# phcavelar/graph-odenet

Measured on AMD Instinct MI355X. Metric: full-graph ODE-GCN forward+backward steps/sec at 64 RK4 evals, higher is better.
Workload: dtype f32; 1 GPU; RMAT scale-20 / 10000000 edges (+self loops, dedup) row-normalised, d=128, ODEGCN3 rk4(3/8) 16 steps = 64 f-evals fwd, adjoint bwd, Adam; one graph per GPU; nodes=1048576, nnz=10758918, nfeat=128, hidden=128, nclass=16, parallelism=dp1 (one graph per rank, 1 gradient all-reduce/step)

## Files before the change

### graph_odenet_amd/_lib.py

```python
import ctypes
import os

import torch

_HERE = os.path.dirname(os.path.abspath(__file__))
LIB_PATH = os.path.join(_HERE, "libgraphode.so")

GODE_MAX_TERMS = 8


class LinComb(ctypes.Structure):
    _fields_ = [("n", ctypes.c_int32),
                ("coef", ctypes.c_float * GODE_MAX_TERMS),
                ("ptr", ctypes.c_void_p * GODE_MAX_TERMS)]


class SpmmEpilogue(ctypes.Structure):
    _fields_ = [("bias", ctypes.c_void_p), ("relu", ctypes.c_int32), ("alpha", ctypes.c_float),
                ("pre", LinComb), ("cot", LinComb), ("Y2", ctypes.c_void_p), ("Y2_colsum", ctypes.c_void_p)]


class Graph(ctypes.Structure):
    _fields_ = [("rowptr", ctypes.c_void_p), ("col", ctypes.c_void_p), ("val", ctypes.c_void_p),
                ("items", ctypes.c_void_p), ("n_items", ctypes.c_int64),
                ("long_rows", ctypes.c_void_p), ("n_long", ctypes.c_int64), ("partial", ctypes.c_void_p),
                ("n_rows", ctypes.c_int64), ("nnz", ctypes.c_int64)]


class GcnOdeFunc(ctypes.Structure):
    _fields_ = [("A", Graph), ("AT", Graph), ("n", ctypes.c_int64), ("d", ctypes.c_int64),
                ("groups", ctypes.c_int32), ("eps", ctypes.c_float),
                ("W", ctypes.c_void_p), ("b", ctypes.c_void_p), ("gamma", ctypes.c_void_p), ("beta", ctypes.c_void_p)]


class GatProj(ctypes.Structure):
    _fields_ = [("ps", ctypes.c_void_p), ("ld_s", ctypes.c_int64), ("pt", ctypes.c_void_p), ("ld_t", ctypes.c_int64),
                ("as_", ctypes.c_void_p), ("at", ctypes.c_void_p), ("ld_a", ctypes.c_int64)]


class Rk4Workspace(ctypes.Structure):
    _fields_ = [("S", ctypes.c_void_p), ("dZ", ctypes.c_void_p), ("dS", ctypes.c_void_p), ("S2", ctypes.c_void_p),
                ("ky", ctypes.c_void_p * 4), ("ka", ctypes.c_void_p * 4), ("ktheta", ctypes.c_void_p * 4),
                ("wpart", ctypes.c_void_p), ("gpart", ctypes.c_void_p), ("bpart", ctypes.c_void_p),
                ("colsum_scratch", ctypes.c_void_p), ("X", ctypes.c_void_p * 2), ("small_part", ctypes.c_void_p),
                ("y2_colsum", ctypes.c_void_p)]


class ReduceSeg(ctypes.Structure):
    _fields_ = [("out", ctypes.c_void_p), ("part", ctypes.c_void_p), ("n_part", ctypes.c_int64), ("ld", ctypes.c_int64),
                ("col0", ctypes.c_int64), ("col_stride", ctypes.c_int64), ("len", ctypes.c_int64),
                ("w_row0", ctypes.c_void_p), ("time_len", ctypes.c_int64)]


class GatOdeFunc(ctypes.Structure):
    _fields_ = [("mt", Graph), ("ms_inc", Graph), ("mt_inc", Graph), ("src", ctypes.c_void_p), ("tgt", ctypes.c_void_p),
                ("n_edges", ctypes.c_int64), ("n", ctypes.c_int64), ("d", ctypes.c_int64), ("groups", ctypes.c_int32),
                ("eps_gn", ctypes.c_float), ("eps", ctypes.c_float), ("Wsrc", ctypes.c_void_p), ("Wtgt", ctypes.c_void_p),
                ("Wlog", ctypes.c_void_p), ("bf", ctypes.c_void_p), ("bw", ctypes.c_void_p), ("gamma", ctypes.c_void_p),
                ("beta", ctypes.c_void_p), ("heads", ctypes.c_int32), ("Wpacked", ctypes.c_void_p)]


class GatWorkspace(ctypes.Structure):
    _fields_ = [(k, ctypes.c_void_p) for k in ("X", "Ps", "Pt", "A2", "a", "amax", "wgt", "den", "logits_scratch", "dz", "da",
                                               "dPs", "dPt", "dA2", "pair", "gp", "bp")] + \
               [("wp", ctypes.c_void_p * 3), ("maxpath_scratch", ctypes.c_void_p), ("colsum_scratch", ctypes.c_void_p),
                ("zeros", ctypes.c_void_p), ("heads_scratch", ctypes.c_void_p), ("colsum_scratch2", ctypes.c_void_p),
                ("small_part", ctypes.c_void_p)]


GODE_ADAM_MAX_TENSORS = 64


class AdamArgs(ctypes.Structure):
    _fields_ = [("param", ctypes.c_void_p * GODE_ADAM_MAX_TENSORS), ("grad", ctypes.c_void_p * GODE_ADAM_MAX_TENSORS),
                ("exp_avg", ctypes.c_void_p * GODE_ADAM_MAX_TENSORS), ("exp_avg_sq", ctypes.c_void_p * GODE_ADAM_MAX_TENSORS),
                ("len", ctypes.c_int64 * GODE_ADAM_MAX_TENSORS)]


c_i64 = ctypes.c_int64
c_p = ctypes.c_void_p
c_f = ctypes.c_float
c_i = ctypes.c_int

SIGNATURES = {
    "gode_abi_version": (c_i, []),
    "gode_error_string": (ctypes.c_char_p, [c_i]),
    "gode_set_option": (c_i, [ctypes.c_char_p, c_i]),
    "gode_get_option": (c_i, [ctypes.c_char_p]),
    "gode_spmm_csr_f32": (c_i, [c_p, c_p, c_p, c_p, c_i64, c_p, c_i64, c_p, c_p, c_i64, c_p, c_i64,
                                c_i64, c_i64, ctypes.POINTER(SpmmEpilogue), c_p]),
    "gode_spmm_csr_save_f32": (c_i, [c_p, c_p, c_p, c_p, c_i64, c_p, c_i64, c_p, c_p, c_i64, c_p, c_i64,
                                     c_i64, c_i64, ctypes.POINTER(SpmmEpilogue), c_p, c_p]),
    "gode_masked_cot_parts": (c_i64, [c_i64, c_i64]),
    "gode_masked_cot_f32": (c_i, [ctypes.POINTER(LinComb), c_p, c_p, c_i64, c_i64, c_p, c_p]),
    "gode_lincomb_f32": (c_i, [c_p, ctypes.POINTER(LinComb), c_i64, c_p]),
    "gode_lincomb_multi_f32": (c_i, [c_p, c_p, c_p, ctypes.c_int32, c_p]),
    "gode_rk_errnorm_multi_f32": (c_i, [c_p, c_p, c_p, c_p, c_p, ctypes.c_int32, c_f, c_f, c_p, c_p]),
    "gode_rk_errnorm_scratch_bytes": (c_i64, []),
    "gode_rk_errnorm_f32": (c_i, [c_p, c_p, c_p, ctypes.POINTER(LinComb), c_f, c_f, c_i64, c_p, c_p]),
    "gode_rk_scaled_sumsq_f32": (c_i, [c_p, ctypes.POINTER(LinComb), c_p, c_f, c_f, c_i64, c_p, c_p]),
    "gode_gn_time_gemm_f32": (c_i, [ctypes.POINTER(LinComb), c_i64, c_i64, ctypes.c_int32, c_f, c_p, c_p,
                                    c_p, c_i64, c_i, c_f, c_p, c_p]),
    "gode_gn_time_gemm_xout_f32": (c_i, [ctypes.POINTER(LinComb), c_i64, c_i64, ctypes.c_int32, c_f, c_p, c_p,
                                         c_p, c_i64, c_i, c_f, c_p, c_p, c_p]),
    "gode_gn_time_gemm_pair_f32": (c_i, [ctypes.POINTER(LinComb), c_i64, c_i64, ctypes.c_int32, c_f, c_p, c_p, c_p, c_p,
                                         c_i, c_f, c_p, c_p, c_p, c_p]),
    "gode_gemm_bwd_parts": (c_i64, [c_i64]),
    "gode_gn_time_gemm_bwd_f32": (c_i, [ctypes.POINTER(LinComb), c_i64, c_i64, ctypes.c_int32, c_f, c_p,
                                        c_p, c_i64, c_i, c_p, c_f, ctypes.POINTER(LinComb), c_p, c_p, c_p, c_p]),
    "gode_bwd_wgrad_supported": (c_i, [c_i64, c_i64, c_i64, ctypes.c_int32]),
    "gode_bwd_wgrad_parts": (c_i64, [c_i64]),
    "gode_gn_time_gemm_bwd_wgrad_f32": (c_i, [ctypes.POINTER(LinComb), c_i64, c_i64, ctypes.c_int32, c_f, c_p, c_p, c_p, c_i64, c_i,
                                              c_p, c_f, ctypes.POINTER(LinComb), c_p, c_p, c_p, c_p, c_p]),
    "gode_group_norm_parts": (c_i64, [c_i64]),
    "gode_group_norm_f32_fwd": (c_i, [c_p, c_i64, c_i64, ctypes.c_int32, c_f, c_p, c_p, c_p, c_p]),
    "gode_group_norm_f32_bwd": (c_i, [c_p, c_i64, c_i64, ctypes.c_int32, c_f, c_p, c_p, c_p, c_p, c_p, c_p]),
    "gode_rect_gemm_f32": (c_i, [c_p, c_i64, c_i64, c_i64, c_p, c_i64, c_p, c_i64, c_p]),
    "gode_rect_gemm_nt_f32": (c_i, [c_p, c_i64, c_i64, c_i64, c_p, c_i64, c_p, c_i64, c_p]),
    "gode_rect_wgrad_parts": (c_i64, [c_i64]),
    "gode_rect_wgrad_f32": (c_i, [c_p, c_i64, c_i64, c_i64, c_p, c_i64, c_i64, c_p, c_p]),
    "gode_rect_wgrad_sum_f32": (c_i, [c_p, c_i64, c_i64, c_i64, c_p, c_i64, c_i64, c_p, c_p, c_p]),
    "gode_gemm_f32": (c_i, [c_i, c_i, c_i64, c_i64, c_i64, c_p, c_i64, c_p, c_i64, c_p, c_i64, c_p, c_i, c_p, c_i64, c_p]),
    "gode_gemm_splitk_parts": (c_i64, [c_i64, c_i64, c_i64]),
    "gode_gemm_splitk_f32": (c_i, [c_i, c_i, c_i64, c_i64, c_i64, c_p, c_i64, c_p, c_i64, c_p, c_p, c_p]),
    "gode_cut_pad": (c_i64, [c_i64]),
    "gode_cut_bf16x3_f32": (c_i, [c_p, c_i64, c_i64, c_i64, c_p, c_p]),
    "gode_pgemm_workspace_bytes": (c_i64, [c_i64, c_i64, c_i64]),
    "gode_pgemm_bf16x3": (c_i, [c_i, c_i, c_i64, c_i64, c_i64, c_p, c_p, c_p, c_i64, c_p, c_i, c_p, c_i64, c_i, c_p, c_p]),
    "gode_adam_chunk": (c_i64, []),
    "gode_adam_tick_f32": (c_i, [c_p, c_f, c_f, c_p]),
    "gode_adam_f32": (c_i, [ctypes.POINTER(AdamArgs), ctypes.c_int32, c_p, c_i64, c_p, c_f, c_f, c_f, c_f, c_f, c_p]),
    "gode_gat_small_supported": (c_i, [c_i64, c_i64, ctypes.c_int32, c_i64]),
    "gode_gat_small_parts": (c_i64, [c_i64, c_i64]),
    "gode_gat_small_part_len": (c_i64, [c_i64, c_i64]),
    "gode_gat_project_small_f32": (c_i, [ctypes.POINTER(LinComb), c_i64, c_i64, ctypes.c_int32, c_f, c_p, c_p, c_p, c_p, c_p,
                                         c_i64, c_p, c_f, c_p, c_p, c_p, c_p, c_p, c_p]),
    "gode_gat_small_pack_len": (c_i64, [c_i64, c_i64]),
    "gode_gat_small_pack_f32": (c_i, [c_p, c_p, c_p, c_i64, c_i64, c_p, c_p]),
    "gode_gat_dense_vjp_small_f32": (c_i, [ctypes.POINTER(LinComb), c_i64, c_i64, ctypes.c_int32, c_f, c_p, c_p, c_p, c_p, c_p,
                                           c_i64, c_p, c_p, c_p, c_f, ctypes.POINTER(LinComb), c_p, c_p, c_p, c_p, c_p, c_i64, c_p, c_p]),
    "gode_gat_maxpath_heads_part_f32": (c_i, [c_p, c_p, c_i64, c_i64, c_p, c_p, c_p]),
    "gode_gat_heads_block_cap": (c_i64, []),
    "gode_gat_small_finish_f32": (c_i, [c_p, c_i64, c_i64, c_i64, c_f, c_p, c_p, c_p]),
    "gode_gat_small_finish_step_f32": (c_i, [c_p, c_i64, c_i64, c_i64, ctypes.c_int32, c_p, c_p, c_p, c_p, c_p]),
    "gode_gcn_small_supported": (c_i, [c_i64, c_i64, ctypes.c_int32]),
    "gode_gcn_small_parts": (c_i64, [c_i64]),
    "gode_gcn_small_part_len": (c_i64, [c_i64]),
    "gode_gcn_feval_small_f32": (c_i, [ctypes.POINTER(GcnOdeFunc), ctypes.POINTER(LinComb), c_f, c_f, ctypes.POINTER(LinComb),
                                       ctypes.POINTER(LinComb), c_p, c_p, c_p]),
    "gode_gcn_feval_small_next_f32": (c_i, [ctypes.POINTER(GcnOdeFunc), ctypes.POINTER(LinComb), c_f, c_f, ctypes.POINTER(LinComb),
                                            ctypes.POINTER(LinComb), c_p, c_p, ctypes.POINTER(LinComb), c_p, c_p]),
    "gode_gcn_vjp_small_f32": (c_i, [ctypes.POINTER(GcnOdeFunc), ctypes.POINTER(LinComb), c_p, c_f, ctypes.POINTER(LinComb),
                                     c_p, c_p, c_p]),
    "gode_gcn_vjp_small_next_f32": (c_i, [ctypes.POINTER(GcnOdeFunc), ctypes.POINTER(LinComb), c_p, c_f, ctypes.POINTER(LinComb),
                                          c_p, c_p, ctypes.POINTER(LinComb), c_p, c_p, c_p]),
    "gode_gcn_feval_small_save_f32": (c_i, [ctypes.POINTER(GcnOdeFunc), ctypes.POINTER(LinComb), c_f, c_f,
                                            ctypes.POINTER(LinComb), c_p, c_p, c_p]),
    "gode_gcn_small_finish_f32": (c_i, [ctypes.POINTER(GcnOdeFunc), c_p, c_p, c_f, c_p]),
    "gode_gcn_small_finish_multi_f32": (c_i, [ctypes.POINTER(GcnOdeFunc), c_p, ctypes.c_int32, ctypes.POINTER(c_p), ctypes.POINTER(c_f), c_p]),
    "gode_gcn_small_finish4_f32": (c_i, [ctypes.POINTER(GcnOdeFunc), c_p, c_p, c_p, c_p, c_p]),
    "gode_wgrad_parts": (c_i64, [c_i64]),
    "gode_wgrad_f32": (c_i, [ctypes.POINTER(LinComb), c_i64, c_i64, ctypes.c_int32, c_f, c_p, c_p,
                             c_p, c_i64, c_i, c_p, c_p]),
    "gode_reduce_parts_f32": (c_i, [c_p, c_p, c_i64, c_i64, c_f, c_i, c_p]),
    "gode_reduce_parts2_f32": (c_i, [c_p, c_p, c_p, c_p, c_i64, c_i64, c_f, c_i, c_p]),
    "gode_reduce_segments_f32": (c_i, [ctypes.POINTER(ReduceSeg), ctypes.c_int32, c_f, c_p, c_p]),
    "gode_colsum_parts_f32": (c_i, [c_p, c_i64, c_i64, c_p, ctypes.POINTER(c_i64), c_p]),
    "gode_colsum_scratch_bytes": (c_i64, [c_i64, c_i64]),
    "gode_spmm_y2_colsum_rows": (c_i64, [c_i64, c_i64, c_i64]),
    "gode_colsum_f32": (c_i, [c_p, c_p, c_i64, c_i64, c_f, c_i, c_p, c_p]),
    "gode_gat_logits_scratch_bytes": (c_i64, [c_i64]),
    "gode_gat_logits_f32": (c_i, [ctypes.POINTER(GatProj), c_p, c_p, c_p, c_i64, c_p, c_p, c_p, c_p]),
    "gode_gat_agg_f32_fwd": (c_i, [ctypes.POINTER(Graph), c_p, c_p, ctypes.POINTER(GatProj), c_i64, c_p, c_p, c_p, c_f,
                                   c_p, c_p, c_p, c_p]),
    "gode_gat_agg_f32_bwd": (c_i, [ctypes.POINTER(Graph), c_p, c_p, ctypes.POINTER(GatProj), c_i64, c_p, c_p, c_p, c_p,
                                   c_p, ctypes.POINTER(LinComb), c_f, c_p, c_p, c_p, c_i64, c_p, c_i64,
                                   ctypes.POINTER(ctypes.c_int32), c_p]),
    "gode_gat_maxpath_scratch_bytes": (c_i64, [c_i64]),
    "gode_gat_maxpath_f32": (c_i, [c_p, c_p, c_p, c_i64, c_p, c_p, c_i64, c_p, c_p]),
    "gode_gat_heads_scratch_bytes": (c_i64, [c_i64, c_i64]),
    "gode_gat_logits_heads_f32": (c_i, [ctypes.POINTER(GatProj), c_p, c_p, c_p, c_i64, c_i64, c_p, c_p, c_p, c_p]),
    "gode_gat_maxpath_heads_f32": (c_i, [c_p, c_p, c_i64, c_i64, c_p, c_p, c_i64, c_p, c_p]),
    "gode_gat_heads_parts": (c_i64, [c_i64]),
    "gode_gat_logits_heads_raw_f32": (c_i, [ctypes.POINTER(GatProj), c_p, c_p, c_p, c_i64, c_i64, c_p, c_p, c_p]),
    "gode_gat_agg_heads_f32_fwd": (c_i, [ctypes.POINTER(Graph), c_p, c_p, ctypes.POINTER(GatProj), c_i64, c_p, c_p, c_p, c_i64,
                                         c_i64, c_f, c_p, c_p, c_p, c_p]),
    "gode_gat_maxpath_heads_raw_f32": (c_i, [c_p, c_p, c_i64, c_i64, c_p, c_p, c_i64, c_p, c_p]),
# ... 126 lines not shown
```

### graph_odenet_amd/csrc/api.hip

```cpp
#include "common.h"

extern "C" int gode_abi_version(void) { return GODE_ABI_VERSION; }

extern "C" const char* gode_error_string(int code) {
    switch (code) {
        case 0: return "success";
        case GODE_E_NULLPTR: return "graphode: required pointer is NULL";
        case GODE_E_SHAPE: return "graphode: invalid shape / leading dimension";
        case GODE_E_ALIGN: return "graphode: operand not 16-byte aligned";
        case GODE_E_RANGE: return "graphode: argument out of range";
        case GODE_E_UNSUPPORTED: return "graphode: unsupported configuration";
        default: break;
    }
    if (code > 0) return hipGetErrorString((hipError_t)code);
    return "graphode: unknown error";
}

#include "options.h"
#include <cstdlib>
#include <cstring>

namespace {
int env_int(const char* name, int dflt) { const char* e = getenv(name); return e ? atoi(e) : dflt; }
int g_gemm_split = -1, g_overlap = -1, g_wgrad_split = -1, g_wgrad_split_small = 0, g_bwd_pc = -1, g_fwd_pc = -1, g_small_fused = -1, g_bwd_wgrad = -1, g_y2_colsum = -1;
}

int gode_opt_gemm_split() { if (g_gemm_split < 0) { const int v = env_int("GODE_GEMM_SPLIT", 2); g_gemm_split = (v == 1 || v == 2) ? v : 0; } return g_gemm_split; }
int gode_opt_wgrad_split() {
    if (g_wgrad_split < 0) { const int v = env_int("GODE_WGRAD_SPLIT", 8); g_wgrad_split = (v == 6 || v == 8) ? v : 0; }
    return g_wgrad_split;
}
int gode_opt_wgrad_split_small() { return g_wgrad_split_small; }
int gode_opt_bwd_pc() { if (g_bwd_pc < 0) g_bwd_pc = env_int("GODE_BWD_PC", 1) != 0; return g_bwd_pc; }
int gode_opt_fwd_pc() { if (g_fwd_pc < 0) g_fwd_pc = env_int("GODE_FWD_PC", 3) & 3; return g_fwd_pc; }
int gode_opt_small_fused() { if (g_small_fused < 0) g_small_fused = env_int("GODE_SMALL_FUSED", 1) != 0; return g_small_fused; }
int gode_opt_bwd_wgrad() { if (g_bwd_wgrad < 0) g_bwd_wgrad = env_int("GODE_BWD_WGRAD", 1) != 0; return g_bwd_wgrad; }
int gode_opt_y2_colsum() { if (g_y2_colsum < 0) g_y2_colsum = env_int("GODE_Y2_COLSUM", 1) != 0; return g_y2_colsum; }
int gode_opt_overlap() { if (g_overlap < 0) g_overlap = env_int("GODE_OVERLAP", 1) != 0; return g_overlap; }

extern "C" int gode_set_option(const char* name, int value) {
    if (!name) return GODE_E_NULLPTR;
    if (!strcmp(name, "gemm_split")) { if (value < 0 || value > 2) return GODE_E_UNSUPPORTED; g_gemm_split = value; return 0; }
    if (!strcmp(name, "overlap")) { g_overlap = value != 0; return 0; }
    if (!strcmp(name, "wgrad_split_small")) { g_wgrad_split_small = value != 0; return 0; }
    if (!strcmp(name, "bwd_pc")) { g_bwd_pc = value != 0; return 0; }
    if (!strcmp(name, "small_fused")) { g_small_fused = value != 0; return 0; }
    if (!strcmp(name, "bwd_wgrad")) { g_bwd_wgrad = value != 0; return 0; }
    if (!strcmp(name, "y2_colsum")) { g_y2_colsum = value != 0; return 0; }
    if (!strcmp(name, "fwd_pc")) { if (value < 0 || value > 3) return GODE_E_UNSUPPORTED; g_fwd_pc = value; return 0; }
    if (!strcmp(name, "wgrad_split")) { if (value != 0 && value != 6 && value != 8) return GODE_E_UNSUPPORTED; g_wgrad_split = value; return 0; }
    return GODE_E_UNSUPPORTED;
}
extern "C" int gode_get_option(const char* name) {
    if (!name) return GODE_E_NULLPTR;
    if (!strcmp(name, "gemm_split")) return gode_opt_gemm_split();
    if (!strcmp(name, "overlap")) return gode_opt_overlap();
    if (!strcmp(name, "wgrad_split")) return gode_opt_wgrad_split();
    if (!strcmp(name, "wgrad_split_small")) return gode_opt_wgrad_split_small();
    if (!strcmp(name, "bwd_pc")) return gode_opt_bwd_pc();
    if (!strcmp(name, "small_fused")) return gode_opt_small_fused();
    if (!strcmp(name, "bwd_wgrad")) return gode_opt_bwd_wgrad();
    if (!strcmp(name, "y2_colsum")) return gode_opt_y2_colsum();
    if (!strcmp(name, "fwd_pc")) return gode_opt_fwd_pc();
    return GODE_E_UNSUPPORTED;
}
```

### graph_odenet_amd/csrc/common.h

```cpp
#pragma once
#include <hip/hip_runtime.h>
#include <stdint.h>
#include "../../include/graphode.h"

#define GODE_WAVE 64

struct LinComb {
    int n;
    float coef[GODE_MAX_TERMS];
    const float* ptr[GODE_MAX_TERMS];
};

static inline LinComb make_lincomb(const gode_lincomb_t* h) {
    LinComb lc;
    lc.n = 0;
    for (int j = 0; j < GODE_MAX_TERMS; ++j) { lc.coef[j] = 0.f; lc.ptr[j] = nullptr; }
    if (h) {
        lc.n = h->n;
        for (int j = 0; j < h->n && j < GODE_MAX_TERMS; ++j) { lc.coef[j] = h->coef[j]; lc.ptr[j] = h->ptr[j]; }
    }
    return lc;
}

static inline int check_lincomb(const gode_lincomb_t* h, bool required) {
    if (!h) return required ? GODE_E_NULLPTR : 0;
    if (h->n < 0 || h->n > GODE_MAX_TERMS) return GODE_E_RANGE;
    if (required && h->n == 0) return GODE_E_RANGE;
    for (int j = 0; j < h->n; ++j) if (!h->ptr[j]) return GODE_E_NULLPTR;
    return 0;
}

static inline bool lincomb_aligned16(const gode_lincomb_t* h) {
    if (!h) return true;
    for (int j = 0; j < h->n; ++j) if (((uintptr_t)h->ptr[j]) & 15) return false;
    return true;
}

template <int NT>
__device__ __forceinline__ float4 lc_load4_n(const LinComb& lc, int64_t idx) {
    float4 v[NT];
#pragma unroll
    for (int j = 0; j < NT; ++j) v[j] = *reinterpret_cast<const float4*>(lc.ptr[j] + idx);
    float4 r = make_float4(0.f, 0.f, 0.f, 0.f);
#pragma unroll
    for (int j = 0; j < NT; ++j) {
        const float c = lc.coef[j];
        r.x = fmaf(c, v[j].x, r.x); r.y = fmaf(c, v[j].y, r.y);
        r.z = fmaf(c, v[j].z, r.z); r.w = fmaf(c, v[j].w, r.w);
    }
    return r;
}

__device__ __forceinline__ float4 lc_load4(const LinComb& lc, int64_t idx) {
    switch (lc.n) {
        case 1: return lc_load4_n<1>(lc, idx);
        case 2: return lc_load4_n<2>(lc, idx);
        case 3: return lc_load4_n<3>(lc, idx);
        case 4: return lc_load4_n<4>(lc, idx);
        case 5: return lc_load4_n<5>(lc, idx);
        case 6: return lc_load4_n<6>(lc, idx);
        case 7: return lc_load4_n<7>(lc, idx);
        case 8: return lc_load4_n<8>(lc, idx);
        default: return make_float4(0.f, 0.f, 0.f, 0.f);
    }
}

__device__ __forceinline__ float lc_load1(const LinComb& lc, int64_t idx) {
    float r = 0.f;
#pragma unroll
    for (int j = 0; j < GODE_MAX_TERMS; ++j)
        if (j < lc.n) r = fmaf(lc.coef[j], lc.ptr[j][idx], r);
    return r;
}

__device__ __forceinline__ float wave_sum(float v) {
#pragma unroll
    for (int o = 32; o > 0; o >>= 1) v += __shfl_xor(v, o, 64);
    return v;
}
__device__ __forceinline__ double wave_sum(double v) {
#pragma unroll
    for (int o = 32; o > 0; o >>= 1) v += __shfl_xor(v, o, 64);
    return v;
}
__device__ __forceinline__ float wave_max(float v) {
#pragma unroll
    for (int o = 32; o > 0; o >>= 1) v = fmaxf(v, __shfl_xor(v, o, 64));
    return v;
}

int gode_set_lds_once(const void* fn, size_t bytes);
int gode_zero_f32(float* out, int64_t n, void* stream);

#define GODE_LAUNCH_CHECK() do { hipError_t e__ = hipGetLastError(); if (e__ != hipSuccess) return (int)e__; } while (0)
```

### graph_odenet_amd/csrc/dense_pc.h

```cpp
#pragma once
#include "common.h"

int gode_pc_fwd_launch(const LinComb& lc, int64_t n_rows, float eps, const float* gamma, const float* beta,
                       const float* W, int has_time, float t, float* S, float* xout, int cg, hipStream_t s);
int gode_pc_bwd_launch(const LinComb& lc, int64_t n_rows, float eps, const float* gamma, const float* W, int has_time,
                       const float* dS, float out_scale, const LinComb& pre, float* dx, float* dgamma_part,
                       float* dbeta_part, int64_t n_part, int cg, hipStream_t s);
int64_t gode_pc_bwd_wgrad_parts(int64_t n_rows);
int gode_pc_bwd_wgrad_launch(const LinComb& lc, int64_t n_rows, float eps, const float* gamma, const float* beta, const float* W,
                             int has_time, const float* dS, float out_scale, const LinComb& pre, float* dx,
                             float* dgamma_part, float* dbeta_part, int64_t n_part, float* dW_part, int cg, hipStream_t s);
```

### graph_odenet_amd/csrc/gemm.hip

```cpp
#include <map>
#include <mutex>
#include <utility>
#include "common.h"
#include "dense_common.h"
#include "dense_pc.h"
#include "options.h"
#include "prof.h"

namespace {

constexpr int kMaxBlocks = 512;
constexpr int64_t kWgradSplitMinRows = 65536;

template <int D, int NTHREADS, bool TRANSPOSE>
__device__ __forceinline__ void fill_w_lds(float* Wl, const float* __restrict__ W, int has_time) {
    constexpr int LDW = D + 4;
    constexpr int N4 = D * D / 4;
    constexpr int IT = (N4 + NTHREADS - 1) / NTHREADS;
    float4 v[IT];
#pragma unroll
    for (int it = 0; it < IT; ++it) {
        const int idx = threadIdx.x + it * NTHREADS;
        v[it] = make_float4(0.f, 0.f, 0.f, 0.f);
        if (idx < N4) v[it] = ld4(W + (int64_t)has_time * D + (int64_t)idx * 4);
// ... 71 lines not shown
    }
}

template <int NJ>
__device__ __forceinline__ void mfma_panel(const float* wl , const float4 (&xv)[NJ], f32x4 (&acc)[NJ]) {
    constexpr int LDW = 16 * NJ + 4;
    float a[2][NJ];
#pragma unroll
    for (int tt = 0; tt < NJ; ++tt) a[0][tt] = wl[16 * tt];
#pragma unroll
    for (int s = 0; s < 4 * NJ; ++s) {
        const int j = s / 4, c = s % 4;
        const float xb = c == 0 ? xv[j].x : (c == 1 ? xv[j].y : (c == 2 ? xv[j].z : xv[j].w));
        if (s + 1 < 4 * NJ) {
            const int jn = (s + 1) / 4, cn = (s + 1) % 4;
#pragma unroll
            for (int tt = 0; tt < NJ; ++tt) a[(s + 1) & 1][tt] = wl[(16 * jn + cn) * LDW + 16 * tt];
        }
#pragma unroll
        for (int tt = 0; tt < NJ; ++tt)
            acc[tt] = __builtin_amdgcn_mfma_f32_16x16x4f32(a[s & 1][tt], xb, acc[tt], 0, 0, 0);
        __builtin_amdgcn_sched_barrier(0);
    }
}

template <int NJ, int S0, int S1>
__device__ __forceinline__ void mfma_panel_part(const float* wl, const float4 (&xv)[NJ], f32x4 (&acc)[NJ]) {
    constexpr int LDW = 16 * NJ + 4;
    float a[2][NJ];
#pragma unroll
    for (int tt = 0; tt < NJ; ++tt) a[S0 & 1][tt] = wl[(16 * (S0 / 4) + (S0 % 4)) * LDW + 16 * tt];
#pragma unroll
    for (int s = S0; s < S1; ++s) {
        const int j = s / 4, c = s % 4;
        const float xb = c == 0 ? xv[j].x : (c == 1 ? xv[j].y : (c == 2 ? xv[j].z : xv[j].w));
        if (s + 1 < S1) {
            const int jn = (s + 1) / 4, cn = (s + 1) % 4;
#pragma unroll
            for (int tt = 0; tt < NJ; ++tt) a[(s + 1) & 1][tt] = wl[(16 * jn + cn) * LDW + 16 * tt];
        }
#pragma unroll
        for (int tt = 0; tt < NJ; ++tt)
            acc[tt] = __builtin_amdgcn_mfma_f32_16x16x4f32(a[s & 1][tt], xb, acc[tt], 0, 0, 0);
        __builtin_amdgcn_sched_barrier(0);
    }
}

template <int NJ>
__device__ __forceinline__ void issue_terms2(const LinComb& lc, int t0, int64_t base, bool valid, float4 (&v)[2][NJ]) {
#pragma unroll
    for (int tt = 0; tt < 2; ++tt)
        if (valid && t0 + tt < lc.n) {
#pragma unroll
            for (int j = 0; j < NJ; ++j) v[tt][j] = ld4(lc.ptr[t0 + tt] + base + 16 * j);
        }
}
template <int NJ>
__device__ __forceinline__ void fold_terms2(const LinComb& lc, int t0, bool valid, const float4 (&v)[2][NJ], float4 (&xv)[NJ]) {
#pragma unroll
    for (int tt = 0; tt < 2; ++tt)
        if (valid && t0 + tt < lc.n) {
            const float c = lc.coef[t0 + tt];
#pragma unroll
            for (int j = 0; j < NJ; ++j) {
                xv[j].x = fmaf(c, v[tt][j].x, xv[j].x); xv[j].y = fmaf(c, v[tt][j].y, xv[j].y);
                xv[j].z = fmaf(c, v[tt][j].z, xv[j].z); xv[j].w = fmaf(c, v[tt][j].w, xv[j].w);
            }
        }
}

__device__ __forceinline__ float4 to_mfma_layout(const float4 v, int src_m_lane_x4) {
    return make_float4(__int_as_float(__builtin_amdgcn_ds_bpermute(src_m_lane_x4, __float_as_int(v.x))),
                       __int_as_float(__builtin_amdgcn_ds_bpermute(src_m_lane_x4, __float_as_int(v.y))),
                       __int_as_float(__builtin_amdgcn_ds_bpermute(src_m_lane_x4, __float_as_int(v.z))),
                       __int_as_float(__builtin_amdgcn_ds_bpermute(src_m_lane_x4, __float_as_int(v.w))));
}
__device__ __forceinline__ float4 acc_to_mem_layout(const f32x4 a, int src_f_lane_x4) {
    return make_float4(__int_as_float(__builtin_amdgcn_ds_bpermute(src_f_lane_x4, __float_as_int(a[0]))),
                       __int_as_float(__builtin_amdgcn_ds_bpermute(src_f_lane_x4, __float_as_int(a[1]))),
                       __int_as_float(__builtin_amdgcn_ds_bpermute(src_f_lane_x4, __float_as_int(a[2]))),
                       __int_as_float(__builtin_amdgcn_ds_bpermute(src_f_lane_x4, __float_as_int(a[3]))));
}

template <int NJ, int CG>
__global__ __launch_bounds__(256, 2) void gn_gemm_fwd_kernel(LinComb xin, int n_rows, float eps,
                                                             const float* __restrict__ gamma,
                                                             const float* __restrict__ beta,
                                                             const float* __restrict__ W, int has_time, float t,
                                                             float* __restrict__ S, float* __restrict__ xout,
                                                             const float* __restrict__ W2, float* __restrict__ S2)
{
    constexpr int D = 16 * NJ;
    constexpr int LDW = D + 4;
    extern __shared__ __attribute__((aligned(16))) float smem[];
    if (blockIdx.y == 1) { W = W2; S = S2; xout = nullptr; }
    float* Ws = smem;
    float* Gs = smem + D * LDW;
    float* Bs = Gs + D;
    float* T0 = Bs + D;
    fill_w_lds<D, 256, false>(Ws, W, has_time);
    fill_vec_lds<D, 256>(Gs, gamma, 1.f);
    fill_vec_lds<D, 256>(Bs, beta, 0.f);
    for (int c = threadIdx.x; c < D; c += 256) T0[c] = has_time ? t * W[c] : 0.f;
    __syncthreads();
    const int wave = threadIdx.x >> 6, l = threadIdx.x & 63;
    const int r = l & 15, g = l >> 4;
    const int mr = l >> 2, mg = l & 3;
    const int to_f = (4 * r + g) * 4, to_m = (mg * 16 + mr) * 4;
    const int n_tiles = (n_rows + 15) / 16;
    const int stride = gridDim.x * 4;
    int tile = blockIdx.x * 4 + wave;
    if (tile >= n_tiles) return;
    float4 nx[NJ];
    load_tile<NJ, 2>(xin, (int64_t)(tile * 16 + mr) * D + 4 * mg, tile * 16 + mr < n_rows, nx);
    for (; tile < n_tiles; tile += stride) {
        const int row = tile * 16 + mr;
        const bool valid = row < n_rows;
        const int nrow = row + stride * 16;
        const bool nvalid = (tile + stride < n_tiles) && nrow < n_rows;
        const int64_t nbase = (int64_t)nrow * D + 4 * mg;
        float4 xv[NJ];
#pragma unroll
        for (int j = 0; j < NJ; ++j) {
            if (xout != nullptr && valid) *reinterpret_cast<float4*>(xout + (int64_t)row * D + 16 * j + 4 * mg) = nx[j];
            xv[j] = gn_forward_v<CG>(nx[j], eps, ld4(Gs + 16 * j + 4 * mg), ld4(Bs + 16 * j + 4 * mg));
            xv[j] = to_mfma_layout(xv[j], to_f);
            nx[j] = make_float4(0.f, 0.f, 0.f, 0.f);
        }
        f32x4 acc[NJ];
#pragma unroll
        for (int tt = 0; tt < NJ; ++tt) {
            const float4 w0 = ld4(T0 + 16 * tt + 4 * g);
            acc[tt] = (f32x4){w0.x, w0.y, w0.z, w0.w};
        }
        float4 v[2][NJ];
        issue_terms2<NJ>(xin, 0, nbase, nvalid, v);
        mfma_panel_part<NJ, 0, 2 * NJ>(Ws + 4 * g * LDW + r, xv, acc);
        fold_terms2<NJ>(xin, 0, nvalid, v, nx);
        issue_terms2<NJ>(xin, 2, nbase, nvalid, v);
        mfma_panel_part<NJ, 2 * NJ, 4 * NJ>(Ws + 4 * g * LDW + r, xv, acc);
        fold_terms2<NJ>(xin, 2, nvalid, v, nx);
        if (xin.n > 4) { issue_terms2<NJ>(xin, 4, nbase, nvalid, v); fold_terms2<NJ>(xin, 4, nvalid, v, nx); }
        if (xin.n > 6) { issue_terms2<NJ>(xin, 6, nbase, nvalid, v); fold_terms2<NJ>(xin, 6, nvalid, v, nx); }
#pragma unroll
        for (int tt = 0; tt < NJ; ++tt) {
            const float4 o = acc_to_mem_layout(acc[tt], to_m);
            if (valid) *reinterpret_cast<float4*>(S + (int64_t)row * D + 16 * tt + 4 * mg) = o;
        }
    }
}


__device__ __forceinline__ unsigned short bf16_bits(float x) {
    const __bf16 h = (__bf16)x;
    return __builtin_bit_cast(unsigned short, h);
}
__device__ __forceinline__ float bf16_val(unsigned short b) { return __uint_as_float((unsigned)b << 16); }
__device__ __forceinline__ void split3(float x, unsigned short& h, unsigned short& m, unsigned short& l) {
    h = bf16_bits(x);
    const float r1 = x - bf16_val(h);
    m = bf16_bits(r1);
    l = bf16_bits(r1 - bf16_val(m));
}

template <int CG, int NX>
__global__ __launch_bounds__(512, 2) void gn_gemm_fwd_split_kernel(LinComb xin, int n_rows, float eps,
                                                                   const float* __restrict__ gamma,
                                                                   const float* __restrict__ beta,
                                                                   const float* __restrict__ W, int has_time, float t,
                                                                   float* __restrict__ S)
{
    constexpr int D = 128, NJ = 8, NK = 4;
    constexpr int LDK = D + 8;
    extern __shared__ __attribute__((aligned(16))) float smem[];
    unsigned short* Wp = reinterpret_cast<unsigned short*>(smem);
    float* Gs = smem + (3 * D * LDK) / 2;
    float* Bs = Gs + D;
    float* T0 = Bs + D;
    for (int idx = threadIdx.x; idx < D * D / 4; idx += 512) {
        const int k = idx / (D / 4), n = (idx % (D / 4)) * 4;
        const float4 w = ld4(W + (int64_t)(k + has_time) * D + n);
        const float wv[4] = {w.x, w.y, w.z, w.w};
#pragma unroll
        for (int q = 0; q < 4; ++q) {
            unsigned short h, m, l;
            split3(wv[q], h, m, l);
            Wp[(0 * D + n + q) * LDK + k] = h; Wp[(1 * D + n + q) * LDK + k] = m; Wp[(2 * D + n + q) * LDK + k] = l;
        }
    }
    fill_vec_lds<D, 512>(Gs, gamma, 1.f);
    fill_vec_lds<D, 512>(Bs, beta, 0.f);
    for (int c = threadIdx.x; c < D; c += 512) T0[c] = has_time ? t * W[c] : 0.f;
    __syncthreads();
    const int wave = threadIdx.x >> 6, l = threadIdx.x & 63;
    const int r = l & 15, g = l >> 4;
    const int mr = l >> 2, mg = l & 3;
    const int to_m = (mg * 16 + mr) * 4;
    const int n_tiles = (n_rows + 15) / 16;
    constexpr int NXR = NX > 0 ? NX : 1;
    float4 raw[NXR][NJ];
    auto request = [&](int tile) {
        const int rr = tile * 16 + mr;
        const int64_t base = (int64_t)(rr < n_rows ? rr : n_rows - 1) * D + 4 * mg;
#pragma unroll
        for (int t = 0; t < NXR; ++t)
#pragma unroll
            for (int j = 0; j < NJ; ++j) raw[t][j] = ld4(xin.ptr[t] + base + 16 * j);
    };
    if (NX > 0 && blockIdx.x * 8 + wave < n_tiles) request(blockIdx.x * 8 + wave);
    for (int tile = blockIdx.x * 8 + wave; tile < n_tiles; tile += gridDim.x * 8) {
        const int row = tile * 16 + mr;
        const bool valid = row < n_rows;
        float4 xv[NJ];
        if (NX > 0) {
#pragma unroll
            for (int j = 0; j < NJ; ++j) {
                xv[j] = make_float4(0.f, 0.f, 0.f, 0.f);
#pragma unroll
                for (int t = 0; t < NXR; ++t) {
                    const float c = xin.coef[t];
                    xv[j].x = fmaf(c, raw[t][j].x, xv[j].x); xv[j].y = fmaf(c, raw[t][j].y, xv[j].y);
                    xv[j].z = fmaf(c, raw[t][j].z, xv[j].z); xv[j].w = fmaf(c, raw[t][j].w, xv[j].w);
                }
                if (!valid) xv[j] = make_float4(0.f, 0.f, 0.f, 0.f);
            }
            const int nt_ = tile + gridDim.x * 8;
// ... 870 lines not shown
int fast_cg(int64_t d_in, int64_t d_out, int32_t groups) {
    if (d_in != d_out) return -1;
    if (d_in != 16 && d_in != 32 && d_in != 64 && d_in != 128) return -1;
    if (groups == 0) return 0;
    if (d_in % groups) return -1;
    const int64_t cg = d_in / groups;
    if (cg == 1 || cg == 2 || cg == 4) return (int)cg;
    return -1;
}

int narrow_cg(int64_t d_in, int64_t d_out, int32_t groups) {
    if (d_out != 2) return -1;
    if (d_in != 16 && d_in != 32 && d_in != 64 && d_in != 128) return -1;
    if (groups == 0) return 0;
    if (d_in % groups) return -1;
    const int64_t cg = d_in / groups;
    return (cg == 1 || cg == 2 || cg == 4) ? (int)cg : -1;
}

int64_t fwd_blocks(int64_t n_rows) {
    int64_t b = ((n_rows + 15) / 16 + 3) / 4;
    if (b < 1) b = 1;
    if (b > kMaxBlocks) b = kMaxBlocks;
    return b;
}
int64_t wgrad_blocks(int64_t n_rows) {
    int64_t b = (n_rows + 31) / 32;
    if (b < 1) b = 1;
    if (b > kMaxBlocks) b = kMaxBlocks;
    return b;
}

}

int gode_set_lds_once(const void* fn, size_t bytes) {
    if (bytes <= 64 * 1024) return 0;
    static std::mutex mu;
    static std::map<std::pair<int, const void*>, size_t> done;
    int dev = 0;
    hipError_t e = hipGetDevice(&dev);
    if (e != hipSuccess) return (int)e;
    std::lock_guard<std::mutex> lk(mu);
    auto key = std::make_pair(dev, fn);
    auto it = done.find(key);
    if (it != done.end() && it->second >= bytes) return 0;
    e = hipFuncSetAttribute(fn, hipFuncAttributeMaxDynamicSharedMemorySize, (int)bytes);
    if (e != hipSuccess) return (int)e;
    done[key] = bytes;
    return 0;
}

#define GODE_DISPATCH_NJ_CG(NJV, CGV, MACRO)                                        \
    if (nj == NJV && cg == CGV) { MACRO(NJV, CGV) }

#define GODE_DISPATCH_ALL(MACRO)                                                    \
    GODE_DISPATCH_NJ_CG(1, 0, MACRO) GODE_DISPATCH_NJ_CG(1, 1, MACRO)               \
    GODE_DISPATCH_NJ_CG(2, 0, MACRO) GODE_DISPATCH_NJ_CG(2, 1, MACRO)               \
    GODE_DISPATCH_NJ_CG(4, 0, MACRO) GODE_DISPATCH_NJ_CG(4, 2, MACRO)               \
    GODE_DISPATCH_NJ_CG(8, 0, MACRO) GODE_DISPATCH_NJ_CG(8, 4, MACRO)               \
    GODE_DISPATCH_NJ_CG(1, 2, MACRO) GODE_DISPATCH_NJ_CG(1, 4, MACRO)               \
    GODE_DISPATCH_NJ_CG(2, 2, MACRO) GODE_DISPATCH_NJ_CG(2, 4, MACRO)               \
    GODE_DISPATCH_NJ_CG(4, 1, MACRO) GODE_DISPATCH_NJ_CG(4, 4, MACRO)               \
    GODE_DISPATCH_NJ_CG(8, 1, MACRO) GODE_DISPATCH_NJ_CG(8, 2, MACRO)

static int check_common(const gode_lincomb_t* xin, int64_t n_rows, int64_t d_in, int32_t groups, int64_t d_out) {
    if (n_rows < 0 || d_in <= 0 || d_out <= 0 || groups < 0) return GODE_E_SHAPE;
    if (groups > 0 && d_in % groups) return GODE_E_SHAPE;
    if (n_rows > INT32_MAX || d_in > 2048 || d_out > 65536) return GODE_E_RANGE;
    return check_lincomb(xin, true);
}

extern "C" int gode_gn_time_gemm_f32(const gode_lincomb_t* xin, int64_t n_rows, int64_t d_in, int32_t groups,
                                     float eps, const float* gamma, const float* beta, const float* W,
                                     int64_t d_out, int has_time, float t, float* S, void* stream)
{
    return gode_gn_time_gemm_xout_f32(xin, n_rows, d_in, groups, eps, gamma, beta, W, d_out, has_time, t, S, nullptr,
                                      stream);
}

extern "C" int gode_gn_time_gemm_xout_f32(const gode_lincomb_t* xin, int64_t n_rows, int64_t d_in, int32_t groups,
                                          float eps, const float* gamma, const float* beta, const float* W,
                                          int64_t d_out, int has_time, float t, float* S, float* x_out, void* stream)
{
    int rc = check_common(xin, n_rows, d_in, groups, d_out); if (rc) return rc;
    if (n_rows == 0) return 0;
    if (!W || !S) return GODE_E_NULLPTR;
    if (x_out && (((uintptr_t)x_out) & 15)) return GODE_E_ALIGN;
    has_time = has_time ? 1 : 0;
    hipStream_t s = (hipStream_t)stream;
    LinComb lc = make_lincomb(xin);
    const int cg = fast_cg(d_in, d_out, groups);
    const bool al = lincomb_aligned16(xin) && !(((uintptr_t)S) & 15) && !(((uintptr_t)W) & 15) &&
                    (!gamma || !(((uintptr_t)gamma) & 15)) && (!beta || !(((uintptr_t)beta) & 15));
    if (cg >= 0 && al && d_in == 128 && (n_rows >= kWgradSplitMinRows || gode_opt_wgrad_split_small()) &&
        ((lc.n <= 2 && !x_out) ? (gode_opt_fwd_pc() & 1) : (gode_opt_fwd_pc() & 2))) {
        rc = gode_pc_fwd_launch(lc, n_rows, eps, gamma, beta, W, has_time, t, S, x_out, cg, s);
        if (rc != GODE_E_UNSUPPORTED) return rc;
    }
    if (cg >= 0 && al && d_in == 128 && !x_out && (gode_opt_gemm_split() == 1 || (gode_opt_gemm_split() == 2 && lc.n <= 2 && n_rows >= 65536))) {
        const size_t lds = (size_t)3 * 128 * (128 + 8) * sizeof(unsigned short) + 3 * 128 * sizeof(float);
        int64_t blocks = ((n_rows + 15) / 16 + 7) / 8; if (blocks < 1) blocks = 1; if (blocks > 256) blocks = 256;
#define GODE_FWDS2(CGV, NXV) { rc = set_lds(gn_gemm_fwd_split_kernel<CGV, NXV>, lds); if (rc) return rc;    \
          const int slot = gode_prof_begin(s, d_in, n_rows, (int64_t)lc.n - 1, GODE_PROF_GEMM_FWD | GODE_PROF_FORM_SPLIT); \
          hipLaunchKernelGGL((gn_gemm_fwd_split_kernel<CGV, NXV>), dim3((unsigned)blocks), dim3(512), lds, s, \
                             lc, (int)n_rows, eps, gamma, beta, W, has_time, t, S);                           \
          gode_prof_end(s, slot);                                                                             \
          GODE_LAUNCH_CHECK(); return 0; }
#define GODE_FWDS(CGV) { if (lc.n == 1) GODE_FWDS2(CGV, 1) else if (lc.n == 2) GODE_FWDS2(CGV, 2) else GODE_FWDS2(CGV, 0) }
        if (cg == 0) GODE_FWDS(0) else if (cg == 1) GODE_FWDS(1) else if (cg == 2) GODE_FWDS(2) else GODE_FWDS(4)
#undef GODE_FWDS
#undef GODE_FWDS2
    }
    if (cg >= 0 && al) {
        const int nj = (int)(d_in / 16);
        const size_t lds = ((size_t)d_in * (d_in + 4) + 3 * d_in) * sizeof(float);
        const int64_t blocks = fwd_blocks(n_rows);
#define GODE_FWD(NJV, CGV)                                                                          \
        { rc = set_lds(gn_gemm_fwd_kernel<NJV, CGV>, lds); if (rc) return rc;                       \
          const int slot = gode_prof_begin(s, d_in, n_rows, (int64_t)lc.n - 1 + (x_out ? 1 : 0), GODE_PROF_GEMM_FWD); \
          hipLaunchKernelGGL((gn_gemm_fwd_kernel<NJV, CGV>), dim3((unsigned)blocks), dim3(256), lds, s, \
                             lc, (int)n_rows, eps, gamma, beta, W, has_time, t, S, x_out,           \
                             (const float*)nullptr, (float*)nullptr);                               \
          gode_prof_end(s, slot);                                                                   \
          GODE_LAUNCH_CHECK(); return 0; }
        GODE_DISPATCH_ALL(GODE_FWD)
#undef GODE_FWD
    }
    {
        const int cg = narrow_cg(d_in, d_out, groups);
        if (cg >= 0 && al) {
            const int nj = (int)(d_in / 16);
            const int64_t blocks = fwd_blocks(n_rows);
#define GODE_NFWD(NJV, CGV)                                                                                 \
            { hipLaunchKernelGGL((gn_narrow_fwd_kernel<NJV, CGV, 2>), dim3((unsigned)blocks), dim3(256), 0, s, \
                                 lc, (int)n_rows, eps, gamma, beta, W, has_time, t, S, x_out);              \
              GODE_LAUNCH_CHECK(); return 0; }
            GODE_DISPATCH_ALL(GODE_NFWD)
#undef GODE_NFWD
        }
    }
    if (x_out) { rc = gode_lincomb_f32(x_out, xin, n_rows * d_in, stream); if (rc) return rc; }
    const size_t lds = ((size_t)RB * d_in + (size_t)RB * (groups > 0 ? groups : 1) * 2) * sizeof(float);
    rc = set_lds(gn_gemm_fwd_generic, lds); if (rc) return rc;
    int64_t blocks = (n_rows + RB - 1) / RB; if (blocks > 2048) blocks = 2048;
    hipLaunchKernelGGL(gn_gemm_fwd_generic, dim3((unsigned)blocks), dim3(256), lds, s, lc, (int)n_rows, (int)d_in,
                       (int)groups, eps, gamma, beta, W, (int)d_out, has_time, t, S);
    GODE_LAUNCH_CHECK();
    return 0;
}

extern "C" int gode_gn_time_gemm_pair_f32(const gode_lincomb_t* xin, int64_t n_rows, int64_t d, int32_t groups, float eps,
                                          const float* gamma, const float* beta, const float* Wa, const float* Wb,
                                          int has_time, float t, float* Sa, float* Sb, float* x_out, void* stream)
{
    int rc = check_common(xin, n_rows, d, groups, d); if (rc) return rc;
    if (n_rows == 0) return 0;
    if (!Wa || !Wb || !Sa || !Sb) return GODE_E_NULLPTR;
    has_time = has_time ? 1 : 0;
    hipStream_t s = (hipStream_t)stream;
    LinComb lc = make_lincomb(xin);
    const int cg = fast_cg(d, d, groups);
    const bool al = lincomb_aligned16(xin) && !((((uintptr_t)Sa) | ((uintptr_t)Sb) | ((uintptr_t)Wa) | ((uintptr_t)Wb)) & 15) &&
                    (!gamma || !(((uintptr_t)gamma) & 15)) && (!beta || !(((uintptr_t)beta) & 15)) &&
                    (!x_out || !(((uintptr_t)x_out) & 15));
    if (cg >= 0 && al) {
        const int nj = (int)(d / 16);
        const size_t lds = ((size_t)d * (d + 4) + 3 * d) * sizeof(float);
        const int64_t blocks = fwd_blocks(n_rows);
#define GODE_FWDP(NJV, CGV)                                                                         \
        { rc = set_lds(gn_gemm_fwd_kernel<NJV, CGV>, lds); if (rc) return rc;                       \
          hipLaunchKernelGGL((gn_gemm_fwd_kernel<NJV, CGV>), dim3((unsigned)blocks, 2), dim3(256), lds, s, \
                             lc, (int)n_rows, eps, gamma, beta, Wa, has_time, t, Sa, x_out, Wb, Sb);  \
          GODE_LAUNCH_CHECK(); return 0; }
        GODE_DISPATCH_ALL(GODE_FWDP)
#undef GODE_FWDP
    }
    rc = gode_gn_time_gemm_xout_f32(xin, n_rows, d, groups, eps, gamma, beta, Wa, d, has_time, t, Sa, x_out, stream);
    if (rc) return rc;
    return gode_gn_time_gemm_f32(xin, n_rows, d, groups, eps, gamma, beta, Wb, d, has_time, t, Sb, stream);
}

extern "C" int64_t gode_gemm_bwd_parts(int64_t n_rows) {
    int64_t a = fwd_blocks(n_rows);
    int64_t b = (n_rows + RB - 1) / RB; if (b > 2048) b = 2048; if (b < 1) b = 1;
    return a > b ? a : b;
}

extern "C" int gode_gn_time_gemm_bwd_f32(const gode_lincomb_t* xin, int64_t n_rows, int64_t d_in, int32_t groups,
                                         float eps, const float* gamma, const float* W, int64_t d_out,
                                         int has_time, const float* dS, float out_scale,
                                         const gode_lincomb_t* pre, float* dx,
                                         float* dgamma_part, float* dbeta_part, void* stream)
{
    int rc = check_common(xin, n_rows, d_in, groups, d_out); if (rc) return rc;
    if (n_rows == 0) return 0;
    if (!W || !dS || !dx) return GODE_E_NULLPTR;
    if ((dgamma_part == nullptr) != (dbeta_part == nullptr)) return GODE_E_NULLPTR;
    if (pre && pre->n > 0) { rc = check_lincomb(pre, true); if (rc) return rc; } else pre = nullptr;
    has_time = has_time ? 1 : 0;
    hipStream_t s = (hipStream_t)stream;
    LinComb lc = make_lincomb(xin);
    LinComb lpre = make_lincomb(pre);
    const int64_t n_part = gode_gemm_bwd_parts(n_rows);
    const int cg = fast_cg(d_in, d_out, groups);
    const bool al = lincomb_aligned16(xin) && lincomb_aligned16(pre) && !(((uintptr_t)dS) & 15) && !(((uintptr_t)dx) & 15) &&
                    (!gamma || !(((uintptr_t)gamma) & 15)) &&
                    (!dgamma_part || (!(((uintptr_t)dgamma_part) & 15) && !(((uintptr_t)dbeta_part) & 15)));
    if ((cg == 0 || cg == 4) && al && d_in == 128 && gode_opt_bwd_pc() &&
        (n_rows >= kWgradSplitMinRows || gode_opt_wgrad_split_small())) {
        rc = gode_pc_bwd_launch(lc, n_rows, eps, gamma, W, has_time, dS, out_scale, lpre, dx, dgamma_part, dbeta_part,
                                n_part, cg, s);
        if (rc != GODE_E_UNSUPPORTED) return rc;
    }
    if (cg >= 0 && al) {
        const int nj = (int)(d_in / 16);
        size_t lds = ((size_t)d_in * (d_in + 4) + d_in) * sizeof(float);
        if (lds < (size_t)8 * d_in * sizeof(float)) lds = (size_t)8 * d_in * sizeof(float);
        const int64_t blocks = fwd_blocks(n_rows);
#define GODE_BWD(NJV, CGV)                                                                          \
        { rc = set_lds(gn_gemm_bwd_kernel<NJV, CGV>, lds); if (rc) return rc;                       \
          const int slot = gode_prof_begin(s, d_in, n_rows, (int64_t)lc.n - 1 + lpre.n, GODE_PROF_GEMM_BWD); \
          hipLaunchKernelGGL((gn_gemm_bwd_kernel<NJV, CGV>), dim3((unsigned)blocks), dim3(256), lds, s, \
                             lc, (int)n_rows, eps, gamma, W, has_time, dS, out_scale, lpre, dx, dgamma_part, dbeta_part, (int)n_part); \
          gode_prof_end(s, slot);                                                                   \
          GODE_LAUNCH_CHECK(); return 0; }
        GODE_DISPATCH_ALL(GODE_BWD)
#undef GODE_BWD
    }
    {
        const int ncg = narrow_cg(d_in, d_out, groups);
        if (ncg >= 0 && al) {
            const int nj = (int)(d_in / 16);
            const int cg = ncg;
            const int64_t blocks = fwd_blocks(n_rows);
#define GODE_NBWD(NJV, CGV)                                                                                 \
            { hipLaunchKernelGGL((gn_narrow_bwd_kernel<NJV, CGV, 2>), dim3((unsigned)blocks), dim3(256), 0, s, \
                                 lc, (int)n_rows, eps, gamma, W, has_time, dS, out_scale, lpre, dx, dgamma_part, \
                                 dbeta_part, (int)n_part);                                                  \
              GODE_LAUNCH_CHECK(); return 0; }
            GODE_DISPATCH_ALL(GODE_NBWD)
#undef GODE_NBWD
        }
    }
    const size_t g2 = (size_t)RB * (groups > 0 ? groups : 1) * 2;
    const size_t lds = ((size_t)RB * d_in * 2 + g2 * 2) * sizeof(float);
    rc = set_lds(gn_gemm_bwd_generic, lds); if (rc) return rc;
    int64_t blocks = (n_rows + RB - 1) / RB; if (blocks > 2048) blocks = 2048;
    hipLaunchKernelGGL(gn_gemm_bwd_generic, dim3((unsigned)blocks), dim3(256), lds, s, lc, (int)n_rows, (int)d_in,
                       (int)groups, eps, gamma, W, (int)d_out, has_time, dS, out_scale, lpre, dx, dgamma_part, dbeta_part,
                       (int)n_part);
    GODE_LAUNCH_CHECK();
    return 0;
}

extern "C" int gode_bwd_wgrad_supported(int64_t n_rows, int64_t d_in, int64_t d_out, int32_t groups) {
// ... 143 lines not shown
```

### graph_odenet_amd/csrc/gemm_pc.hip

```cpp
#include "common.h"
#include "dense_common.h"
#include "dense_pc.h"
#include "prof.h"

namespace {

constexpr int D = 128;
constexpr int LDK = D + 8;
constexpr int LDX = D + 4;
constexpr int kBlocks = 256;
template <int R> struct Img { static constexpr int PIECE_B = R * LDK * 2, BUF_B = 3 * PIECE_B; };

__device__ __forceinline__ bf16x8 pack8(const unsigned (&u)[8]) {
    const uint2 a = pack_hi16x4(u[0], u[1], u[2], u[3]), b = pack_hi16x4(u[4], u[5], u[6], u[7]);
    typedef unsigned u32x4 __attribute__((ext_vector_type(4)));
    const u32x4 v = {a.x, a.y, b.x, b.y};
    return __builtin_bit_cast(bf16x8, v);
}

template <typename F>
__device__ __forceinline__ void load_weight_pieces(bf16x8 (&A)[4][3], F element) {
    const int l = threadIdx.x & 63, m = l & 15, g = l >> 4;
#pragma unroll
    for (int kb = 0; kb < 4; ++kb) {
        unsigned h[8], md[8], lo[8];
#pragma unroll
        for (int e = 0; e < 8; ++e) split3_trunc(element(m, 32 * kb + 8 * g + e), h[e], md[e], lo[e]);
        A[kb][0] = pack8(h); A[kb][1] = pack8(md); A[kb][2] = pack8(lo);
    }
}

template <int R>
__device__ __forceinline__ void tile_product(const char* img , const bf16x8 (&A)[4][3], f32x4 (&acc)[R / 16]) {
    constexpr int PIECE_B = Img<R>::PIECE_B, NS = (R / 16) * 4;
    bf16x8 b[2][3];
#pragma unroll
    for (int pc = 0; pc < 3; ++pc) b[0][pc] = *reinterpret_cast<const bf16x8*>(img + pc * PIECE_B);
#pragma unroll
    for (int s = 0; s < NS; ++s) {
        const int rt = s >> 2, kb = s & 3;
        if (s + 1 < NS) {
            const int rt2 = (s + 1) >> 2, kb2 = (s + 1) & 3;
#pragma unroll
            for (int pc = 0; pc < 3; ++pc)
                b[(s + 1) & 1][pc] = *reinterpret_cast<const bf16x8*>(img + pc * PIECE_B + rt2 * 16 * LDK * 2 + kb2 * 64);
        }
        const bf16x8 bh = b[s & 1][0], bm = b[s & 1][1], bl = b[s & 1][2];
        f32x4 c = acc[rt];
        c = __builtin_amdgcn_mfma_f32_16x16x32_bf16(A[kb][2], bm, c, 0, 0, 0);
        c = __builtin_amdgcn_mfma_f32_16x16x32_bf16(A[kb][1], bl, c, 0, 0, 0);
        c = __builtin_amdgcn_mfma_f32_16x16x32_bf16(A[kb][2], bh, c, 0, 0, 0);
        c = __builtin_amdgcn_mfma_f32_16x16x32_bf16(A[kb][0], bl, c, 0, 0, 0);
        c = __builtin_amdgcn_mfma_f32_16x16x32_bf16(A[kb][1], bm, c, 0, 0, 0);
        c = __builtin_amdgcn_mfma_f32_16x16x32_bf16(A[kb][1], bh, c, 0, 0, 0);
        c = __builtin_amdgcn_mfma_f32_16x16x32_bf16(A[kb][0], bm, c, 0, 0, 0);
        c = __builtin_amdgcn_mfma_f32_16x16x32_bf16(A[kb][0], bh, c, 0, 0, 0);
        acc[rt] = c;
        __builtin_amdgcn_sched_barrier(0);
    }
}

template <int PIECE_B>
__device__ __forceinline__ void stage_row4(char* dst , const float4 v) {
    unsigned h0, m0, l0, h1, m1, l1, h2, m2, l2, h3, m3, l3;
    split3_trunc(v.x, h0, m0, l0); split3_trunc(v.y, h1, m1, l1); split3_trunc(v.z, h2, m2, l2); split3_trunc(v.w, h3, m3, l3);
    *reinterpret_cast<uint2*>(dst) = pack_hi16x4(h0, h1, h2, h3);
    *reinterpret_cast<uint2*>(dst + PIECE_B) = pack_hi16x4(m0, m1, m2, m3);
    *reinterpret_cast<uint2*>(dst + 2 * PIECE_B) = pack_hi16x4(l0, l1, l2, l3);
}

struct TileWalk {
    int n_tiles, stride, mine;
    __device__ TileWalk(int n_rows, int R) {
        n_tiles = (n_rows + R - 1) / R;
        stride = gridDim.x;
        mine = (int)blockIdx.x < n_tiles ? (n_tiles - 1 - (int)blockIdx.x) / stride + 1 : 0;
    }
    __device__ int tile(int k) const { return blockIdx.x + k * stride; }
    __device__ int clamped(int k) const { return blockIdx.x + (k < mine ? k : (mine > 0 ? mine - 1 : 0)) * stride; }
};

template <int CG, int NX, bool XOUT, int R>
__global__ __launch_bounds__(1024, 1) void gn_gemm_fwd_pc_kernel(LinComb xin, int n_rows, float eps,
                                                                const float* __restrict__ gamma,
                                                                const float* __restrict__ beta,
                                                                const float* __restrict__ W, int has_time, float t,
                                                                float* __restrict__ S, float* __restrict__ xout)
{
    constexpr int PIECE_B = Img<R>::PIECE_B, BUF_B = Img<R>::BUF_B;
    constexpr int RPT = R / 8;
    extern __shared__ __attribute__((aligned(16))) float smem[];
    char* lds = reinterpret_cast<char*>(smem);
    const TileWalk tw(n_rows, R);
    if (threadIdx.x >= 512) {
        const int grp = (threadIdx.x - 512) >> 8, pt = (threadIdx.x - 512) & 255;
        const int trow = pt >> 5, tcol = 4 * (pt & 31);
        const float4 gmv = gamma ? ld4(gamma + tcol) : make_float4(1.f, 1.f, 1.f, 1.f);
        const float4 btv = beta ? ld4(beta + tcol) : make_float4(0.f, 0.f, 0.f, 0.f);
        constexpr int NXR = NX > 0 ? NX : 1;
        float4 xr[NXR][RPT];
        auto prefetch = [&](int k) {
            const int tile = tw.clamped(k);
#pragma unroll
            for (int p = 0; p < RPT; ++p) {
                const int row = tile * R + RPT * trow + p;
                const int64_t off = (int64_t)(row < n_rows ? row : n_rows - 1) * D + tcol;
                if (NX > 0) {
#pragma unroll
                    for (int j = 0; j < NXR; ++j) xr[j][p] = ld4(xin.ptr[j] + off);
                } else {
                    xr[0][p] = lc_load4(xin, off);
                }
            }
        };
        auto stage = [&](int k) {
            char* img = lds + (k & 1) * BUF_B + (RPT * trow) * LDK * 2 + tcol * 2;
            const int tile = tw.tile(k);
#pragma unroll
            for (int p = 0; p < RPT; ++p) {
                const int row = tile * R + RPT * trow + p;
                float4 x = xr[0][p];
                if (NX > 0) {
                    x = make_float4(0.f, 0.f, 0.f, 0.f);
#pragma unroll
                    for (int j = 0; j < NXR; ++j) {
                        const float c = xin.coef[j];
                        x.x = fmaf(c, xr[j][p].x, x.x); x.y = fmaf(c, xr[j][p].y, x.y);
                        x.z = fmaf(c, xr[j][p].z, x.z); x.w = fmaf(c, xr[j][p].w, x.w);
                    }
                }
                if (XOUT && row < n_rows) *reinterpret_cast<float4*>(xout + (int64_t)row * D + tcol) = x;
                float4 xn = gn_forward_v<CG>(x, eps, gmv, btv);
                if (row >= n_rows) xn = make_float4(0.f, 0.f, 0.f, 0.f);
                stage_row4<PIECE_B>(img + p * LDK * 2, xn);
            }
        };
        prefetch(grp);
        if (grp == 0 && tw.mine > 0) { stage(0); prefetch(2); }
        lds_barrier();
        for (int k = 0; k < tw.mine; ++k) {
            if (((k + 1) & 1) == grp && k + 1 < tw.mine) { stage(k + 1); prefetch(k + 3); }
            lds_barrier();
        }
        return;
    }
    const int wave = threadIdx.x >> 6, l = threadIdx.x & 63, r = l & 15, g = l >> 4;
    const int n0 = 16 * wave;
    bf16x8 A[4][3];
    load_weight_pieces(A, [&](int m, int k) { return W[(int64_t)(k + has_time) * D + n0 + m]; });
    f32x4 t0 = {0.f, 0.f, 0.f, 0.f};
    if (has_time) { const float4 w0 = ld4(W + n0 + 4 * g); t0 = (f32x4){t * w0.x, t * w0.y, t * w0.z, t * w0.w}; }
    const int rd_off = r * LDK * 2 + g * 16;
    lds_barrier();
    for (int k = 0; k < tw.mine; ++k) {
        f32x4 acc[R / 16];
#pragma unroll
        for (int rt = 0; rt < R / 16; ++rt) acc[rt] = t0;
        tile_product<R>(lds + (k & 1) * BUF_B + rd_off, A, acc);
        const int row0 = tw.tile(k) * R + r;
#pragma unroll
        for (int rt = 0; rt < R / 16; ++rt) {
            const int row = row0 + 16 * rt;
            if (row < n_rows)
                *reinterpret_cast<float4*>(S + (int64_t)row * D + n0 + 4 * g) = make_float4(acc[rt][0], acc[rt][1], acc[rt][2], acc[rt][3]);
        }
        lds_barrier();
    }
}

template <int CG, int NX, bool XLDS>
__global__ __launch_bounds__(1024, 1) void gn_gemm_bwd_pc_kernel(LinComb xin, int n_rows, float eps,
                                                                const float* __restrict__ gamma,
                                                                const float* __restrict__ W, int has_time,
                                                                const float* __restrict__ dS, float out_scale,
                                                                LinComb pre, float* __restrict__ dx,
                                                                float* __restrict__ dgamma_part,
                                                                float* __restrict__ dbeta_part, int n_part)
{
    constexpr int R = 32, PIECE_B = Img<R>::PIECE_B;
    constexpr int XT_B = (CG != 0 && XLDS) ? R * LDX * 4 : 0;
    constexpr int BUF_B = Img<R>::BUF_B + XT_B;
    extern __shared__ __attribute__((aligned(16))) float smem[];
    char* lds = reinterpret_cast<char*>(smem);
    const TileWalk tw(n_rows, R);
    if (threadIdx.x >= 512) {
        const int grp = (threadIdx.x - 512) >> 8, pt = (threadIdx.x - 512) & 255;
        const int trow = pt >> 5, tcol = 4 * (pt & 31);
        constexpr int NXR = NX > 0 ? NX : 1;
        float4 gr[4], xr[NXR][4];
        auto prefetch = [&](int k) {
            const int tile = tw.clamped(k);
#pragma unroll
            for (int p = 0; p < 4; ++p) {
                const int row = tile * R + 4 * trow + p;
                const int64_t off = (int64_t)(row < n_rows ? row : n_rows - 1) * D + tcol;
                gr[p] = ld4(dS + off);
                if (CG != 0 && XLDS) {
                    if (NX > 0) {
#pragma unroll
                        for (int j = 0; j < NXR; ++j) xr[j][p] = ld4(xin.ptr[j] + off);
                    } else {
                        xr[0][p] = lc_load4(xin, off);
                    }
                }
            }
        };
        auto stage = [&](int k) {
            char* buf = lds + (k & 1) * BUF_B;
            char* img = buf + (4 * trow) * LDK * 2 + tcol * 2;
            const int tile = tw.tile(k);
#pragma unroll
            for (int p = 0; p < 4; ++p) {
                float4 v = gr[p];
                if (tile * R + 4 * trow + p >= n_rows) v = make_float4(0.f, 0.f, 0.f, 0.f);
// ... 261 lines not shown
                if (valid) {
                    dgs.x += dy.x * xh.x; dgs.y += dy.y * xh.y; dgs.z += dy.z * xh.z; dgs.w += dy.w * xh.w;
                    dbs.x += dy.x; dbs.y += dy.y; dbs.z += dy.z; dbs.w += dy.w;
                }
                const float m1 = ((dh.x + dh.y) + (dh.z + dh.w)) * 0.25f;
                const float m2 = ((dh.x * xh.x + dh.y * xh.y) + (dh.z * xh.z + dh.w * xh.w)) * 0.25f;
                const float rs = rstd.x;
                o4 = make_float4(rs * (dh.x - m1 - xh.x * m2), rs * (dh.y - m1 - xh.y * m2),
                                 rs * (dh.z - m1 - xh.z * m2), rs * (dh.w - m1 - xh.w * m2));
            }
            if (valid) {
                float4 o = make_float4(out_scale * o4.x, out_scale * o4.y, out_scale * o4.z, out_scale * o4.w);
                if (pre.n > 0) {
                    const float4 pv = lc_load4(pre, (int64_t)row * D + c0);
                    o.x += pv.x; o.y += pv.y; o.z += pv.z; o.w += pv.w;
                }
                *reinterpret_cast<float4*>(dx + (int64_t)row * D + c0) = o;
            }
        }
        const char* Gp = buf + tr_off;
        const char* Xp = buf + IMG_B + tr_off;
        bf16x8 Bf[2][3];
#pragma unroll
        for (int b = 0; b < 2; ++b)
#pragma unroll
            for (int pc = 0; pc < 3; ++pc) Bf[b][pc] = tr_frag(Gp + pc * PIECE_B, 16 * (b0 + b) * 2);
#pragma unroll
        for (int a = 0; a < 4; ++a) {
            bf16x8 Af[3];
#pragma unroll
            for (int pc = 0; pc < 3; ++pc) Af[pc] = tr_frag(Xp + pc * PIECE_B, 16 * (a0 + a) * 2);
#pragma unroll
            for (int b = 0; b < 2; ++b) {
                f32x4 c = wacc[a][b];
                c = __builtin_amdgcn_mfma_f32_16x16x32_bf16(Af[2], Bf[b][1], c, 0, 0, 0);
                c = __builtin_amdgcn_mfma_f32_16x16x32_bf16(Af[1], Bf[b][2], c, 0, 0, 0);
                c = __builtin_amdgcn_mfma_f32_16x16x32_bf16(Af[2], Bf[b][0], c, 0, 0, 0);
                c = __builtin_amdgcn_mfma_f32_16x16x32_bf16(Af[0], Bf[b][2], c, 0, 0, 0);
                c = __builtin_amdgcn_mfma_f32_16x16x32_bf16(Af[1], Bf[b][1], c, 0, 0, 0);
                c = __builtin_amdgcn_mfma_f32_16x16x32_bf16(Af[1], Bf[b][0], c, 0, 0, 0);
                c = __builtin_amdgcn_mfma_f32_16x16x32_bf16(Af[0], Bf[b][1], c, 0, 0, 0);
                c = __builtin_amdgcn_mfma_f32_16x16x32_bf16(Af[0], Bf[b][0], c, 0, 0, 0);
                wacc[a][b] = c;
            }
        }
        lds_barrier();
    }
#pragma unroll
    for (int a = 0; a < 4; ++a)
#pragma unroll
        for (int b = 0; b < 2; ++b)
#pragma unroll
            for (int q = 0; q < 4; ++q) {
                const int i = 16 * (a0 + a) + 4 * g + q;
                out[(int64_t)(i + has_time) * D + 16 * (b0 + b) + r] = wacc[a][b][q];
            }
    if (CG != 0 && dgamma_part) {
#pragma unroll
        for (int o = 1; o < 16; o <<= 1) {
            dgs.x += __shfl_xor(dgs.x, o, 64); dgs.y += __shfl_xor(dgs.y, o, 64); dgs.z += __shfl_xor(dgs.z, o, 64); dgs.w += __shfl_xor(dgs.w, o, 64);
            dbs.x += __shfl_xor(dbs.x, o, 64); dbs.y += __shfl_xor(dbs.y, o, 64); dbs.z += __shfl_xor(dbs.z, o, 64); dbs.w += __shfl_xor(dbs.w, o, 64);
        }
        if (r == 0) {
            *reinterpret_cast<float4*>(dgamma_part + (int64_t)blockIdx.x * D + c0) = dgs;
            *reinterpret_cast<float4*>(dbeta_part + (int64_t)blockIdx.x * D + c0) = dbs;
        }
    }
    __syncthreads();
}

int64_t pc_blocks(int64_t n_rows, int R) {
    int64_t b = (n_rows + R - 1) / R;
    if (b < 1) b = 1;
    if (b > kBlocks) b = kBlocks;
    return b;
}

template <typename K>
int set_lds_pc(K kernel, size_t bytes) { return gode_set_lds_once(reinterpret_cast<const void*>(kernel), bytes); }

}

int gode_pc_fwd_launch(const LinComb& lc, int64_t n_rows, float eps, const float* gamma, const float* beta,
                       const float* W, int has_time, float t, float* S, float* xout, int cg, hipStream_t s)
{
    int rc = 0;
#define GODE_FPC4(CGV, NXV, XO, RV)                                                                               \
    { const size_t lds = 2 * (size_t)Img<RV>::BUF_B;                                                               \
      const int64_t blocks = pc_blocks(n_rows, RV);                                                                \
      rc = set_lds_pc(gn_gemm_fwd_pc_kernel<CGV, NXV, XO, RV>, lds); if (rc) return rc;                            \
      const int slot = gode_prof_begin(s, D, n_rows, (int64_t)lc.n - 1 + (XO ? 1 : 0), GODE_PROF_GEMM_FWD | GODE_PROF_FORM_PC); \
      hipLaunchKernelGGL((gn_gemm_fwd_pc_kernel<CGV, NXV, XO, RV>), dim3((unsigned)blocks), dim3(1024), lds, s,    \
                         lc, (int)n_rows, eps, gamma, beta, W, has_time, t, S, xout);                             \
      gode_prof_end(s, slot);                                                                                      \
      GODE_LAUNCH_CHECK(); return 0; }
#define GODE_FPC2(CGV, NXV, RV) { if (xout) GODE_FPC4(CGV, NXV, true, RV) else GODE_FPC4(CGV, NXV, false, RV) }
#define GODE_FPC(CGV) { switch (lc.n) { case 1: GODE_FPC2(CGV, 1, 32) case 2: GODE_FPC2(CGV, 2, 32) case 3: GODE_FPC2(CGV, 3, 32) \
                                        case 4: GODE_FPC2(CGV, 4, 32) default: GODE_FPC2(CGV, 0, 32) } }
    if (cg == 0) GODE_FPC(0) else if (cg == 1) GODE_FPC(1) else if (cg == 2) GODE_FPC(2) else if (cg == 4) GODE_FPC(4)
#undef GODE_FPC
#undef GODE_FPC2
#undef GODE_FPC4
    return GODE_E_UNSUPPORTED;
}

int gode_pc_bwd_launch(const LinComb& lc, int64_t n_rows, float eps, const float* gamma, const float* W, int has_time,
                       const float* dS, float out_scale, const LinComb& pre, float* dx, float* dgamma_part,
                       float* dbeta_part, int64_t n_part, int cg, hipStream_t s)
{
    const int64_t blocks = pc_blocks(n_rows, 32);
    int rc = 0;
#define GODE_BPC3(CGV, NXV, XL)                                                                                   \
    { const size_t lds = 2 * ((size_t)Img<32>::BUF_B + ((CGV != 0 && XL) ? 32 * LDX * 4 : 0));                     \
      rc = set_lds_pc(gn_gemm_bwd_pc_kernel<CGV, NXV, XL>, lds); if (rc) return rc;                                \
      const int slot = gode_prof_begin(s, D, n_rows, (int64_t)lc.n - 1 + pre.n, GODE_PROF_GEMM_BWD | GODE_PROF_FORM_PC); \
      hipLaunchKernelGGL((gn_gemm_bwd_pc_kernel<CGV, NXV, XL>), dim3((unsigned)blocks), dim3(1024), lds, s,        \
                         lc, (int)n_rows, eps, gamma, W, has_time, dS, out_scale, pre, dx, dgamma_part, dbeta_part, \
                         (int)n_part);                                                                             \
      gode_prof_end(s, slot);                                                                                      \
      GODE_LAUNCH_CHECK(); return 0; }
#define GODE_BPC(CGV) { if (lc.n == 1) GODE_BPC3(CGV, 1, false) else if (lc.n == 2) GODE_BPC3(CGV, 2, true) else GODE_BPC3(CGV, 0, true) }
    if (cg == 0) GODE_BPC3(0, 1, false) else if (cg == 4) GODE_BPC(4)
#undef GODE_BPC
#undef GODE_BPC3
    return GODE_E_UNSUPPORTED;
}

int64_t gode_pc_bwd_wgrad_parts(int64_t n_rows) { return pc_blocks(n_rows, 32); }

int gode_pc_bwd_wgrad_launch(const LinComb& lc, int64_t n_rows, float eps, const float* gamma, const float* beta, const float* W,
                             int has_time, const float* dS, float out_scale, const LinComb& pre, float* dx,
                             float* dgamma_part, float* dbeta_part, int64_t n_part, float* dW_part, int cg, hipStream_t s)
{
    const int64_t blocks = pc_blocks(n_rows, 32);
    int rc = 0;
#define GODE_BW(CGV, NXV)                                                                                          \
    { const size_t lds = 2 * ((size_t)2 * 3 * Img<32>::PIECE_B + (CGV != 0 ? 32 * LDX * 4 : 0));                     \
      rc = set_lds_pc(gn_gemm_bwd_wgrad_pc_kernel<CGV, NXV>, lds); if (rc) return rc;                               \
      const int slot = gode_prof_begin(s, D, n_rows, (int64_t)lc.n - 1 + pre.n, GODE_PROF_BWD_WGRAD | GODE_PROF_FORM_PC); \
      hipLaunchKernelGGL((gn_gemm_bwd_wgrad_pc_kernel<CGV, NXV>), dim3((unsigned)blocks), dim3(768), lds, s,         \
                         lc, (int)n_rows, eps, gamma, beta, W, has_time, dS, out_scale, pre, dx, dgamma_part,       \
                         dbeta_part, (int)n_part, dW_part);                                                        \
      gode_prof_end(s, slot);                                                                                       \
      GODE_LAUNCH_CHECK(); return 0; }
#define GODE_BWN(CGV) { if (lc.n == 1) GODE_BW(CGV, 1) else if (lc.n == 2) GODE_BW(CGV, 2) else GODE_BW(CGV, 0) }
    if (cg == 0) GODE_BWN(0) else if (cg == 4) GODE_BWN(4)
#undef GODE_BWN
#undef GODE_BW
    return GODE_E_UNSUPPORTED;
}
```

### graph_odenet_amd/csrc/ode_driver.hip

```cpp
#include <map>
#include <mutex>
#include <utility>
#include "common.h"
#include "options.h"

namespace {

const double C38[4] = {0.0, 1.0 / 3.0, 2.0 / 3.0, 1.0};
const double A38[4][3] = {{0.0, 0.0, 0.0}, {1.0 / 3.0, 0.0, 0.0}, {-1.0 / 3.0, 1.0, 0.0}, {1.0, -1.0, 1.0}};
const double B38[4] = {1.0 / 8.0, 3.0 / 8.0, 3.0 / 8.0, 1.0 / 8.0};

gode_lincomb_t stage_terms(const float* y, float* const* k, int s, double h) {
    gode_lincomb_t lc;
    lc.n = 0;
    lc.coef[lc.n] = 1.f; lc.ptr[lc.n] = y; ++lc.n;
    for (int j = 0; j < s; ++j)
        if (A38[s][j] != 0.0) { lc.coef[lc.n] = (float)(h * A38[s][j]); lc.ptr[lc.n] = k[j]; ++lc.n; }
    return lc;
}
gode_lincomb_t combine_terms(const float* y, float* const* k, double h) {
    gode_lincomb_t lc;
    lc.n = 0;
    lc.coef[lc.n] = 1.f; lc.ptr[lc.n] = y; ++lc.n;
    for (int j = 0; j < 3; ++j) { lc.coef[lc.n] = (float)(h * B38[j]); lc.ptr[lc.n] = k[j]; ++lc.n; }
    return lc;
}

int spmm(const gode_graph_t& g, const float* X, float* Y, int64_t d, const gode_spmm_epilogue_t* ep, void* s) {
    return gode_spmm_csr_f32(g.rowptr, g.col, g.val, g.items, g.n_items, g.long_rows, g.n_long, g.partial,
                             X, d, Y, d, g.n_rows, d, ep, s);
}

__global__ void theta_fixup_kernel(float* ktheta, const float* W, float t, int d, int64_t off_at) {
    __shared__ float sm[4];
    float s = 0.f;
    for (int c = threadIdx.x; c < d; c += blockDim.x) s += ktheta[c] * W[c];
    s = wave_sum(s);
    if ((threadIdx.x & 63) == 0) sm[threadIdx.x >> 6] = s;
    __syncthreads();
    if (threadIdx.x == 0) ktheta[off_at] = sm[0] + sm[1] + sm[2] + sm[3];
    __syncthreads();
    for (int c = threadIdx.x; c < d; c += blockDim.x) ktheta[c] *= t;
}

#define GODE_TRY(expr) do { int rc__ = (expr); if (rc__) return rc__; } while (0)

constexpr int64_t kMergedFinishMaxRows = 1 << 16;

int stage_finish_merged(const gode_gcn_odefunc_t* f, const gode_rk4_workspace_t* ws, float* kt, float ts, void* stream) {
    const int64_t n = f->n, d = f->d, nW = (d + 1) * d, P = gode_gcn_ode_theta_len(d);
    int64_t cparts = 0;
    GODE_TRY(gode_colsum_parts_f32(ws->dZ, n, d, (float*)ws->colsum_scratch, &cparts, stream));
    const int64_t gp = gode_gemm_bwd_parts(n);
    gode_reduce_seg_t sg[4] = {};
    sg[0] = {kt, ws->wpart, gode_wgrad_parts(n), nW, 0, 1, nW, f->W, d};
    sg[1] = {kt + nW, (const float*)ws->colsum_scratch, cparts, d, 0, 1, d, nullptr, 0};
    sg[2] = {kt + nW + d, ws->gpart, gp, d, 0, 1, d, nullptr, 0};
    sg[3] = {kt + nW + 2 * d, ws->bpart, gp, d, 0, 1, d, nullptr, 0};
    GODE_TRY(gode_reduce_segments_f32(sg, f->groups > 0 ? 4 : 2, ts, kt + (P - 1), stream));
    if (f->groups <= 0) GODE_TRY(gode_zero_f32(kt + nW + d, 2 * d, stream));
    return 0;
}

bool fused_small(const gode_gcn_odefunc_t* f) {
    return gode_opt_small_fused() && gode_gcn_small_supported(f->n, f->d, f->groups);
}
gode_lincomb_t negated(gode_lincomb_t lc) { for (int j = 0; j < lc.n; ++j) lc.coef[j] = -lc.coef[j]; return lc; }

}

extern "C" int64_t gode_gcn_ode_theta_len(int64_t d) { return (d + 1) * d + 3 * d + 1; }

extern "C" int gode_gcn_ode_rk4_forward(const gode_gcn_odefunc_t* f, float* y, float** result,
                                        const gode_rk4_workspace_t* ws, float t0, float t1, int32_t n_steps,
                                        void* stream)
{
    if (!f || !y || !ws || !result) return GODE_E_NULLPTR;
    if (n_steps <= 0 || f->n <= 0 || f->d <= 0) return GODE_E_SHAPE;
    if (!ws->S || !ws->ky[0] || !ws->ky[1] || !ws->ky[2] || !ws->ky[3]) return GODE_E_NULLPTR;
    const int64_t n = f->n, d = f->d;
    const double h = ((double)t1 - (double)t0) / n_steps;
    float* cur = y;
    float* k[4] = {ws->ky[0], ws->ky[1], ws->ky[2], ws->ky[3]};
    const bool fused = fused_small(f);
    for (int i = 0; i < n_steps; ++i) {
        const double t = (double)t0 + i * h;
        for (int s = 0; s < 4; ++s) {
            gode_lincomb_t xin = stage_terms(cur, k, s, h);
            if (fused) {
                gode_lincomb_t pre = combine_terms(cur, k, h);
                GODE_TRY(gode_gcn_feval_small_f32(f, &xin, (float)(t + C38[s] * h), s == 3 ? (float)(h * B38[3]) : 1.f,
                                                  s == 3 ? &pre : nullptr, nullptr, nullptr, k[s], stream));
                continue;
            }
            GODE_TRY(gode_gn_time_gemm_f32(&xin, n, d, f->groups, f->eps, f->gamma, f->beta, f->W, d, 1,
                                           (float)(t + C38[s] * h), ws->S, stream));
            gode_spmm_epilogue_t ep = {};
            ep.bias = f->b; ep.relu = 1; ep.alpha = 1.f;
            if (s == 3) { ep.pre = combine_terms(cur, k, h); ep.alpha = (float)(h * B38[3]); }
            GODE_TRY(spmm(f->A, ws->S, k[s], d, &ep, stream));
        }
        float* tmp = cur; cur = k[3]; k[3] = tmp;
    }
    *result = cur;
    return 0;
}

namespace {

struct Overlap {
    hipStream_t side = nullptr;
    hipEvent_t sp = nullptr, gf = nullptr, spt = nullptr, wg = nullptr;
    bool ok = false;
};
Overlap* overlap_ctx(hipStream_t caller) {
    static std::mutex mu;
    static std::map<std::pair<int, hipStream_t>, Overlap*> ctxs;
    int dev = 0;
    if (hipGetDevice(&dev) != hipSuccess) return nullptr;
    std::lock_guard<std::mutex> lk(mu);
    auto key = std::make_pair(dev, caller);
    auto it = ctxs.find(key);
    if (it != ctxs.end()) return it->second;
    Overlap* c = new Overlap();
    if (hipStreamCreateWithFlags(&c->side, hipStreamNonBlocking) == hipSuccess) {
        bool ok = true;
        for (hipEvent_t* ev : {&c->sp, &c->gf, &c->spt, &c->wg})
            ok = ok && hipEventCreateWithFlags(ev, hipEventDisableTiming) == hipSuccess;
        c->ok = ok;
    }
    ctxs[key] = c;
    return c;
}
#define GODE_HIP(expr) do { hipError_t e__ = (expr); if (e__ != hipSuccess) return (int)e__; } while (0)

}

extern "C" int gode_gcn_ode_rk4_adjoint(const gode_gcn_odefunc_t* f, float* y, float* a, float* theta,
                                        float** y_result, float** a_result,
                                        const gode_rk4_workspace_t* ws, float t0, float t1, int32_t n_steps,
                                        void* stream)
{
    if (!f || !y || !a || !theta || !ws || !y_result || !a_result) return GODE_E_NULLPTR;
    if (n_steps <= 0 || f->n <= 0 || f->d <= 0) return GODE_E_SHAPE;
    for (int s = 0; s < 4; ++s) if (!ws->ky[s] || !ws->ka[s] || !ws->ktheta[s]) return GODE_E_NULLPTR;
    if (!ws->S || !ws->dZ || !ws->dS || !ws->wpart || !ws->colsum_scratch) return GODE_E_NULLPTR;
    if (f->groups > 0 && (!ws->gpart || !ws->bpart)) return GODE_E_NULLPTR;
    const int64_t n = f->n, d = f->d;
    const int64_t nW = (d + 1) * d, P = gode_gcn_ode_theta_len(d);
    const double h = ((double)t1 - (double)t0) / n_steps;
    hipStream_t hs = (hipStream_t)stream;
    const bool small = f->n <= kMergedFinishMaxRows;
    Overlap* ov = (!small && ws->S2 != nullptr && gode_opt_overlap()) ? overlap_ctx(hs) : nullptr;
    const bool two = ov != nullptr && ov->ok;
    void* side = two ? (void*)ov->side : stream;
    float* Sbuf[2] = {ws->S, two ? ws->S2 : ws->S};
    float* ycur = y; float* acur = a;
    float* ky[4] = {ws->ky[0], ws->ky[1], ws->ky[2], ws->ky[3]};
    float* ka[4] = {ws->ka[0], ws->ka[1], ws->ka[2], ws->ka[3]};
    const int64_t wparts = gode_wgrad_parts(n), gparts = gode_gemm_bwd_parts(n);
    const int total = 4 * n_steps;
    const bool bw = !small && gode_bwd_wgrad_supported(n, d, d, f->groups) && gode_bwd_wgrad_parts(n) <= wparts;

    const bool mat = ws->X[0] != nullptr && ws->X[1] != nullptr;
    auto x_out_of = [&](int g) -> float* { return (mat && (g % 4) >= 2) ? ws->X[g & 1] : nullptr; };

    const bool fused = fused_small(f) && ws->small_part != nullptr;
    if (!fused) {
        gode_lincomb_t yin0 = stage_terms(ycur, ky, 0, h);
        GODE_TRY(gode_gn_time_gemm_xout_f32(&yin0, n, d, f->groups, f->eps, f->gamma, f->beta, f->W, d, 1,
                                            (float)((double)t0), Sbuf[0], x_out_of(0), stream));
    }
    bool wg_pending = false;
    float stage_t[4] = {0.f, 0.f, 0.f, 0.f};
    for (int g = 0; g < total; ++g) {
        const int i = g / 4, s = g % 4;
        const float ts = (float)((double)t0 + i * h + C38[s] * h);
        if (fused) {
            const gode_lincomb_t yin = stage_terms(ycur, ky, s, h);
            const gode_lincomb_t cot = negated(stage_terms(acur, ka, s, h));
            const gode_lincomb_t ypre = combine_terms(ycur, ky, h), apre = combine_terms(acur, ka, h);
            GODE_TRY(gode_gcn_feval_small_f32(f, &yin, ts, s == 3 ? (float)(h * B38[3]) : 1.f, s == 3 ? &ypre : nullptr,
                                              &cot, ws->dZ, ky[s], stream));
            const int64_t slot = gode_gcn_small_parts(n) * gode_gcn_small_part_len(d);
            GODE_TRY(gode_gcn_vjp_small_f32(f, &yin, ws->dZ, s == 3 ? (float)(h * B38[3]) : 1.f, s == 3 ? &apre : nullptr,
                                            ka[s], ws->small_part + s * slot, stream));
            stage_t[s] = ts;
            if (s == 3) {
                const float wb[4] = {(float)(h * B38[0]), (float)(h * B38[1]), (float)(h * B38[2]), (float)(h * B38[3])};
                GODE_TRY(gode_gcn_small_finish4_f32(f, ws->small_part, theta, wb, stage_t, stream));
                float* tmp = ycur; ycur = ky[3]; ky[3] = tmp;
                tmp = acur; acur = ka[3]; ka[3] = tmp;
            }
            continue;
        }
        gode_lincomb_t yin = stage_terms(ycur, ky, s, h);
        if (x_out_of(g)) { yin.n = 1; yin.coef[0] = 1.f; yin.ptr[0] = x_out_of(g); }
        gode_lincomb_t ain = stage_terms(acur, ka, s, h);
        gode_spmm_epilogue_t ep = {};
        ep.bias = f->b; ep.relu = 1; ep.alpha = 1.f;
        ep.cot = ain;
        for (int j = 0; j < ep.cot.n; ++j) ep.cot.coef[j] = -ep.cot.coef[j];
        ep.Y2 = ws->dZ;
        const int64_t y2rows = (bw && ws->y2_colsum && gode_opt_y2_colsum())
            ? gode_spmm_y2_colsum_rows(f->A.items ? f->A.n_items : f->A.n_rows, f->A.items ? f->A.n_long : 0, d) : 0;
        if (y2rows > 0) ep.Y2_colsum = ws->y2_colsum;
        gode_lincomb_t apre; apre.n = 0;
        if (s == 3) { ep.pre = combine_terms(ycur, ky, h); ep.alpha = (float)(h * B38[3]); apre = combine_terms(acur, ka, h); }
        if (two && g > 0) GODE_HIP(hipStreamWaitEvent(hs, ov->gf, 0));
        GODE_TRY(spmm(f->A, Sbuf[g & 1], ky[s], d, &ep, stream));
        float* ycur_n = ycur; float* ky_n[4] = {ky[0], ky[1], ky[2], ky[3]};
        if (s == 3) { ycur_n = ky[3]; ky_n[3] = ycur; }
        if (two && wg_pending) GODE_HIP(hipStreamWaitEvent(hs, ov->wg, 0));
        GODE_TRY(spmm(f->AT, ws->dZ, ws->dS, d, nullptr, stream));
        if (two) {
            GODE_HIP(hipEventRecord(ov->spt, hs));
            GODE_HIP(hipStreamWaitEvent(ov->side, ov->spt, 0));
        }
        float* kt = ws->ktheta[s];
        if (bw) {
            if (two) GODE_HIP(hipStreamWaitEvent(ov->side, ov->spt, 0));
            if (y2rows > 0) GODE_TRY(gode_colsum_f32(kt + nW, ws->y2_colsum, y2rows, d, 1.f, 0, ws->colsum_scratch, side));
            else GODE_TRY(gode_colsum_f32(kt + nW, ws->dZ, n, d, 1.f, 0, ws->colsum_scratch, side));
            GODE_TRY(gode_gn_time_gemm_bwd_wgrad_f32(&yin, n, d, f->groups, f->eps, f->gamma, f->beta, f->W, d, 1, ws->dS,
                                                     s == 3 ? (float)(h * B38[3]) : 1.f, s == 3 ? &apre : nullptr, ka[s],
                                                     f->groups > 0 ? ws->gpart : nullptr, f->groups > 0 ? ws->bpart : nullptr,
                                                     ws->wpart, stream));
            if (two) {
                GODE_HIP(hipEventRecord(ov->sp, hs));
                GODE_HIP(hipStreamWaitEvent(ov->side, ov->sp, 0));
            }
            GODE_TRY(gode_reduce_parts_f32(kt, ws->wpart, gode_bwd_wgrad_parts(n), nW, 1.f, 0, side));
            hipLaunchKernelGGL(theta_fixup_kernel, dim3(1), dim3(256), 0, (hipStream_t)side, kt, f->W, ts, (int)d, P - 1);
            GODE_LAUNCH_CHECK();
            if (f->groups > 0) {
                GODE_TRY(gode_reduce_parts2_f32(kt + nW + d, ws->gpart, kt + nW + 2 * d, ws->bpart, gparts, d, 1.f, 0, side));
            } else {
                GODE_TRY(gode_zero_f32(kt + nW + d, 2 * d, side));
            }
            if (two) { GODE_HIP(hipEventRecord(ov->wg, ov->side)); wg_pending = true; }
            if (g + 1 < total) {
                const int i2 = (g + 1) / 4, s2 = (g + 1) % 4;
                gode_lincomb_t yin2 = stage_terms(ycur_n, ky_n, s2, h);
                GODE_TRY(gode_gn_time_gemm_xout_f32(&yin2, n, d, f->groups, f->eps, f->gamma, f->beta, f->W, d, 1,
                                                    (float)((double)t0 + i2 * h + C38[s2] * h), Sbuf[(g + 1) & 1],
                                                    x_out_of(g + 1), stream));
                if (two) GODE_HIP(hipEventRecord(ov->gf, hs));
            }
            if (two) { GODE_HIP(hipStreamWaitEvent(hs, ov->wg, 0)); wg_pending = false; }
        } else {
        const bool merged = small;
        GODE_TRY(gode_wgrad_f32(&yin, n, d, f->groups, f->eps, f->gamma, f->beta, ws->dS, d, 1, ws->wpart, side));
        if (!merged) {
            GODE_TRY(gode_reduce_parts_f32(kt, ws->wpart, wparts, nW, 1.f, 0, side));
            hipLaunchKernelGGL(theta_fixup_kernel, dim3(1), dim3(256), 0, (hipStream_t)side, kt, f->W, ts, (int)d, P - 1);
            GODE_LAUNCH_CHECK();
        }
        if (two) { GODE_HIP(hipEventRecord(ov->wg, ov->side)); wg_pending = true; }
        if (g + 1 < total) {
            const int i2 = (g + 1) / 4, s2 = (g + 1) % 4;
            gode_lincomb_t yin2 = stage_terms(ycur_n, ky_n, s2, h);
            GODE_TRY(gode_gn_time_gemm_xout_f32(&yin2, n, d, f->groups, f->eps, f->gamma, f->beta, f->W, d, 1,
                                                (float)((double)t0 + i2 * h + C38[s2] * h), Sbuf[(g + 1) & 1],
                                                x_out_of(g + 1), side));
            if (two) GODE_HIP(hipEventRecord(ov->gf, ov->side));
        }
        GODE_TRY(gode_gn_time_gemm_bwd_f32(&yin, n, d, f->groups, f->eps, f->gamma, f->W, d, 1, ws->dS,
                                           s == 3 ? (float)(h * B38[3]) : 1.f, s == 3 ? &apre : nullptr, ka[s],
                                           f->groups > 0 ? ws->gpart : nullptr, f->groups > 0 ? ws->bpart : nullptr, stream));
        if (merged) {
            GODE_TRY(stage_finish_merged(f, ws, kt, ts, stream));
        } else {
            GODE_TRY(gode_colsum_f32(kt + nW, ws->dZ, n, d, 1.f, 0, ws->colsum_scratch, stream));
            if (f->groups > 0) {
                GODE_TRY(gode_reduce_parts2_f32(kt + nW + d, ws->gpart, kt + nW + 2 * d, ws->bpart, gparts, d, 1.f, 0, stream));
            } else {
                GODE_TRY(gode_zero_f32(kt + nW + d, 2 * d, stream));
            }
        }
        }
        if (s == 3) {
            if (two) { GODE_HIP(hipStreamWaitEvent(hs, ov->wg, 0)); wg_pending = false; }
            gode_lincomb_t tc;
            tc.n = 5; tc.coef[0] = 1.f; tc.ptr[0] = theta;
            for (int q = 0; q < 4; ++q) { tc.coef[1 + q] = (float)(h * B38[q]); tc.ptr[1 + q] = ws->ktheta[q]; }
            GODE_TRY(gode_lincomb_f32(theta, &tc, P, stream));
            float* tmp = ycur; ycur = ky[3]; ky[3] = tmp;
            tmp = acur; acur = ka[3]; ka[3] = tmp;
        }
    }
    if (two) {
        GODE_HIP(hipEventRecord(ov->gf, ov->side));
        GODE_HIP(hipStreamWaitEvent(hs, ov->gf, 0));
    }
    *y_result = ycur;
    *a_result = acur;
    return 0;
}

namespace {

const double DPC[7] = {0.0, 1.0 / 5, 3.0 / 10, 4.0 / 5, 8.0 / 9, 1.0, 1.0};
const double DPA[7][6] = {
    {0, 0, 0, 0, 0, 0},
    {1.0 / 5, 0, 0, 0, 0, 0},
    {3.0 / 40, 9.0 / 40, 0, 0, 0, 0},
    {44.0 / 45, -56.0 / 15, 32.0 / 9, 0, 0, 0},
    {19372.0 / 6561, -25360.0 / 2187, 64448.0 / 6561, -212.0 / 729, 0, 0},
    {9017.0 / 3168, -355.0 / 33, 46732.0 / 5247, 49.0 / 176, -5103.0 / 18656, 0},
    {35.0 / 384, 0, 500.0 / 1113, 125.0 / 192, -2187.0 / 6784, 11.0 / 84},
};
const double DPB[7] = {35.0 / 384, 0, 500.0 / 1113, 125.0 / 192, -2187.0 / 6784, 11.0 / 84, 0};
const double DPE[7] = {35.0 / 384 - 1951.0 / 21600, 0, 500.0 / 1113 - 22642.0 / 50085, 125.0 / 192 - 451.0 / 720,
                       -2187.0 / 6784 - -12231.0 / 42400, 11.0 / 84 - 649.0 / 6300, -1.0 / 60.0};

gode_lincomb_t dp_terms(const float* y, float* const* k, const double* coef, int count, double h, bool with_y) {
    gode_lincomb_t lc;
    lc.n = 0;
    if (with_y) { lc.coef[0] = 1.f; lc.ptr[0] = y; lc.n = 1; }
    for (int j = 0; j < count; ++j)
        if (coef[j] != 0.0) { lc.coef[lc.n] = (float)(h * coef[j]); lc.ptr[lc.n] = k[j]; ++lc.n; }
    return lc;
}

int dp_eval_forward(const gode_gcn_odefunc_t* f, const gode_rk4_workspace_t* ws, const gode_lincomb_t* yin, float t,
                    float* k_out, const gode_lincomb_t* next, float* x_next, void* stream) {
    if (fused_small(f)) return gode_gcn_feval_small_next_f32(f, yin, t, 1.f, nullptr, nullptr, nullptr, k_out, next, x_next, stream);
    GODE_TRY(gode_gn_time_gemm_f32(yin, f->n, f->d, f->groups, f->eps, f->gamma, f->beta, f->W, f->d, 1, t, ws->S, stream));
    gode_spmm_epilogue_t ep = {};
// ... 63 lines not shown
    gode_lincomb_t sol = dp_terms(y, k, DPB, 7, h, true);
    GODE_TRY(gode_lincomb_f32(y1, &sol, nd, stream));
    gode_lincomb_t err = dp_terms(nullptr, k, DPE, 7, h, false);
    return gode_rk_errnorm_f32(sums, y, y1, &err, rtol, atol, nd, err_scratch, stream);
}

extern "C" int gode_gcn_ode_dopri5_step_adjoint(const gode_gcn_odefunc_t* f, const float* y, const float* a,
                                                const float* theta, float* const* ky, float* const* ka,
                                                float* const* kth, float* y1, float* a1, float* theta1,
                                                const gode_rk4_workspace_t* ws, double t, double h, float rtol,
                                                float atol, double* sums , void* err_scratch, void* stream)
{
    if (!f || !y || !a || !theta || !ky || !ka || !kth || !y1 || !a1 || !theta1 || !ws || !sums || !err_scratch)
        return GODE_E_NULLPTR;
    if (f->n <= 0 || f->d <= 0) return GODE_E_SHAPE;
    for (int s = 0; s < 7; ++s) if (!ky[s] || !ka[s] || !kth[s]) return GODE_E_NULLPTR;
    if (!ws->S || !ws->dZ || !ws->dS || !ws->wpart || !ws->colsum_scratch) return GODE_E_NULLPTR;
    if (f->groups > 0 && (!ws->gpart || !ws->bpart)) return GODE_E_NULLPTR;
    const int64_t nd = f->n * f->d, P = gode_gcn_ode_theta_len(f->d);
    const bool fused = fused_small(f) && ws->small_part;
    const bool chain = fused && ws->X[0] && ws->X[1];
    for (int s = 1; s < 7; ++s) {
        gode_lincomb_t yin = dp_terms(y, ky, DPA[s], s, h, true);
        if (chain && s >= 2) { yin.n = 1; yin.coef[0] = 1.f; yin.ptr[0] = ws->X[s & 1]; }
        gode_lincomb_t ain = dp_terms(a, ka, DPA[s], s, h, true);
        gode_lincomb_t nxt; nxt.n = 0;
        if (chain && s < 6) nxt = dp_terms(y, ky, DPA[s + 1], s + 1, h, true);
        GODE_TRY(dp_eval_adjoint(f, ws, yin, ain, (float)(t + DPC[s] * h), ky[s], ka[s], kth[s], nxt.n > 0 ? &nxt : nullptr,
                                 nxt.n > 0 ? ws->X[(s + 1) & 1] : nullptr, fused ? s - 1 : -1, stream));
    }
    if (fused) {
        float* kout[6]; float tsv[6];
        for (int s = 1; s < 7; ++s) { kout[s - 1] = kth[s]; tsv[s - 1] = (float)(t + DPC[s] * h); }
        GODE_TRY(gode_gcn_small_finish_multi_f32(f, ws->small_part, 6, kout, tsv, stream));
    }
    gode_lincomb_t sy = dp_terms(y, ky, DPB, 7, h, true), sa = dp_terms(a, ka, DPB, 7, h, true),
                   st = dp_terms(theta, kth, DPB, 7, h, true);
    {
        float* outs[3] = {y1, a1, theta1};
        const gode_lincomb_t sols[3] = {sy, sa, st};
        const int64_t lens[3] = {nd, nd, P};
        GODE_TRY(gode_lincomb_multi_f32(outs, sols, lens, 3, stream));
    }
    gode_lincomb_t ey = dp_terms(nullptr, ky, DPE, 7, h, false), ea = dp_terms(nullptr, ka, DPE, 7, h, false),
                   et = dp_terms(nullptr, kth, DPE, 7, h, false);
    gode_lincomb_t et_at = et;
    for (int j = 0; j < et_at.n; ++j) et_at.ptr[j] = et.ptr[j] + (P - 1);
    const float* e0[4] = {y, a, theta + (P - 1), theta};
    const float* e1[4] = {y1, a1, theta1 + (P - 1), theta1};
    const gode_lincomb_t errs[4] = {ey, ea, et_at, et};
    const int64_t ens[4] = {nd, nd, 1, P - 1};
    return gode_rk_errnorm_multi_f32(sums, e0, e1, errs, ens, 4, rtol, atol, err_scratch, stream);
}

namespace {

int spmm_save(const gode_graph_t& g, const float* X, float* Y, int64_t d, const gode_spmm_epilogue_t* ep, float* K, void* s) {
    return gode_spmm_csr_save_f32(g.rowptr, g.col, g.val, g.items, g.n_items, g.long_rows, g.n_long, g.partial,
                                  X, d, Y, d, g.n_rows, d, ep, K, s);
}

gode_lincomb_t stage_cotangent(const float* abar, float* const* ybar, int s, double h) {
    gode_lincomb_t lc;
    lc.n = 0;
    lc.coef[lc.n] = (float)(h * B38[s]); lc.ptr[lc.n] = abar; ++lc.n;
    for (int q = s + 1; q < 4; ++q)
        if (A38[q][s] != 0.0) { lc.coef[lc.n] = (float)(h * A38[q][s]); lc.ptr[lc.n] = ybar[q]; ++lc.n; }
    return lc;
}

}

extern "C" int gode_gcn_ode_rk4_forward_save(const gode_gcn_odefunc_t* f, const float* y0, float* y_end, float* save,
                                             const gode_rk4_workspace_t* ws, float t0, float t1, int32_t n_steps,
                                             int32_t step_begin, int32_t step_end, void* stream)
{
    if (!f || !y0 || !y_end || !save || !ws) return GODE_E_NULLPTR;
    if (n_steps <= 0 || f->n <= 0 || f->d <= 0) return GODE_E_SHAPE;
    if (step_begin < 0 || step_end > n_steps || step_begin >= step_end) return GODE_E_SHAPE;
    if (!ws->S) return GODE_E_NULLPTR;
    const int64_t n = f->n, d = f->d, nd = n * d;
    const double h = ((double)t1 - (double)t0) / n_steps;
    const bool fused = fused_small(f);
    if (y0 != save) {
        gode_lincomb_t c; c.n = 1; c.coef[0] = 1.f; c.ptr[0] = y0;
        GODE_TRY(gode_lincomb_f32(save, &c, nd, stream));
    }
    for (int i = step_begin; i < step_end; ++i) {
        float* rec = save + (int64_t)(i - step_begin) * 5 * nd;
        const float* y = rec;
        float* k[4] = {rec + nd, rec + 2 * nd, rec + 3 * nd, rec + 4 * nd};
        float* ynext = (i + 1 < step_end) ? rec + 5 * nd : y_end;
        const double t = (double)t0 + i * h;
        for (int s = 0; s < 4; ++s) {
            gode_lincomb_t xin = stage_terms(y, k, s, h);
            const float ts = (float)(t + C38[s] * h);
            if (fused) {
                if (s < 3) {
                    GODE_TRY(gode_gcn_feval_small_f32(f, &xin, ts, 1.f, nullptr, nullptr, nullptr, k[s], stream));
                } else {
                    gode_lincomb_t pre = combine_terms(y, k, h);
                    GODE_TRY(gode_gcn_feval_small_save_f32(f, &xin, ts, (float)(h * B38[3]), &pre, ynext, k[3], stream));
                }
                continue;
            }
            GODE_TRY(gode_gn_time_gemm_f32(&xin, n, d, f->groups, f->eps, f->gamma, f->beta, f->W, d, 1, ts, ws->S, stream));
            gode_spmm_epilogue_t ep = {};
            ep.bias = f->b; ep.relu = 1; ep.alpha = 1.f;
            if (s < 3) {
                GODE_TRY(spmm(f->A, ws->S, k[s], d, &ep, stream));
            } else {
                ep.pre = combine_terms(y, k, h); ep.alpha = (float)(h * B38[3]);
                GODE_TRY(spmm_save(f->A, ws->S, ynext, d, &ep, k[3], stream));
            }
        }
    }
    return 0;
}

extern "C" int gode_gcn_ode_rk4_backprop(const gode_gcn_odefunc_t* f, const float* save, float* a, float* theta,
                                         float** a_result, const gode_rk4_workspace_t* ws, float* cot_colpart,
                                         float t0, float t1, int32_t n_steps, int32_t step_begin, int32_t step_end,
                                         void* stream)
{
    if (!f || !save || !a || !theta || !a_result || !ws) return GODE_E_NULLPTR;
    if (n_steps <= 0 || f->n <= 0 || f->d <= 0) return GODE_E_SHAPE;
    if (step_begin < 0 || step_end > n_steps || step_begin >= step_end) return GODE_E_SHAPE;
    for (int s = 0; s < 4; ++s) if (!ws->ka[s] || !ws->ktheta[s]) return GODE_E_NULLPTR;
    if (!ws->dZ || !ws->dS || !ws->wpart || !ws->colsum_scratch) return GODE_E_NULLPTR;
    if (f->groups > 0 && (!ws->gpart || !ws->bpart)) return GODE_E_NULLPTR;
    const int64_t n = f->n, d = f->d, nd = n * d;
    const int64_t nW = (d + 1) * d, P = gode_gcn_ode_theta_len(d);
    const double h = ((double)t1 - (double)t0) / n_steps;
    float* acur = a;
    float* yb[4] = {ws->ka[0], ws->ka[1], ws->ka[2], ws->ka[3]};
    auto record = [&](int i) { return save + (int64_t)(i - step_begin) * 5 * nd; };
    const bool fused = fused_small(f) && ws->small_part != nullptr;
    if (fused) {
        const int64_t slot = gode_gcn_small_parts(n) * gode_gcn_small_part_len(d);
        float* dz[2] = {ws->dZ, ws->dS};
        int cur = 0;
        {
            const float* r = record(step_end - 1);
            const gode_lincomb_t c4 = stage_cotangent(acur, yb, 3, h);
            GODE_TRY(gode_masked_cot_f32(&c4, r + 4 * nd, dz[0], n, d, nullptr, stream));
        }
        for (int i = step_end - 1; i >= step_begin; --i) {
            const float* y = record(i);
            float* k[4] = {(float*)y + nd, (float*)y + 2 * nd, (float*)y + 3 * nd, (float*)y + 4 * nd};
            const double t = (double)t0 + i * h;
            float stage_t[4];
            for (int s = 3; s >= 0; --s) {
                stage_t[s] = (float)(t + C38[s] * h);
                const gode_lincomb_t yin = stage_terms(y, k, s, h);
                gode_lincomb_t pre; pre.n = 0;
                if (s == 0) {
                    pre.n = 4;
                    pre.coef[0] = 1.f; pre.ptr[0] = acur;
                    for (int q = 1; q < 4; ++q) { pre.coef[q] = 1.f; pre.ptr[q] = yb[q]; }
                }
                gode_lincomb_t nxt; nxt.n = 0;
                const float* knext = nullptr;
                if (s > 0) {
                    nxt = stage_cotangent(acur, yb, s - 1, h);
                    knext = k[s - 1];
                } else if (i > step_begin) {
                    nxt.n = 1; nxt.coef[0] = (float)(h * B38[3]); nxt.ptr[0] = yb[0];
                    knext = record(i - 1) + 4 * nd;
                }
                float* part = ws->small_part + s * slot;
                if (knext) {
                    GODE_TRY(gode_gcn_vjp_small_next_f32(f, &yin, dz[cur], 1.f, s == 0 ? &pre : nullptr, yb[s], part,
                                                         &nxt, knext, dz[cur ^ 1], stream));
                    cur ^= 1;
                } else {
                    GODE_TRY(gode_gcn_vjp_small_f32(f, &yin, dz[cur], 1.f, s == 0 ? &pre : nullptr, yb[s], part, stream));
                }
            }
            const float w1[4] = {1.f, 1.f, 1.f, 1.f};
            GODE_TRY(gode_gcn_small_finish4_f32(f, ws->small_part, theta, w1, stage_t, stream));
            float* tmp = acur; acur = yb[0]; yb[0] = tmp;
        }
        *a_result = acur;
        return 0;
    }
    const bool small = n <= kMergedFinishMaxRows;
    const int64_t wparts = gode_wgrad_parts(n), gparts = gode_gemm_bwd_parts(n);
    const bool bw = !small && gode_bwd_wgrad_supported(n, d, d, f->groups) && gode_bwd_wgrad_parts(n) <= wparts;
    const int64_t cparts = (!small && cot_colpart) ? gode_masked_cot_parts(n, d) : 0;
    for (int i = step_end - 1; i >= step_begin; --i) {
        const float* y = record(i);
        float* k[4] = {(float*)y + nd, (float*)y + 2 * nd, (float*)y + 3 * nd, (float*)y + 4 * nd};
        const double t = (double)t0 + i * h;
        for (int s = 3; s >= 0; --s) {
            const float ts = (float)(t + C38[s] * h);
// ... 48 lines not shown
```

### graph_odenet_amd/csrc/options.h

```cpp
#pragma once
int gode_opt_gemm_split();
int gode_opt_overlap();
int gode_opt_wgrad_split();
int gode_opt_wgrad_split_small();
int gode_opt_bwd_pc();
int gode_opt_fwd_pc();
int gode_opt_small_fused();
int gode_opt_bwd_wgrad();
int gode_opt_y2_colsum();
```

### graph_odenet_amd/csrc/spmm.hip

```cpp
#include "common.h"
#include "prof.h"

namespace {

struct Epilogue {
    const float* bias;
    int relu;
    float alpha;
    LinComb pre;
    LinComb cot;
    float* Y2;
    float* colpart;
    int64_t colpart_row0;
    float* K;
};

template <int LPR>
__device__ __forceinline__ float4 epilogue_store4(const Epilogue& ep, float4 z, int row, int lane,
                                                  int64_t d, float* Y, int64_t ldy) {
    if (ep.bias) {
        const float4 b = *reinterpret_cast<const float4*>(ep.bias + lane * 4);
        z.x += b.x; z.y += b.y; z.z += b.z; z.w += b.w;
    }
    float4 y = z;
    if (ep.relu) { y.x = fmaxf(z.x, 0.f); y.y = fmaxf(z.y, 0.f); y.z = fmaxf(z.z, 0.f); y.w = fmaxf(z.w, 0.f); }
    if (ep.K) *reinterpret_cast<float4*>(ep.K + (int64_t)row * d + lane * 4) = y;
    if (ep.pre.n > 0) {
        const float4 p = lc_load4(ep.pre, (int64_t)row * d + lane * 4);
        y.x = fmaf(ep.alpha, y.x, p.x); y.y = fmaf(ep.alpha, y.y, p.y);
        y.z = fmaf(ep.alpha, y.z, p.z); y.w = fmaf(ep.alpha, y.w, p.w);
    } else if (ep.alpha != 1.f) {
        y.x *= ep.alpha; y.y *= ep.alpha; y.z *= ep.alpha; y.w *= ep.alpha;
    }
    *reinterpret_cast<float4*>(Y + (int64_t)row * ldy + lane * 4) = y;
    if (ep.Y2) {
        const int64_t o = (int64_t)row * d + lane * 4;
        float4 g = lc_load4(ep.cot, o);
        g.x = z.x > 0.f ? g.x : 0.f; g.y = z.y > 0.f ? g.y : 0.f;
        g.z = z.z > 0.f ? g.z : 0.f; g.w = z.w > 0.f ? g.w : 0.f;
        *reinterpret_cast<float4*>(ep.Y2 + o) = g;
        return g;
    }
    return make_float4(0.f, 0.f, 0.f, 0.f);
}

template <int LPR>
__device__ __forceinline__ void block_colsum_store(const float4 g, float* __restrict__ colpart_row) {
    __shared__ float4 cs[256];
    cs[threadIdx.x] = g;
    __syncthreads();
    if (threadIdx.x < LPR) {
        float4 t = cs[threadIdx.x];
#pragma unroll
        for (int r = 1; r < 256 / LPR; ++r) {
            const float4 a = cs[r * LPR + threadIdx.x];
            t.x += a.x; t.y += a.y; t.z += a.z; t.w += a.w;
        }
        *reinterpret_cast<float4*>(colpart_row + 4 * threadIdx.x) = t;
    }
}

template <int LPR>
__global__ __launch_bounds__(256) void spmm_vec4_kernel(
    const int* __restrict__ rowptr, const int* __restrict__ col, const float* __restrict__ val,
    const int4* __restrict__ items, int n_items, float* __restrict__ partial,
    const float* __restrict__ X, int64_t ldx, float* __restrict__ Y, int64_t ldy, Epilogue ep)
{
    constexpr int U = 4;
    const int64_t tid = (int64_t)blockIdx.x * blockDim.x + threadIdx.x;
    const int gid = (int)(tid / LPR);
    const int lane = threadIdx.x & (LPR - 1);
    const bool active = gid < n_items;
    int row = 0, b = 0, e = 0, slot = -1;
    if (active) {
        if (items) { const int4 it = items[gid]; row = it.x; b = it.y; e = it.z; slot = it.w; }
        else { row = gid; b = rowptr[gid]; e = rowptr[gid + 1]; }
    }
    const int len = e - b;
    float4 acc = make_float4(0.f, 0.f, 0.f, 0.f);
    const float* Xl = X + lane * 4;

    for (int base = 0; __any(base < len); base += LPR) {
        int c = 0; float v = 0.f;
        if (base + lane < len) {
            c = col[b + base + lane];
            v = val ? val[b + base + lane] : 1.f;
        }
        const int cnt = len - base;
        for (int k = 0; k < LPR; k += U) {
            if (!__any(k < cnt)) break;
            int cc[U]; float vv[U]; float4 xv[U];
#pragma unroll
            for (int u = 0; u < U; ++u) {
                cc[u] = __shfl(c, k + u, LPR);
                vv[u] = __shfl(v, k + u, LPR);
            }
#pragma unroll
            for (int u = 0; u < U; ++u) {
                xv[u] = make_float4(0.f, 0.f, 0.f, 0.f);
                if (k + u < cnt && k + u < LPR)
                    xv[u] = *reinterpret_cast<const float4*>(Xl + (int64_t)cc[u] * ldx);
            }
#pragma unroll
            for (int u = 0; u < U; ++u) {
                acc.x = fmaf(vv[u], xv[u].x, acc.x); acc.y = fmaf(vv[u], xv[u].y, acc.y);
                acc.z = fmaf(vv[u], xv[u].z, acc.z); acc.w = fmaf(vv[u], xv[u].w, acc.w);
            }
        }
    }
    if (ep.colpart) {
        float4 g = make_float4(0.f, 0.f, 0.f, 0.f);
        if (active) {
            if (slot < 0) g = epilogue_store4<LPR>(ep, acc, row, lane, (int64_t)LPR * 4, Y, ldy);
            else *reinterpret_cast<float4*>(partial + (int64_t)slot * (LPR * 4) + lane * 4) = acc;
        }
        block_colsum_store<LPR>(g, ep.colpart + (int64_t)blockIdx.x * (LPR * 4));
        return;
    }
    if (!active) return;
    if (slot < 0) epilogue_store4<LPR>(ep, acc, row, lane, (int64_t)LPR * 4, Y, ldy);
    else *reinterpret_cast<float4*>(partial + (int64_t)slot * (LPR * 4) + lane * 4) = acc;
}

template <int LPR>
__global__ __launch_bounds__(256) void spmm_vec4_wave_kernel(
    const int* __restrict__ rowptr, const int* __restrict__ col, const float* __restrict__ val,
    const int4* __restrict__ items, int n_items, float* __restrict__ partial,
    const float* __restrict__ X, int64_t ldx, float* __restrict__ Y, int64_t ldy, Epilogue ep)
{
    const int gid = (int)(((int64_t)blockIdx.x * blockDim.x + threadIdx.x) >> 6);
    const int wl = threadIdx.x & 63;
    const int lane = wl & (LPR - 1), sub = wl / LPR;
    if (gid >= n_items) return;
    int row, b, e, slot = -1;
    if (items) { const int4 it = items[gid]; row = it.x; b = it.y; e = it.z; slot = it.w; }
    else { row = gid; b = rowptr[gid]; e = rowptr[gid + 1]; }
    const int len = e - b;
    float4 acc = make_float4(0.f, 0.f, 0.f, 0.f);
    const float* Xl = X + lane * 4;
    for (int base = sub * LPR; base - sub * LPR < len; base += 64) {
        int c = 0; float v = 0.f;
        if (base + lane < len) {
            c = col[b + base + lane];
            v = val ? val[b + base + lane] : 1.f;
        }
        const int cnt = len - base;
        constexpr int U = LPR < 4 ? LPR : 4;
        for (int k = 0; k < LPR; k += U) {
            if (!__any(k < cnt)) break;
            int cc[U]; float vv[U]; float4 xv[U];
#pragma unroll
            for (int u = 0; u < U; ++u) { cc[u] = __shfl(c, k + u, LPR); vv[u] = __shfl(v, k + u, LPR); }
#pragma unroll
            for (int u = 0; u < U; ++u) {
                xv[u] = make_float4(0.f, 0.f, 0.f, 0.f);
                if (k + u < cnt) xv[u] = *reinterpret_cast<const float4*>(Xl + (int64_t)cc[u] * ldx);
            }
#pragma unroll
            for (int u = 0; u < U; ++u) {
                acc.x = fmaf(vv[u], xv[u].x, acc.x); acc.y = fmaf(vv[u], xv[u].y, acc.y);
                acc.z = fmaf(vv[u], xv[u].z, acc.z); acc.w = fmaf(vv[u], xv[u].w, acc.w);
            }
        }
    }
#pragma unroll
    for (int off = LPR; off < 64; off <<= 1) {
        acc.x += __shfl_xor(acc.x, off, 64); acc.y += __shfl_xor(acc.y, off, 64);
        acc.z += __shfl_xor(acc.z, off, 64); acc.w += __shfl_xor(acc.w, off, 64);
    }
    if (sub != 0) return;
    if (slot < 0) epilogue_store4<LPR>(ep, acc, row, lane, (int64_t)LPR * 4, Y, ldy);
    else *reinterpret_cast<float4*>(partial + (int64_t)slot * (LPR * 4) + lane * 4) = acc;
}

template <int LPR>
__global__ __launch_bounds__(256) void spmm_finish_vec4_kernel(
    const int4* __restrict__ long_rows, int n_long, const float* __restrict__ partial,
    float* __restrict__ Y, int64_t ldy, Epilogue ep)
{
    const int64_t tid = (int64_t)blockIdx.x * blockDim.x + threadIdx.x;
    const int gid = (int)(tid / LPR);
    const int lane = threadIdx.x & (LPR - 1);
    const bool active = gid < n_long;
    if (!active && !ep.colpart) return;
    const int4 lr = active ? long_rows[gid] : make_int4(0, 0, 0, 0);
    float4 acc = make_float4(0.f, 0.f, 0.f, 0.f);
    int s = lr.y;
    for (; s + 3 < lr.z; s += 4) {
        const float4 p0 = *reinterpret_cast<const float4*>(partial + (int64_t)s * (LPR * 4) + lane * 4);
        const float4 p1 = *reinterpret_cast<const float4*>(partial + (int64_t)(s + 1) * (LPR * 4) + lane * 4);
        const float4 p2 = *reinterpret_cast<const float4*>(partial + (int64_t)(s + 2) * (LPR * 4) + lane * 4);
        const float4 p3 = *reinterpret_cast<const float4*>(partial + (int64_t)(s + 3) * (LPR * 4) + lane * 4);
        acc.x += p0.x; acc.y += p0.y; acc.z += p0.z; acc.w += p0.w;
        acc.x += p1.x; acc.y += p1.y; acc.z += p1.z; acc.w += p1.w;
        acc.x += p2.x; acc.y += p2.y; acc.z += p2.z; acc.w += p2.w;
        acc.x += p3.x; acc.y += p3.y; acc.z += p3.z; acc.w += p3.w;
    }
    for (; s < lr.z; ++s) {
        const float4 p = *reinterpret_cast<const float4*>(partial + (int64_t)s * (LPR * 4) + lane * 4);
        acc.x += p.x; acc.y += p.y; acc.z += p.z; acc.w += p.w;
    }
    if (ep.colpart) {
        float4 g = make_float4(0.f, 0.f, 0.f, 0.f);
        if (active) g = epilogue_store4<LPR>(ep, acc, lr.x, lane, (int64_t)LPR * 4, Y, ldy);
        block_colsum_store<LPR>(g, ep.colpart + (ep.colpart_row0 + blockIdx.x) * (LPR * 4));
        return;
    }
    epilogue_store4<LPR>(ep, acc, lr.x, lane, (int64_t)LPR * 4, Y, ldy);
}

__device__ __forceinline__ void epilogue_store1(const Epilogue& ep, float z, int row, int c, int64_t d,
                                                float* Y, int64_t ldy) {
    if (ep.bias) z += ep.bias[c];
    float y = ep.relu ? fmaxf(z, 0.f) : z;
    if (ep.K) ep.K[(int64_t)row * d + c] = y;
    if (ep.pre.n > 0) y = fmaf(ep.alpha, y, lc_load1(ep.pre, (int64_t)row * d + c));
    else y *= ep.alpha;
    Y[(int64_t)row * ldy + c] = y;
    if (ep.Y2) {
        const int64_t o = (int64_t)row * d + c;
        const float g = lc_load1(ep.cot, o);
        ep.Y2[o] = z > 0.f ? g : 0.f;
    }
}

__global__ __launch_bounds__(256) void spmm_generic_kernel(
    const int* __restrict__ rowptr, const int* __restrict__ col, const float* __restrict__ val,
    const int4* __restrict__ items, int n_items, float* __restrict__ partial,
    const float* __restrict__ X, int64_t ldx, float* __restrict__ Y, int64_t ldy, int d, int G, Epilogue ep)
{
    const int64_t tid = (int64_t)blockIdx.x * blockDim.x + threadIdx.x;
    const int gid = (int)(tid / G);
    const int lane = threadIdx.x & (G - 1);
    if (gid >= n_items) return;
    int row, b, e, slot = -1;
    if (items) { const int4 it = items[gid]; row = it.x; b = it.y; e = it.z; slot = it.w; }
    else { row = gid; b = rowptr[gid]; e = rowptr[gid + 1]; }
    for (int c = lane; c < d; c += G) {
        float acc = 0.f;
        int j = b;
        for (; j + 4 <= e; j += 4) {
            const int c0 = col[j], c1 = col[j + 1], c2 = col[j + 2], c3 = col[j + 3];
            const float x0 = X[(int64_t)c0 * ldx + c], x1 = X[(int64_t)c1 * ldx + c], x2 = X[(int64_t)c2 * ldx + c],
                        x3 = X[(int64_t)c3 * ldx + c];
            float v0 = 1.f, v1 = 1.f, v2 = 1.f, v3 = 1.f;
            if (val) { v0 = val[j]; v1 = val[j + 1]; v2 = val[j + 2]; v3 = val[j + 3]; }
            acc = fmaf(v0, x0, acc); acc = fmaf(v1, x1, acc); acc = fmaf(v2, x2, acc); acc = fmaf(v3, x3, acc);
        }
        for (; j < e; ++j) {
            const float v = val ? val[j] : 1.f;
            acc = fmaf(v, X[(int64_t)col[j] * ldx + c], acc);
        }
        if (slot < 0) epilogue_store1(ep, acc, row, c, d, Y, ldy);
        else partial[(int64_t)slot * d + c] = acc;
    }
}

__global__ __launch_bounds__(256) void spmv_wave_kernel(
    const int* __restrict__ rowptr, const int* __restrict__ col, const float* __restrict__ val,
    const int4* __restrict__ items, int n_items, float* __restrict__ partial,
    const float* __restrict__ X, int64_t ldx, float* __restrict__ Y, int64_t ldy, Epilogue ep)
{
    const int gid = (int)(((int64_t)blockIdx.x * blockDim.x + threadIdx.x) >> 6);
    const int lane = threadIdx.x & 63;
    if (gid >= n_items) return;
    int row, b, e, slot = -1;
    if (items) { const int4 it = items[gid]; row = it.x; b = it.y; e = it.z; slot = it.w; }
    else { row = gid; b = rowptr[gid]; e = rowptr[gid + 1]; }
    float acc = 0.f;
    for (int j = b + lane; j < e; j += 64) acc = fmaf(val ? val[j] : 1.f, X[(int64_t)col[j] * ldx], acc);
    acc = wave_sum(acc);
    if (lane == 0) {
        if (slot < 0) epilogue_store1(ep, acc, row, 0, 1, Y, ldy);
        else partial[slot] = acc;
    }
}

__global__ __launch_bounds__(256) void spmm_finish_generic_kernel(
    const int4* __restrict__ long_rows, int n_long, const float* __restrict__ partial,
    float* __restrict__ Y, int64_t ldy, int d, int G, Epilogue ep)
{
    const int64_t tid = (int64_t)blockIdx.x * blockDim.x + threadIdx.x;
    const int gid = (int)(tid / G);
    const int lane = threadIdx.x & (G - 1);
    if (gid >= n_long) return;
    const int4 lr = long_rows[gid];
    for (int c = lane; c < d; c += G) {
        float acc = 0.f;
        for (int s = lr.y; s < lr.z; ++s) acc += partial[(int64_t)s * d + c];
        epilogue_store1(ep, acc, lr.x, c, d, Y, ldy);
    }
}

template <int LPR>
int launch_vec4(const int* rowptr, const int* col, const float* val, const int4* items, int n_items,
                const int4* long_rows, int n_long, float* partial, const float* X, int64_t ldx,
                float* Y, int64_t ldy, const Epilogue& ep, hipStream_t s) {
    if (LPR < 64 && n_items > 0 && n_items <= 65536) {
        if (ep.colpart) return GODE_E_UNSUPPORTED;
        const int64_t wb = ((int64_t)n_items * 64 + 255) / 256;
        const int slot = gode_prof_begin(s, (int64_t)LPR * 4, n_items, (int64_t)ep.pre.n + ep.cot.n + (ep.Y2 ? 1 : 0));
        hipLaunchKernelGGL(spmm_vec4_wave_kernel<LPR>, dim3((unsigned)wb), dim3(256), 0, s,
                           rowptr, col, val, items, n_items, partial, X, ldx, Y, ldy, ep);
        gode_prof_end(s, slot);
        GODE_LAUNCH_CHECK();
        if (n_long > 0) {
            const int64_t b2 = ((int64_t)n_long * LPR + 255) / 256;
            hipLaunchKernelGGL(spmm_finish_vec4_kernel<LPR>, dim3((unsigned)b2), dim3(256), 0, s,
                               long_rows, n_long, partial, Y, ldy, ep);
            GODE_LAUNCH_CHECK();
        }
        return 0;
    }
    const int64_t threads = (int64_t)n_items * LPR;
    const int64_t blocks = (threads + 255) / 256;
    if (blocks > 0) {
        const int slot = gode_prof_begin(s, (int64_t)LPR * 4, n_items, (int64_t)ep.pre.n + ep.cot.n + (ep.Y2 ? 1 : 0));
        hipLaunchKernelGGL(spmm_vec4_kernel<LPR>, dim3((unsigned)blocks), dim3(256), 0, s,
                           rowptr, col, val, items, n_items, partial, X, ldx, Y, ldy, ep);
        gode_prof_end(s, slot);
        GODE_LAUNCH_CHECK();
    }
    if (n_long > 0) {
        const int64_t b2 = ((int64_t)n_long * LPR + 255) / 256;
        Epilogue ep2 = ep;
        ep2.colpart_row0 = blocks;
        hipLaunchKernelGGL(spmm_finish_vec4_kernel<LPR>, dim3((unsigned)b2), dim3(256), 0, s,
                           long_rows, n_long, partial, Y, ldy, ep2);
        GODE_LAUNCH_CHECK();
    }
    return 0;
}

}

extern "C" int64_t gode_spmm_y2_colsum_rows(int64_t n_items, int64_t n_long, int64_t d)
{
    if (n_items <= 0 || n_long < 0 || d <= 0 || d % 4) return 0;
    const int64_t lpr = d / 4;
    if (lpr > 64 || (lpr & (lpr - 1))) return 0;
    if (lpr < 64 && n_items <= 65536) return 0;
    return (n_items * lpr + 255) / 256 + (n_long * lpr + 255) / 256;
}

namespace {

int spmm_csr_impl(const int32_t* rowptr, const int32_t* col, const float* val,
                  const int32_t* items, int64_t n_items,
                  const int32_t* long_rows, int64_t n_long, float* partial,
                  const float* X, int64_t ldx, float* Y, int64_t ldy,
                  int64_t n_rows, int64_t d,
                  const gode_spmm_epilogue_t* epi, float* K, void* stream)
{
    if (n_rows < 0 || d <= 0 || ldx < d || ldy < d) return GODE_E_SHAPE;
    if (n_rows == 0) return 0;
    if (!rowptr || !col || !X || !Y) return GODE_E_NULLPTR;
    if (n_rows > INT32_MAX || d > (1 << 20)) return GODE_E_RANGE;
    if (!items) { n_items = n_rows; n_long = 0; }
    if (n_items < 0 || n_items > INT32_MAX || n_long < 0 || n_long > INT32_MAX) return GODE_E_RANGE;
    if (n_long > 0 && (!long_rows || !partial)) return GODE_E_NULLPTR;
    if (n_items * 64 >= ((int64_t)1 << 32)) return GODE_E_RANGE;
    const float* bias = epi ? epi->bias : nullptr;
    float* Y2 = epi ? epi->Y2 : nullptr;
    const gode_lincomb_t* cot = (epi && Y2) ? &epi->cot : nullptr;
    const gode_lincomb_t* pre = (epi && epi->pre.n > 0) ? &epi->pre : nullptr;
    if (Y2) { int rc = check_lincomb(cot, true); if (rc) return rc; }
    if (pre) { int rc = check_lincomb(pre, true); if (rc) return rc; }
    hipStream_t s = (hipStream_t)stream;

    Epilogue ep;
    ep.bias = bias; ep.relu = epi ? epi->relu : 0; ep.alpha = epi ? epi->alpha : 1.f;
    ep.pre = make_lincomb(pre); ep.cot = make_lincomb(cot); ep.Y2 = Y2;
    ep.colpart = (epi && Y2) ? epi->Y2_colsum : nullptr; ep.colpart_row0 = 0;
    ep.K = K;
    if (ep.colpart && ((((uintptr_t)ep.colpart) & 15) || gode_spmm_y2_colsum_rows(n_items, n_long, d) == 0)) return GODE_E_UNSUPPORTED;

    const bool al = !(((uintptr_t)X) & 15) && !(((uintptr_t)Y) & 15) && (ldx % 4 == 0) && (ldy % 4 == 0) &&
                    (!bias || !(((uintptr_t)bias) & 15)) && (!partial || !(((uintptr_t)partial) & 15)) &&
                    (!Y2 || (!(((uintptr_t)Y2) & 15) && lincomb_aligned16(cot))) && lincomb_aligned16(pre) &&
                    !(((uintptr_t)K) & 15);
    const int4* it4 = reinterpret_cast<const int4*>(items);
    const int4* lr4 = reinterpret_cast<const int4*>(long_rows);
    if (al && d % 4 == 0) {
        switch (d / 4) {
#define GODE_CASE(L) case L: return launch_vec4<L>(rowptr, col, val, it4, (int)n_items, lr4, (int)n_long, partial, X, ldx, Y, ldy, ep, s);
            GODE_CASE(1) GODE_CASE(2) GODE_CASE(4) GODE_CASE(8) GODE_CASE(16) GODE_CASE(32) GODE_CASE(64)
#undef GODE_CASE
            default: break;
        }
    }
    if (ep.colpart) return GODE_E_UNSUPPORTED;
    int G = 1; while (G < d && G < 64) G <<= 1;
    if (d == 1 && it4 != nullptr) {
        const int64_t blocks = ((int64_t)n_items * 64 + 255) / 256;
        const int slot = gode_prof_begin(s, 1, n_items, (int64_t)ep.pre.n + ep.cot.n + (ep.Y2 ? 1 : 0));
        hipLaunchKernelGGL(spmv_wave_kernel, dim3((unsigned)blocks), dim3(256), 0, s,
                           rowptr, col, val, it4, (int)n_items, partial, X, ldx, Y, ldy, ep);
        gode_prof_end(s, slot);
        GODE_LAUNCH_CHECK();
    } else {
        const int64_t blocks = ((int64_t)n_items * G + 255) / 256;
        hipLaunchKernelGGL(spmm_generic_kernel, dim3((unsigned)blocks), dim3(256), 0, s,
                           rowptr, col, val, it4, (int)n_items, partial, X, ldx, Y, ldy, (int)d, G, ep);
        GODE_LAUNCH_CHECK();
    }
    if (n_long > 0) {
        const int64_t b2 = ((int64_t)n_long * G + 255) / 256;
        hipLaunchKernelGGL(spmm_finish_generic_kernel, dim3((unsigned)b2), dim3(256), 0, s,
                           lr4, (int)n_long, partial, Y, ldy, (int)d, G, ep);
        GODE_LAUNCH_CHECK();
    }
    return 0;
}

}

extern "C" int gode_spmm_csr_f32(const int32_t* rowptr, const int32_t* col, const float* val,
                                 const int32_t* items, int64_t n_items,
                                 const int32_t* long_rows, int64_t n_long, float* partial,
                                 const float* X, int64_t ldx, float* Y, int64_t ldy,
                                 int64_t n_rows, int64_t d,
                                 const gode_spmm_epilogue_t* epi, void* stream)
{
    return spmm_csr_impl(rowptr, col, val, items, n_items, long_rows, n_long, partial, X, ldx, Y, ldy, n_rows, d, epi,
                         nullptr, stream);
}

extern "C" int gode_spmm_csr_save_f32(const int32_t* rowptr, const int32_t* col, const float* val,
                                      const int32_t* items, int64_t n_items,
                                      const int32_t* long_rows, int64_t n_long, float* partial,
                                      const float* X, int64_t ldx, float* Y, int64_t ldy,
                                      int64_t n_rows, int64_t d,
                                      const gode_spmm_epilogue_t* epi, float* K, void* stream)
{
    if (n_rows < 0 || d <= 0 || ldx < d || ldy < d) return GODE_E_SHAPE;
    if (n_rows > 0 && !K) return GODE_E_NULLPTR;
    return spmm_csr_impl(rowptr, col, val, items, n_items, long_rows, n_long, partial, X, ldx, Y, ldy, n_rows, d, epi,
                         K, stream);
}
```

### graph_odenet_amd/ops.py

```python
import ctypes

import torch

from . import _lib
from ._lib import check, lincomb, ptr, stream_ptr


def _need(t, name, dtype=torch.float32):
    if t is None:
        return
    if not t.is_cuda:
        raise RuntimeError("graph_odenet_amd: %s must live on the GPU (got %s); there is no CPU path" % (name, t.device))
    if t.dtype != dtype:
        raise TypeError("graph_odenet_amd: %s must be %s, got %s" % (name, dtype, t.dtype))
    if not t.is_contiguous():
        raise ValueError("graph_odenet_amd: %s must be contiguous" % name)


def _need_terms(terms, name):
    n = None
    for c, t in terms:
        _need(t, name)
        if n is None:
            n = t.numel()
        elif t.numel() != n:
            raise ValueError("graph_odenet_amd: %s terms differ in size" % name)
    return n


def spmm(graph, X, bias=None, relu=False, out=None, cot_terms=None, out2=None, pre_terms=None, alpha=1.0, out2_colsum=None):
    lib = _lib.load()
    _need(X, "X")
    _need(bias, "bias")
    if getattr(graph, "is_partitioned", False):
        if X.dim() != 2 or X.shape[0] != graph.n_cols:
            raise ValueError("spmm: X has shape %s, this rank owns %d rows" % (tuple(X.shape), graph.n_cols))
        X, graph = graph.gather(X), graph.local
    if X.dim() != 2 or X.shape[0] != graph.n_cols:
        raise ValueError("spmm: X has shape %s, graph is %d x %d" % (tuple(X.shape), graph.n_rows, graph.n_cols))
    d = X.shape[1]
    if bias is not None and bias.numel() != d:
        raise ValueError("spmm: bias has %d elements, expected %d" % (bias.numel(), d))
    ldy = d
    if out is None:
        out = torch.empty(graph.n_rows, d, dtype=torch.float32, device=X.device)
    else:
        if tuple(out.shape) != (graph.n_rows, d):
            raise ValueError("spmm: out has wrong shape")
        if out.is_contiguous():
            _need(out, "out")
        else:
            if not out.is_cuda or out.dtype != torch.float32 or out.stride(1) != 1 or out.stride(0) < d:
                raise ValueError("spmm: out must be contiguous or a unit-stride column block of a row-major matrix")
            ldy = out.stride(0)
    ep = None
    if bias is not None or relu or cot_terms is not None or pre_terms is not None or alpha != 1.0:
        ep = _lib.SpmmEpilogue()
        ep.bias = bias.data_ptr() if bias is not None else None
        ep.relu = 1 if relu else 0
        ep.alpha = float(alpha)
        if pre_terms is not None:
            if _need_terms(pre_terms, "pre") != graph.n_rows * d:
                raise ValueError("spmm: pre terms have wrong size")
            ep.pre = lincomb(pre_terms)
        if cot_terms is not None:
            if _need_terms(cot_terms, "cot") != graph.n_rows * d:
                raise ValueError("spmm: cotangent terms have wrong size")
            ep.cot = lincomb(cot_terms)
            if out2 is None:
                out2 = torch.empty(graph.n_rows, d, dtype=torch.float32, device=X.device)
            _need(out2, "out2")
            ep.Y2 = out2.data_ptr()
            if out2_colsum is not None:
                _need(out2_colsum, "out2_colsum")
                if out2_colsum.numel() != spmm_y2_colsum_rows(graph, d) * d or out2_colsum.numel() == 0:
                    raise ValueError("spmm: out2_colsum must be spmm_y2_colsum_rows(graph, d) x d (and the shape must support it)")
                ep.Y2_colsum = out2_colsum.data_ptr()
    partial = graph.partial(d)
    rc = lib.gode_spmm_csr_f32(ptr(graph.rowptr), ptr(graph.col), ptr(graph.val),
                               ptr(graph.items), graph.n_items,
                               ptr(graph.long_rows), graph.n_long, ptr(partial),
                               ptr(X), d, ptr(out), ldy, graph.n_rows, d,
                               ctypes.byref(ep) if ep is not None else None, stream_ptr())
    check(rc, "gode_spmm_csr_f32")
    return (out, out2) if cot_terms is not None else out


def spmm_y2_colsum_rows(graph, d):
    return int(_lib.load().gode_spmm_y2_colsum_rows(graph.n_items if graph.items is not None else graph.n_rows, graph.n_long, int(d)))


def lincomb_(out, terms):
    lib = _lib.load()
    _need(out, "out")
    if _need_terms(terms, "lincomb") != out.numel():
        raise ValueError("lincomb: size mismatch")
    lc = lincomb(terms)
    check(lib.gode_lincomb_f32(ptr(out), ctypes.byref(lc), out.numel(), stream_ptr()), "gode_lincomb_f32")
    return out


def lincomb_multi_(outs, terms_list):
    lib = _lib.load()
    k = len(outs)
    if k != len(terms_list) or not 1 <= k <= 4:
        raise ValueError("lincomb_multi: one term list per output, at most four")
    lcs = (_lib.LinComb * k)()
    ptrs = (ctypes.c_void_p * k)()
    ns = (ctypes.c_int64 * k)()
    for c, (out, terms) in enumerate(zip(outs, terms_list)):
        _need(out, "out")
        if _need_terms(terms, "lincomb") != out.numel():
            raise ValueError("lincomb_multi: size mismatch in component %d" % c)
        lcs[c] = lincomb(terms)
        ptrs[c] = out.data_ptr()
        ns[c] = out.numel()
    check(lib.gode_lincomb_multi_f32(ptrs, lcs, ns, k, stream_ptr()), "gode_lincomb_multi_f32")
    return outs


_red_scratch = {}
_retired = []


def _scratch(device, nbytes):
    key = (device, _lib.current_stream_handle(device.index if device.index is not None else torch.cuda.current_device()))
    buf = _red_scratch.get(key)
    if buf is None or buf.numel() < nbytes:
        if buf is not None:
            _retired.append(buf)
        buf = torch.empty(max(nbytes, 1 << 20), dtype=torch.uint8, device=device)
        _red_scratch[key] = buf
    return buf


def rk_error_sumsq(y0, y1, err_terms, rtol, atol, out=None):
    lib = _lib.load()
    _need(y0, "y0"); _need(y1, "y1")
    n = y0.numel()
    if _need_terms(err_terms, "err") != n or y1.numel() != n:
        raise ValueError("rk_error_sumsq: size mismatch")
    if out is None:
        out = torch.empty(1, dtype=torch.float64, device=y0.device)
    sc = _scratch(y0.device, lib.gode_rk_errnorm_scratch_bytes())
    lc = lincomb(err_terms)
    check(lib.gode_rk_errnorm_f32(ptr(out), ptr(y0), ptr(y1), ctypes.byref(lc), float(rtol), float(atol), n,
                                  ptr(sc), stream_ptr()), "gode_rk_errnorm_f32")
    return out


def rk_scaled_sumsq(terms, y, rtol, atol, out=None):
    lib = _lib.load()
    _need(y, "y")
    n = y.numel()
    if _need_terms(terms, "terms") != n:
        raise ValueError("rk_scaled_sumsq: size mismatch")
    if out is None:
        out = torch.empty(1, dtype=torch.float64, device=y.device)
    sc = _scratch(y.device, lib.gode_rk_errnorm_scratch_bytes())
    lc = lincomb(terms)
    check(lib.gode_rk_scaled_sumsq_f32(ptr(out), ctypes.byref(lc), ptr(y), float(rtol), float(atol), n,
                                       ptr(sc), stream_ptr()), "gode_rk_scaled_sumsq_f32")
    return out


def gn_time_gemm(x_terms, n_rows, d_in, groups, eps, gamma, beta, W, has_time, t, out=None, x_out=None):
    lib = _lib.load()
    _need(W, "W"); _need(gamma, "gamma"); _need(beta, "beta")
    if _need_terms(x_terms, "x") != n_rows * d_in:
        raise ValueError("gn_time_gemm: x terms have wrong size")
    if W.dim() != 2 or W.shape[0] != d_in + (1 if has_time else 0):
        raise ValueError("gn_time_gemm: W has shape %s" % (tuple(W.shape),))
    d_out = W.shape[1]
    if out is None:
        out = torch.empty(n_rows, d_out, dtype=torch.float32, device=W.device)
    _need(out, "out")
    lc = lincomb(x_terms)
    if x_out is not None:
        _need(x_out, "x_out")
        if x_out.numel() != n_rows * d_in:
            raise ValueError("gn_time_gemm: x_out has wrong size")
    check(lib.gode_gn_time_gemm_xout_f32(ctypes.byref(lc), n_rows, d_in, groups, float(eps), ptr(gamma), ptr(beta),
                                         ptr(W), d_out, 1 if has_time else 0, float(t), ptr(out), ptr(x_out),
                                         stream_ptr()), "gode_gn_time_gemm_xout_f32")
    return out


def gn_time_gemm_pair(x_terms, n_rows, d, groups, eps, gamma, beta, Wa, Wb, has_time, t, out_a, out_b, x_out=None):
    lib = _lib.load()
    for tns, nm in ((Wa, "Wa"), (Wb, "Wb"), (gamma, "gamma"), (beta, "beta"), (out_a, "out_a"), (out_b, "out_b"), (x_out, "x_out")):
        _need(tns, nm)
    if _need_terms(x_terms, "x") != n_rows * d:
        raise ValueError("gn_time_gemm_pair: x terms have wrong size")
    k = d + (1 if has_time else 0)
    if tuple(Wa.shape) != (k, d) or tuple(Wb.shape) != (k, d) or out_a.numel() != n_rows * d or out_b.numel() != n_rows * d:
        raise ValueError("gn_time_gemm_pair: weights must be (%d, %d) and outputs n x d" % (k, d))
    lc = lincomb(x_terms)
    check(lib.gode_gn_time_gemm_pair_f32(ctypes.byref(lc), n_rows, d, groups, float(eps), ptr(gamma), ptr(beta), ptr(Wa), ptr(Wb),
                                         1 if has_time else 0, float(t), ptr(out_a), ptr(out_b), ptr(x_out), stream_ptr()),
          "gode_gn_time_gemm_pair_f32")


def gat_small_supported(n_rows, d, groups, heads=1):
    lib = _lib.load()
    return bool(lib.gode_get_option(b"small_fused")) and bool(lib.gode_gat_small_supported(n_rows, d, groups, heads))


def gat_small_part(n_rows, d, heads, device):
    lib = _lib.load()
    return torch.empty(lib.gode_gat_small_parts(n_rows, d), lib.gode_gat_small_part_len(d, heads), dtype=torch.float32, device=device)


def gat_small_pack(Wsrc, Wtgt, Wlog, heads, out=None):
    lib = _lib.load()
    _need(Wsrc, "Wsrc"); _need(Wtgt, "Wtgt"); _need(Wlog, "Wlog"); _need(out, "packed")
    d = Wsrc.shape[1]
    n = lib.gode_gat_small_pack_len(d, heads)
    if out is None:
        out = torch.empty(n, dtype=torch.float32, device=Wsrc.device)
    elif out.numel() != n:
        raise ValueError("gat_small_pack: packed buffer must hold %d floats" % n)
    check(lib.gode_gat_small_pack_f32(ptr(Wsrc), ptr(Wtgt), ptr(Wlog), d, heads, ptr(out), stream_ptr()), "gode_gat_small_pack_f32")
    return out


def gat_project_small(x_terms, n_rows, d, groups, eps, gamma, beta, Wsrc, Wtgt, Wlog, heads, pt_bias, t, Ps, Pt, A2, x_out=None,
                      packed=None):
    lib = _lib.load()
    for tns, nm in ((gamma, "gamma"), (beta, "beta"), (Wsrc, "Wsrc"), (Wtgt, "Wtgt"), (Wlog, "Wlog"), (pt_bias, "pt_bias"),
                    (Ps, "Ps"), (Pt, "Pt"), (A2, "A2"), (x_out, "x_out")):
        _need(tns, nm)
    if _need_terms(x_terms, "x") != n_rows * d:
        raise ValueError("gat_project_small: x terms have wrong size")
    if tuple(Wsrc.shape) != (d + 1, d) or tuple(Wtgt.shape) != (d + 1, d) or tuple(Wlog.shape) != (d + 1, 2 * heads):
        raise ValueError("gat_project_small: weights must be (d+1) x d, (d+1) x d, (d+1) x 2H")
    if Ps.numel() != n_rows * d or Pt.numel() != n_rows * d or A2.numel() != n_rows * 2 * heads or \
            (x_out is not None and x_out.numel() != n_rows * d) or (pt_bias is not None and pt_bias.numel() != d):
        raise ValueError("gat_project_small: output buffers have wrong size")
    lc = lincomb(x_terms)
    check(lib.gode_gat_project_small_f32(ctypes.byref(lc), n_rows, d, groups, float(eps), ptr(gamma), ptr(beta), ptr(Wsrc), ptr(Wtgt),
                                         ptr(Wlog), heads, ptr(pt_bias), float(t), ptr(Ps), ptr(Pt), ptr(A2), ptr(x_out),
                                         ptr(packed), stream_ptr()), "gode_gat_project_small_f32")


def gat_dense_vjp_small(x_terms, n_rows, d, groups, eps, gamma, beta, Wsrc, Wtgt, Wlog, heads, dPs, dPt, dA2, ka, part,
                        out_scale=1.0, pre_terms=None, maxfix=None, packed=None):
    lib = _lib.load()
    for tns, nm in ((gamma, "gamma"), (beta, "beta"), (Wsrc, "Wsrc"), (Wtgt, "Wtgt"), (Wlog, "Wlog"), (dPs, "dPs"), (dPt, "dPt"),
                    (dA2, "dA2"), (ka, "ka"), (part, "part")):
        _need(tns, nm)
    if _need_terms(x_terms, "x") != n_rows * d:
        raise ValueError("gat_dense_vjp_small: x terms have wrong size")
    if tuple(Wsrc.shape) != (d + 1, d) or tuple(Wtgt.shape) != (d + 1, d) or tuple(Wlog.shape) != (d + 1, 2 * heads):
        raise ValueError("gat_dense_vjp_small: weights must be (d+1) x d, (d+1) x d, (d+1) x 2H")
    if dPs.numel() != n_rows * d or dPt.numel() != n_rows * d or dA2.numel() != n_rows * 2 * heads or ka.numel() != n_rows * d or \
            part.numel() != lib.gode_gat_small_parts(n_rows, d) * lib.gode_gat_small_part_len(d, heads):
        raise ValueError("gat_dense_vjp_small: buffers have wrong size")
    lc = lincomb(x_terms)
    pre = None
    if pre_terms:
        if _need_terms(pre_terms, "pre") != n_rows * d:
            raise ValueError("gat_dense_vjp_small: pre terms have wrong size")
        pre = lincomb(pre_terms)
    check(lib.gode_gat_dense_vjp_small_f32(ctypes.byref(lc), n_rows, d, groups, float(eps), ptr(gamma), ptr(beta), ptr(Wsrc), ptr(Wtgt),
# ... 822 lines not shown
```

### include/graphode.h

```cpp
#ifndef GRAPHODE_H
#define GRAPHODE_H

#include <stdint.h>

#ifdef __cplusplus
extern "C" {
#endif

#define GODE_ABI_VERSION 1

#define GODE_E_NULLPTR  (-1)
#define GODE_E_SHAPE    (-2)
#define GODE_E_ALIGN    (-3)
#define GODE_E_RANGE    (-4)
#define GODE_E_UNSUPPORTED (-5)

#define GODE_MAX_TERMS 8

typedef struct gode_lincomb {
    int32_t      n;
    float        coef[GODE_MAX_TERMS];
    const float* ptr[GODE_MAX_TERMS];
} gode_lincomb_t;

int         gode_abi_version(void);
int         gode_set_option(const char* name, int value);
int         gode_get_option(const char* name);
const char* gode_error_string(int code);

typedef struct gode_spmm_epilogue {
    const float*   bias;
    int32_t        relu;
    float          alpha;
    gode_lincomb_t pre;
    gode_lincomb_t cot;
    float*         Y2;
    float*         Y2_colsum;
} gode_spmm_epilogue_t;

int64_t gode_spmm_y2_colsum_rows(int64_t n_items, int64_t n_long, int64_t d);

int gode_spmm_csr_f32(const int32_t* rowptr, const int32_t* col, const float* val,
                      const int32_t* items, int64_t n_items,
                      const int32_t* long_rows, int64_t n_long, float* partial,
                      const float* X, int64_t ldx, float* Y, int64_t ldy,
                      int64_t n_rows, int64_t d,
                      const gode_spmm_epilogue_t* epi ,
                      void* stream);
int gode_spmm_csr_save_f32(const int32_t* rowptr, const int32_t* col, const float* val,
                           const int32_t* items, int64_t n_items,
                           const int32_t* long_rows, int64_t n_long, float* partial,
                           const float* X, int64_t ldx, float* Y, int64_t ldy,
                           int64_t n_rows, int64_t d,
                           const gode_spmm_epilogue_t* epi , float* K,
                           void* stream);

int64_t gode_masked_cot_parts(int64_t n_rows, int64_t d);
int gode_masked_cot_f32(const gode_lincomb_t* cot , const float* k, float* dZ, int64_t n_rows, int64_t d,
                        float* colpart , void* stream);

int gode_lincomb_f32(float* out, const gode_lincomb_t* lc , int64_t n, void* stream);
int gode_lincomb_multi_f32(float* const* outs , const gode_lincomb_t* lcs ,
                           const int64_t* ns , int32_t count, void* stream);

int64_t gode_rk_errnorm_scratch_bytes(void);
int gode_rk_errnorm_f32(double* out, const float* y0, const float* y1,
                        const gode_lincomb_t* elc , float rtol, float atol,
                        int64_t n, void* scratch, void* stream);
int gode_rk_errnorm_multi_f32(double* out, const float* const* y0 , const float* const* y1,
                              const gode_lincomb_t* elcs , const int64_t* ns, int32_t count, float rtol,
                              float atol, void* scratch, void* stream);

int gode_rk_scaled_sumsq_f32(double* out, const gode_lincomb_t* lc , const float* y,
                             float rtol, float atol, int64_t n, void* scratch, void* stream);

int gode_gn_time_gemm_f32(const gode_lincomb_t* xin , int64_t n_rows, int64_t d_in,
                          int32_t groups, float eps, const float* gamma, const float* beta,
                          const float* W, int64_t d_out, int has_time, float t,
                          float* S, void* stream);
int gode_gn_time_gemm_xout_f32(const gode_lincomb_t* xin , int64_t n_rows, int64_t d_in,
                               int32_t groups, float eps, const float* gamma, const float* beta,
                               const float* W, int64_t d_out, int has_time, float t,
                               float* S, float* x_out, void* stream);

int gode_gn_time_gemm_pair_f32(const gode_lincomb_t* xin , int64_t n_rows, int64_t d, int32_t groups, float eps,
                               const float* gamma, const float* beta, const float* Wa, const float* Wb,
                               int has_time, float t, float* Sa, float* Sb, float* x_out, void* stream);

int64_t gode_gemm_bwd_parts(int64_t n_rows);
int gode_gn_time_gemm_bwd_f32(const gode_lincomb_t* xin , int64_t n_rows, int64_t d_in,
                              int32_t groups, float eps, const float* gamma,
                              const float* W, int64_t d_out, int has_time,
                              const float* dS, float out_scale,
                              const gode_lincomb_t* pre , float* dx,
                              float* dgamma_part, float* dbeta_part, void* stream);

int gode_bwd_wgrad_supported(int64_t n_rows, int64_t d_in, int64_t d_out, int32_t groups);
int64_t gode_bwd_wgrad_parts(int64_t n_rows);
int gode_gn_time_gemm_bwd_wgrad_f32(const gode_lincomb_t* xin , int64_t n_rows, int64_t d_in, int32_t groups,
                                    float eps, const float* gamma, const float* beta, const float* W, int64_t d_out,
                                    int has_time, const float* dS, float out_scale, const gode_lincomb_t* pre ,
                                    float* dx, float* dgamma_part, float* dbeta_part, float* dW_part, void* stream);

#define GODE_MAX_REDUCE_SEGS 8
typedef struct gode_reduce_seg {
    float* out; const float* part;
    int64_t n_part, ld, col0, col_stride, len;
    const float* w_row0; int64_t time_len;
} gode_reduce_seg_t;
int gode_reduce_segments_f32(const gode_reduce_seg_t* segs, int32_t n_segs, float t, float* at , void* stream);
int gode_colsum_parts_f32(const float* X, int64_t n_rows, int64_t d, float* scratch, int64_t* n_parts , void* stream);

int64_t gode_group_norm_parts(int64_t n_rows);
int gode_group_norm_f32_fwd(const float* x, int64_t n_rows, int64_t d, int32_t groups, float eps,
                            const float* gamma , const float* beta , float* y, void* stream);
int gode_group_norm_f32_bwd(const float* x, int64_t n_rows, int64_t d, int32_t groups, float eps,
                            const float* gamma , const float* dy, float* dx,
                            float* dgamma_part , float* dbeta_part , void* stream);

int64_t gode_wgrad_parts(int64_t n_rows);
int gode_wgrad_f32(const gode_lincomb_t* xin , int64_t n_rows, int64_t d_in,
                   int32_t groups, float eps, const float* gamma, const float* beta,
                   const float* dS, int64_t d_out, int has_time,
                   float* dW_part, void* stream);

int gode_rect_gemm_f32(const float* X, int64_t ldx, int64_t n_rows, int64_t K, const float* W, int64_t M,
                       float* S, int64_t lds, void* stream);
int gode_rect_gemm_nt_f32(const float* dS, int64_t ldds, int64_t n_rows, int64_t M, const float* W, int64_t K,
                          float* dX, int64_t lddx, void* stream);
int64_t gode_rect_wgrad_parts(int64_t n_rows);
int gode_rect_wgrad_f32(const float* X, int64_t ldx, int64_t n_rows, int64_t K, const float* dS, int64_t ldds,
                        int64_t M, float* part, void* stream);
int gode_rect_wgrad_sum_f32(const float* X, int64_t ldx, int64_t n_rows, int64_t K, const float* dS, int64_t ldds, int64_t M,
                            float* part, float* dW, void* stream);

int gode_gemm_f32(int trans_a, int trans_b, int64_t M, int64_t N, int64_t K, const float* A, int64_t lda,
                  const float* B, int64_t ldb, float* C, int64_t ldc, const float* bias, int relu,
                  const float* mask, int64_t ldmask, void* stream);
int64_t gode_gemm_splitk_parts(int64_t M, int64_t N, int64_t K);
int gode_gemm_splitk_f32(int trans_a, int trans_b, int64_t M, int64_t N, int64_t K, const float* A, int64_t lda,
                         const float* B, int64_t ldb, float* part, float* C , void* stream);

int64_t gode_cut_pad(int64_t n);
int gode_cut_bf16x3_f32(const float* X, int64_t ld, int64_t R, int64_t C, void* planes, void* stream);
int64_t gode_pgemm_workspace_bytes(int64_t M, int64_t N, int64_t K);
int gode_pgemm_bf16x3(int trans_a, int trans_b, int64_t M, int64_t N, int64_t K, const void* A_planes,
                      const void* B_planes, float* C, int64_t ldc, const float* bias, int relu,
                      const float* mask, int64_t ldmask, int products, void* workspace, void* stream);

#define GODE_ADAM_MAX_TENSORS 64
typedef struct gode_adam_args {
    float*       param[GODE_ADAM_MAX_TENSORS];
    const float* grad[GODE_ADAM_MAX_TENSORS];
    float*       exp_avg[GODE_ADAM_MAX_TENSORS];
    float*       exp_avg_sq[GODE_ADAM_MAX_TENSORS];
    int64_t      len[GODE_ADAM_MAX_TENSORS];
} gode_adam_args_t;
int64_t gode_adam_chunk(void);
int gode_adam_tick_f32(float* state, float beta1, float beta2, void* stream);
int gode_adam_f32(const gode_adam_args_t* args , int32_t n_tensors, const void* chunks, int64_t n_chunks,
                  const float* state, float lr, float beta1, float beta2, float eps, float weight_decay, void* stream);

int gode_reduce_parts_f32(float* out, const float* part, int64_t n_part, int64_t len,
                          float scale, int accumulate, void* stream);
int gode_reduce_parts2_f32(float* out_a, const float* part_a, float* out_b, const float* part_b,
                           int64_t n_part, int64_t len, float scale, int accumulate, void* stream);
// ... 274 lines not shown
```

Before: 3.924 steps/s.

## Fuse RK step closing linear combination into GEMM and SpMM epilogues

Adds an auxiliary output to the fused group-norm/GEMM forward kernel and a third output to the SpMM cotangent epilogue. Each one computes a second linear combination of the same input terms with different coefficients, so the RK step's final combination (the state or adjoint update) is written while the stage inputs are already in registers. This removes a separate lincomb pass that would re-read all stage buffers from memory, at the cost of extra register pressure and an extra store stream in already heavy kernels. A new rk_close_once option, on by default, gates its use in the solver.

Result: faster. 4.042 steps/s, median of 6 (+3.0%).

```diff
diff --git a/graph_odenet_amd/_lib.py b/graph_odenet_amd/_lib.py
--- a/graph_odenet_amd/_lib.py
+++ b/graph_odenet_amd/_lib.py
@@ -17,7 +17,8 @@
 
 class SpmmEpilogue(ctypes.Structure):
     _fields_ = [("bias", ctypes.c_void_p), ("relu", ctypes.c_int32), ("alpha", ctypes.c_float),
-                ("pre", LinComb), ("cot", LinComb), ("Y2", ctypes.c_void_p), ("Y2_colsum", ctypes.c_void_p)]
+                ("pre", LinComb), ("cot", LinComb), ("Y2", ctypes.c_void_p), ("Y2_colsum", ctypes.c_void_p),
+                ("cot_out", ctypes.c_void_p), ("cot_out_coef", ctypes.c_float * GODE_MAX_TERMS)]
 
 
 class Graph(ctypes.Structure):
@@ -103,6 +104,8 @@
                                     c_p, c_i64, c_i, c_f, c_p, c_p]),
     "gode_gn_time_gemm_xout_f32": (c_i, [ctypes.POINTER(LinComb), c_i64, c_i64, ctypes.c_int32, c_f, c_p, c_p,
                                          c_p, c_i64, c_i, c_f, c_p, c_p, c_p]),
+    "gode_gn_time_gemm_xout_aux_f32": (c_i, [ctypes.POINTER(LinComb), c_i64, c_i64, ctypes.c_int32, c_f, c_p, c_p,
+                                             c_p, c_i64, c_i, c_f, c_p, c_p, c_p, c_p, c_p]),
     "gode_gn_time_gemm_pair_f32": (c_i, [ctypes.POINTER(LinComb), c_i64, c_i64, ctypes.c_int32, c_f, c_p, c_p, c_p, c_p,
                                          c_i, c_f, c_p, c_p, c_p, c_p]),
     "gode_gemm_bwd_parts": (c_i64, [c_i64]),
diff --git a/graph_odenet_amd/csrc/api.hip b/graph_odenet_amd/csrc/api.hip
--- a/graph_odenet_amd/csrc/api.hip
+++ b/graph_odenet_amd/csrc/api.hip
@@ -22,7 +22,7 @@
 
 namespace {
 int env_int(const char* name, int dflt) { const char* e = getenv(name); return e ? atoi(e) : dflt; }
-int g_gemm_split = -1, g_overlap = -1, g_wgrad_split = -1, g_wgrad_split_small = 0, g_bwd_pc = -1, g_fwd_pc = -1, g_small_fused = -1, g_bwd_wgrad = -1, g_y2_colsum = -1;
+int g_gemm_split = -1, g_overlap = -1, g_wgrad_split = -1, g_wgrad_split_small = 0, g_bwd_pc = -1, g_fwd_pc = -1, g_small_fused = -1, g_bwd_wgrad = -1, g_y2_colsum = -1, g_rk_close_once = -1;
 }
 
 int gode_opt_gemm_split() { if (g_gemm_split < 0) { const int v = env_int("GODE_GEMM_SPLIT", 2); g_gemm_split = (v == 1 || v == 2) ? v : 0; } return g_gemm_split; }
@@ -36,6 +36,7 @@
 int gode_opt_small_fused() { if (g_small_fused < 0) g_small_fused = env_int("GODE_SMALL_FUSED", 1) != 0; return g_small_fused; }
 int gode_opt_bwd_wgrad() { if (g_bwd_wgrad < 0) g_bwd_wgrad = env_int("GODE_BWD_WGRAD", 1) != 0; return g_bwd_wgrad; }
 int gode_opt_y2_colsum() { if (g_y2_colsum < 0) g_y2_colsum = env_int("GODE_Y2_COLSUM", 1) != 0; return g_y2_colsum; }
+int gode_opt_rk_close_once() { if (g_rk_close_once < 0) g_rk_close_once = env_int("GODE_RK_CLOSE_ONCE", 1) != 0; return g_rk_close_once; }
 int gode_opt_overlap() { if (g_overlap < 0) g_overlap = env_int("GODE_OVERLAP", 1) != 0; return g_overlap; }
 
 extern "C" int gode_set_option(const char* name, int value) {
@@ -47,6 +48,7 @@
     if (!strcmp(name, "small_fused")) { g_small_fused = value != 0; return 0; }
     if (!strcmp(name, "bwd_wgrad")) { g_bwd_wgrad = value != 0; return 0; }
     if (!strcmp(name, "y2_colsum")) { g_y2_colsum = value != 0; return 0; }
+    if (!strcmp(name, "rk_close_once")) { g_rk_close_once = value != 0; return 0; }
     if (!strcmp(name, "fwd_pc")) { if (value < 0 || value > 3) return GODE_E_UNSUPPORTED; g_fwd_pc = value; return 0; }
     if (!strcmp(name, "wgrad_split")) { if (value != 0 && value != 6 && value != 8) return GODE_E_UNSUPPORTED; g_wgrad_split = value; return 0; }
     return GODE_E_UNSUPPORTED;
@@ -61,6 +63,7 @@
     if (!strcmp(name, "small_fused")) return gode_opt_small_fused();
     if (!strcmp(name, "bwd_wgrad")) return gode_opt_bwd_wgrad();
     if (!strcmp(name, "y2_colsum")) return gode_opt_y2_colsum();
+    if (!strcmp(name, "rk_close_once")) return gode_opt_rk_close_once();
     if (!strcmp(name, "fwd_pc")) return gode_opt_fwd_pc();
     return GODE_E_UNSUPPORTED;
 }
diff --git a/graph_odenet_amd/csrc/common.h b/graph_odenet_amd/csrc/common.h
--- a/graph_odenet_amd/csrc/common.h
+++ b/graph_odenet_amd/csrc/common.h
@@ -65,6 +65,39 @@
     }
 }
 
+template <int NT>
+__device__ __forceinline__ void lc_load4_pair_n(const LinComb& lc, const float* coef2, int64_t idx, float4& r, float4& r2) {
+    float4 v[NT];
+#pragma unroll
+    for (int j = 0; j < NT; ++j) v[j] = *reinterpret_cast<const float4*>(lc.ptr[j] + idx);
+    r = make_float4(0.f, 0.f, 0.f, 0.f);
+    r2 = make_float4(0.f, 0.f, 0.f, 0.f);
+#pragma unroll
+    for (int j = 0; j < NT; ++j) {
+        const float c = lc.coef[j], c2 = coef2[j];
+        r.x = fmaf(c, v[j].x, r.x); r.y = fmaf(c, v[j].y, r.y);
+        r.z = fmaf(c, v[j].z, r.z); r.w = fmaf(c, v[j].w, r.w);
+        r2.x = fmaf(c2, v[j].x, r2.x); r2.y = fmaf(c2, v[j].y, r2.y);
+        r2.z = fmaf(c2, v[j].z, r2.z); r2.w = fmaf(c2, v[j].w, r2.w);
+    }
+}
+
+__device__ __forceinline__ void lc_load4_pair(const LinComb& lc, const float* coef2, int64_t idx, float4& r, float4& r2) {
+    switch (lc.n) {
+        case 1: lc_load4_pair_n<1>(lc, coef2, idx, r, r2); break;
+        case 2: lc_load4_pair_n<2>(lc, coef2, idx, r, r2); break;
+        case 3: lc_load4_pair_n<3>(lc, coef2, idx, r, r2); break;
+        case 4: lc_load4_pair_n<4>(lc, coef2, idx, r, r2); break;
+        case 5: lc_load4_pair_n<5>(lc, coef2, idx, r, r2); break;
+        case 6: lc_load4_pair_n<6>(lc, coef2, idx, r, r2); break;
+        case 7: lc_load4_pair_n<7>(lc, coef2, idx, r, r2); break;
+        case 8: lc_load4_pair_n<8>(lc, coef2, idx, r, r2); break;
+        default: r = make_float4(0.f, 0.f, 0.f, 0.f); r2 = r; break;
+    }
+}
+
+struct AuxCoef { float c[GODE_MAX_TERMS]; };
+
 __device__ __forceinline__ float lc_load1(const LinComb& lc, int64_t idx) {
     float r = 0.f;
 #pragma unroll
diff --git a/graph_odenet_amd/csrc/dense_pc.h b/graph_odenet_amd/csrc/dense_pc.h
--- a/graph_odenet_amd/csrc/dense_pc.h
+++ b/graph_odenet_amd/csrc/dense_pc.h
@@ -2,7 +2,8 @@
 #include "common.h"
 
 int gode_pc_fwd_launch(const LinComb& lc, int64_t n_rows, float eps, const float* gamma, const float* beta,
-                       const float* W, int has_time, float t, float* S, float* xout, int cg, hipStream_t s);
+                       const float* W, int has_time, float t, float* S, float* xout, const float* aux_coef, float* aux,
+                       int cg, hipStream_t s);
 int gode_pc_bwd_launch(const LinComb& lc, int64_t n_rows, float eps, const float* gamma, const float* W, int has_time,
                        const float* dS, float out_scale, const LinComb& pre, float* dx, float* dgamma_part,
                        float* dbeta_part, int64_t n_part, int cg, hipStream_t s);
diff --git a/graph_odenet_amd/csrc/gemm.hip b/graph_odenet_amd/csrc/gemm.hip
--- a/graph_odenet_amd/csrc/gemm.hip
+++ b/graph_odenet_amd/csrc/gemm.hip
@@ -177,13 +177,14 @@
                        __int_as_float(__builtin_amdgcn_ds_bpermute(src_f_lane_x4, __float_as_int(a[3]))));
 }
 
-template <int NJ, int CG>
+template <int NJ, int CG, bool AUX = false>
 __global__ __launch_bounds__(256, 2) void gn_gemm_fwd_kernel(LinComb xin, int n_rows, float eps,
                                                              const float* __restrict__ gamma,
                                                              const float* __restrict__ beta,
                                                              const float* __restrict__ W, int has_time, float t,
                                                              float* __restrict__ S, float* __restrict__ xout,
-                                                             const float* __restrict__ W2, float* __restrict__ S2)
+                                                             const float* __restrict__ W2, float* __restrict__ S2,
+                                                             AuxCoef acoef, float* __restrict__ aux)
 {
     constexpr int D = 16 * NJ;
     constexpr int LDW = D + 4;
@@ -207,7 +208,26 @@
     int tile = blockIdx.x * 4 + wave;
     if (tile >= n_tiles) return;
     float4 nx[NJ];
-    load_tile<NJ, 2>(xin, (int64_t)(tile * 16 + mr) * D + 4 * mg, tile * 16 + mr < n_rows, nx);
+    LinComb xa = xin;
+    float4 na[NJ];
+    if (AUX) {
+#pragma unroll
+        for (int j = 0; j < GODE_MAX_TERMS; ++j) xa.coef[j] = acoef.c[j];
+        const int64_t base0 = (int64_t)(tile * 16 + mr) * D + 4 * mg;
+        const bool valid0 = tile * 16 + mr < n_rows;
+#pragma unroll
+        for (int j = 0; j < NJ; ++j) { nx[j] = make_float4(0.f, 0.f, 0.f, 0.f); na[j] = nx[j]; }
+        float4 v0[2][NJ];
+#pragma unroll
+        for (int t0 = 0; t0 < GODE_MAX_TERMS; t0 += 2)
+            if (t0 < xin.n) {
+                issue_terms2<NJ>(xin, t0, base0, valid0, v0);
+                fold_terms2<NJ>(xin, t0, valid0, v0, nx);
+                fold_terms2<NJ>(xa, t0, valid0, v0, na);
+            }
+    } else {
+        load_tile<NJ, 2>(xin, (int64_t)(tile * 16 + mr) * D + 4 * mg, tile * 16 + mr < n_rows, nx);
+    }
     for (; tile < n_tiles; tile += stride) {
         const int row = tile * 16 + mr;
         const bool valid = row < n_rows;
@@ -218,6 +238,10 @@
 #pragma unroll
         for (int j = 0; j < NJ; ++j) {
             if (xout != nullptr && valid) *reinterpret_cast<float4*>(xout + (int64_t)row * D + 16 * j + 4 * mg) = nx[j];
+            if (AUX) {
+                if (valid) *reinterpret_cast<float4*>(aux + (int64_t)row * D + 16 * j + 4 * mg) = na[j];
+                na[j] = make_float4(0.f, 0.f, 0.f, 0.f);
+            }
             xv[j] = gn_forward_v<CG>(nx[j], eps, ld4(Gs + 16 * j + 4 * mg), ld4(Bs + 16 * j + 4 * mg));
             xv[j] = to_mfma_layout(xv[j], to_f);
             nx[j] = make_float4(0.f, 0.f, 0.f, 0.f);
@@ -232,11 +256,13 @@
         issue_terms2<NJ>(xin, 0, nbase, nvalid, v);
         mfma_panel_part<NJ, 0, 2 * NJ>(Ws + 4 * g * LDW + r, xv, acc);
         fold_terms2<NJ>(xin, 0, nvalid, v, nx);
+        if (AUX) fold_terms2<NJ>(xa, 0, nvalid, v, na);
         issue_terms2<NJ>(xin, 2, nbase, nvalid, v);
         mfma_panel_part<NJ, 2 * NJ, 4 * NJ>(Ws + 4 * g * LDW + r, xv, acc);
         fold_terms2<NJ>(xin, 2, nvalid, v, nx);
-        if (xin.n > 4) { issue_terms2<NJ>(xin, 4, nbase, nvalid, v); fold_terms2<NJ>(xin, 4, nvalid, v, nx); }
-        if (xin.n > 6) { issue_terms2<NJ>(xin, 6, nbase, nvalid, v); fold_terms2<NJ>(xin, 6, nvalid, v, nx); }
+        if (AUX) fold_terms2<NJ>(xa, 2, nvalid, v, na);
+        if (xin.n > 4) { issue_terms2<NJ>(xin, 4, nbase, nvalid, v); fold_terms2<NJ>(xin, 4, nvalid, v, nx); if (AUX) fold_terms2<NJ>(xa, 4, nvalid, v, na); }
+        if (xin.n > 6) { issue_terms2<NJ>(xin, 6, nbase, nvalid, v); fold_terms2<NJ>(xin, 6, nvalid, v, nx); if (AUX) fold_terms2<NJ>(xa, 6, nvalid, v, na); }
 #pragma unroll
         for (int tt = 0; tt < NJ; ++tt) {
             const float4 o = acc_to_mem_layout(acc[tt], to_m);
@@ -1273,22 +1299,42 @@
                                           float eps, const float* gamma, const float* beta, const float* W,
                                           int64_t d_out, int has_time, float t, float* S, float* x_out, void* stream)
 {
+    return gode_gn_time_gemm_xout_aux_f32(xin, n_rows, d_in, groups, eps, gamma, beta, W, d_out, has_time, t, S, x_out,
+                                          nullptr, nullptr, stream);
+}
+
+extern "C" int gode_gn_time_gemm_xout_aux_f32(const gode_lincomb_t* xin, int64_t n_rows, int64_t d_in, int32_t groups,
+                                              float eps, const float* gamma, const float* beta, const float* W,
+                                              int64_t d_out, int has_time, float t, float* S, float* x_out,
+                                              const float* aux_coef, float* aux_out, void* stream)
+{
     int rc = check_common(xin, n_rows, d_in, groups, d_out); if (rc) return rc;
+    if (aux_out && !aux_coef) return GODE_E_NULLPTR;
     if (n_rows == 0) return 0;
     if (!W || !S) return GODE_E_NULLPTR;
     if (x_out && (((uintptr_t)x_out) & 15)) return GODE_E_ALIGN;
+    if (aux_out && (((uintptr_t)aux_out) & 15)) return GODE_E_ALIGN;
+    if (aux_out) {
+        if (aux_out == S || aux_out == x_out) return GODE_E_RANGE;
+        for (int j = 0; j < xin->n; ++j) if (aux_out == xin->ptr[j]) return GODE_E_RANGE;
+    }
     has_time = has_time ? 1 : 0;
     hipStream_t s = (hipStream_t)stream;
     LinComb lc = make_lincomb(xin);
+    AuxCoef ac;
+    for (int j = 0; j < GODE_MAX_TERMS; ++j) ac.c[j] = (aux_out && j < lc.n) ? aux_coef[j] : 0.f;
     const int cg = fast_cg(d_in, d_out, groups);
     const bool al = lincomb_aligned16(xin) && !(((uintptr_t)S) & 15) && !(((uintptr_t)W) & 15) &&
                     (!gamma || !(((uintptr_t)gamma) & 15)) && (!beta || !(((uintptr_t)beta) & 15));
+    if (aux_out && !(cg >= 0 && al && d_in == 128)) return GODE_E_UNSUPPORTED;
     if (cg >= 0 && al && d_in == 128 && (n_rows >= kWgradSplitMinRows || gode_opt_wgrad_split_small()) &&
         ((lc.n <= 2 && !x_out) ? (gode_opt_fwd_pc() & 1) : (gode_opt_fwd_pc() & 2))) {
-        rc = gode_pc_fwd_launch(lc, n_rows, eps, gamma, beta, W, has_time, t, S, x_out, cg, s);
+        rc = gode_pc_fwd_launch(lc, n_rows, eps, gamma, beta, W, has_time, t, S, x_out, aux_coef, aux_out, cg, s);
         if (rc != GODE_E_UNSUPPORTED) return rc;
+        if (aux_out && (cg == 0 || cg == 1 || cg == 2 || cg == 4)) return GODE_E_UNSUPPORTED;
     }
     if (cg >= 0 && al && d_in == 128 && !x_out && (gode_opt_gemm_split() == 1 || (gode_opt_gemm_split() == 2 && lc.n <= 2 && n_rows >= 65536))) {
+        if (aux_out) return GODE_E_UNSUPPORTED;
         const size_t lds = (size_t)3 * 128 * (128 + 8) * sizeof(unsigned short) + 3 * 128 * sizeof(float);
         int64_t blocks = ((n_rows + 15) / 16 + 7) / 8; if (blocks < 1) blocks = 1; if (blocks > 256) blocks = 256;
 #define GODE_FWDS2(CGV, NXV) { rc = set_lds(gn_gemm_fwd_split_kernel<CGV, NXV>, lds); if (rc) return rc;    \
@@ -1311,10 +1357,24 @@
           const int slot = gode_prof_begin(s, d_in, n_rows, (int64_t)lc.n - 1 + (x_out ? 1 : 0), GODE_PROF_GEMM_FWD); \
           hipLaunchKernelGGL((gn_gemm_fwd_kernel<NJV, CGV>), dim3((unsigned)blocks), dim3(256), lds, s, \
                              lc, (int)n_rows, eps, gamma, beta, W, has_time, t, S, x_out,           \
-                             (const float*)nullptr, (float*)nullptr);                               \
+                             (const float*)nullptr, (float*)nullptr, ac, (float*)nullptr);          \
           gode_prof_end(s, slot);                                                                   \
           GODE_LAUNCH_CHECK(); return 0; }
+#define GODE_FWDA(NJV, CGV)                                                                         \
+        { rc = set_lds(gn_gemm_fwd_kernel<NJV, CGV, true>, lds); if (rc) return rc;                 \
+          const int slot = gode_prof_begin(s, d_in, n_rows, (int64_t)lc.n - 1 + (x_out ? 1 : 0) + 1, GODE_PROF_GEMM_FWD); \
+          hipLaunchKernelGGL((gn_gemm_fwd_kernel<NJV, CGV, true>), dim3((unsigned)blocks), dim3(256), lds, s, \
+                             lc, (int)n_rows, eps, gamma, beta, W, has_time, t, S, x_out,           \
+                             (const float*)nullptr, (float*)nullptr, ac, aux_out);                  \
+          gode_prof_end(s, slot);                                                                   \
+          GODE_LAUNCH_CHECK(); return 0; }
+        if (aux_out) {
+            GODE_DISPATCH_NJ_CG(8, 0, GODE_FWDA) GODE_DISPATCH_NJ_CG(8, 1, GODE_FWDA)
+            GODE_DISPATCH_NJ_CG(8, 2, GODE_FWDA) GODE_DISPATCH_NJ_CG(8, 4, GODE_FWDA)
+            return GODE_E_UNSUPPORTED;
+        }
         GODE_DISPATCH_ALL(GODE_FWD)
+#undef GODE_FWDA
 #undef GODE_FWD
     }
     {
@@ -1361,7 +1421,7 @@
 #define GODE_FWDP(NJV, CGV)                                                                         \
         { rc = set_lds(gn_gemm_fwd_kernel<NJV, CGV>, lds); if (rc) return rc;                       \
           hipLaunchKernelGGL((gn_gemm_fwd_kernel<NJV, CGV>), dim3((unsigned)blocks, 2), dim3(256), lds, s, \
-                             lc, (int)n_rows, eps, gamma, beta, Wa, has_time, t, Sa, x_out, Wb, Sb);  \
+                             lc, (int)n_rows, eps, gamma, beta, Wa, has_time, t, Sa, x_out, Wb, Sb, AuxCoef(), (float*)nullptr);  \
           GODE_LAUNCH_CHECK(); return 0; }
         GODE_DISPATCH_ALL(GODE_FWDP)
 #undef GODE_FWDP
diff --git a/graph_odenet_amd/csrc/gemm_pc.hip b/graph_odenet_amd/csrc/gemm_pc.hip
--- a/graph_odenet_amd/csrc/gemm_pc.hip
+++ b/graph_odenet_amd/csrc/gemm_pc.hip
@@ -80,13 +80,15 @@
     __device__ int clamped(int k) const { return blockIdx.x + (k < mine ? k : (mine > 0 ? mine - 1 : 0)) * stride; }
 };
 
-template <int CG, int NX, bool XOUT, int R>
+template <int CG, int NX, bool XOUT, int R, bool AUX = false>
 __global__ __launch_bounds__(1024, 1) void gn_gemm_fwd_pc_kernel(LinComb xin, int n_rows, float eps,
                                                                 const float* __restrict__ gamma,
                                                                 const float* __restrict__ beta,
                                                                 const float* __restrict__ W, int has_time, float t,
-                                                                float* __restrict__ S, float* __restrict__ xout)
+                                                                float* __restrict__ S, float* __restrict__ xout,
+                                                                AuxCoef acoef, float* __restrict__ aux)
 {
+    static_assert(!AUX || NX > 0, "the second combination needs the raw terms");
     constexpr int PIECE_B = Img<R>::PIECE_B, BUF_B = Img<R>::BUF_B;
     constexpr int RPT = R / 8;
     extern __shared__ __attribute__((aligned(16))) float smem[];
@@ -130,6 +132,16 @@
                     }
                 }
                 if (XOUT && row < n_rows) *reinterpret_cast<float4*>(xout + (int64_t)row * D + tcol) = x;
+                if (AUX) {
+                    float4 a = make_float4(0.f, 0.f, 0.f, 0.f);
+#pragma unroll
+                    for (int j = 0; j < NXR; ++j) {
+                        const float c = acoef.c[j];
+                        a.x = fmaf(c, xr[j][p].x, a.x); a.y = fmaf(c, xr[j][p].y, a.y);
+                        a.z = fmaf(c, xr[j][p].z, a.z); a.w = fmaf(c, xr[j][p].w, a.w);
+                    }
+                    if (row < n_rows) *reinterpret_cast<float4*>(aux + (int64_t)row * D + tcol) = a;
+                }
                 float4 xn = gn_forward_v<CG>(x, eps, gmv, btv);
                 if (row >= n_rows) xn = make_float4(0.f, 0.f, 0.f, 0.f);
                 stage_row4<PIECE_B>(img + p * LDK * 2, xn);
@@ -557,25 +569,35 @@
 }
 
 int gode_pc_fwd_launch(const LinComb& lc, int64_t n_rows, float eps, const float* gamma, const float* beta,
-                       const float* W, int has_time, float t, float* S, float* xout, int cg, hipStream_t s)
+                       const float* W, int has_time, float t, float* S, float* xout, const float* aux_coef, float* aux,
+                       int cg, hipStream_t s)
 {
     int rc = 0;
-#define GODE_FPC4(CGV, NXV, XO, RV)                                                                               \
+    AuxCoef ac;
+    for (int j = 0; j < GODE_MAX_TERMS; ++j) ac.c[j] = (aux && j < lc.n) ? aux_coef[j] : 0.f;
+#define GODE_FPC5(CGV, NXV, XO, RV, AX)                                                                           \
     { const size_t lds = 2 * (size_t)Img<RV>::BUF_B;                                                               \
       const int64_t blocks = pc_blocks(n_rows, RV);                                                                \
-      rc = set_lds_pc(gn_gemm_fwd_pc_kernel<CGV, NXV, XO, RV>, lds); if (rc) return rc;                            \
-      const int slot = gode_prof_begin(s, D, n_rows, (int64_t)lc.n - 1 + (XO ? 1 : 0), GODE_PROF_GEMM_FWD | GODE_PROF_FORM_PC); \
-      hipLaunchKernelGGL((gn_gemm_fwd_pc_kernel<CGV, NXV, XO, RV>), dim3((unsigned)blocks), dim3(1024), lds, s,    \
-                         lc, (int)n_rows, eps, gamma, beta, W, has_time, t, S, xout);                             \
+      rc = set_lds_pc(gn_gemm_fwd_pc_kernel<CGV, NXV, XO, RV, AX>, lds); if (rc) return rc;                        \
+      const int slot = gode_prof_begin(s, D, n_rows, (int64_t)lc.n - 1 + (XO ? 1 : 0) + (AX ? 1 : 0), GODE_PROF_GEMM_FWD | GODE_PROF_FORM_PC); \
+      hipLaunchKernelGGL((gn_gemm_fwd_pc_kernel<CGV, NXV, XO, RV, AX>), dim3((unsigned)blocks), dim3(1024), lds, s, \
+                         lc, (int)n_rows, eps, gamma, beta, W, has_time, t, S, xout, ac, aux);                    \
       gode_prof_end(s, slot);                                                                                      \
       GODE_LAUNCH_CHECK(); return 0; }
-#define GODE_FPC2(CGV, NXV, RV) { if (xout) GODE_FPC4(CGV, NXV, true, RV) else GODE_FPC4(CGV, NXV, false, RV) }
+#define GODE_FPC2(CGV, NXV, RV) { if (xout) GODE_FPC5(CGV, NXV, true, RV, false) else GODE_FPC5(CGV, NXV, false, RV, false) }
 #define GODE_FPC(CGV) { switch (lc.n) { case 1: GODE_FPC2(CGV, 1, 32) case 2: GODE_FPC2(CGV, 2, 32) case 3: GODE_FPC2(CGV, 3, 32) \
                                         case 4: GODE_FPC2(CGV, 4, 32) default: GODE_FPC2(CGV, 0, 32) } }
+#define GODE_FPCA(CGV) { if (xout) GODE_FPC5(CGV, 4, true, 32, true) else GODE_FPC5(CGV, 4, false, 32, true) }
+    if (aux) {
+        if (lc.n != 4) return GODE_E_UNSUPPORTED;
+        if (cg == 0) GODE_FPCA(0) else if (cg == 1) GODE_FPCA(1) else if (cg == 2) GODE_FPCA(2) else if (cg == 4) GODE_FPCA(4)
+        return GODE_E_UNSUPPORTED;
+    }
     if (cg == 0) GODE_FPC(0) else if (cg == 1) GODE_FPC(1) else if (cg == 2) GODE_FPC(2) else if (cg == 4) GODE_FPC(4)
+#undef GODE_FPCA
 #undef GODE_FPC
 #undef GODE_FPC2
-#undef GODE_FPC4
+#undef GODE_FPC5
     return GODE_E_UNSUPPORTED;
 }
 
diff --git a/graph_odenet_amd/csrc/ode_driver.hip b/graph_odenet_amd/csrc/ode_driver.hip
--- a/graph_odenet_amd/csrc/ode_driver.hip
+++ b/graph_odenet_amd/csrc/ode_driver.hip
@@ -67,6 +67,25 @@
 }
 gode_lincomb_t negated(gode_lincomb_t lc) { for (int j = 0; j < lc.n; ++j) lc.coef[j] = -lc.coef[j]; return lc; }
 
+bool close_once_route(const gode_gcn_odefunc_t* f) {
+    return gode_opt_rk_close_once() && !fused_small(f) && f->n > kMergedFinishMaxRows && f->d == 128;
+}
+gode_lincomb_t one_term(const float* p) { gode_lincomb_t lc; lc.n = 1; lc.coef[0] = 1.f; lc.ptr[0] = p; return lc; }
+
+int gf_last_stage(const gode_gcn_odefunc_t* f, const float* y, float* const* k, double h, float t, float* S, float* x_out,
+                  float* p_out, bool* formed, void* stream) {
+    const gode_lincomb_t xin = stage_terms(y, k, 3, h), pre = combine_terms(y, k, h);
+    *formed = false;
+    bool distinct = p_out != S && p_out != x_out;
+    for (int j = 0; j < xin.n; ++j) distinct = distinct && p_out != xin.ptr[j];
+    if (distinct && xin.n == pre.n) {
+        const int rc = gode_gn_time_gemm_xout_aux_f32(&xin, f->n, f->d, f->groups, f->eps, f->gamma, f->beta, f->W, f->d, 1, t, S,
+                                                      x_out, pre.coef, p_out, stream);
+        if (rc != GODE_E_UNSUPPORTED) { *formed = rc == 0; return rc; }
+    }
+    return gode_gn_time_gemm_xout_f32(&xin, f->n, f->d, f->groups, f->eps, f->gamma, f->beta, f->W, f->d, 1, t, S, x_out, stream);
+}
+
 }
 
 extern "C" int64_t gode_gcn_ode_theta_len(int64_t d) { return (d + 1) * d + 3 * d + 1; }
@@ -83,6 +102,7 @@
     float* cur = y;
     float* k[4] = {ws->ky[0], ws->ky[1], ws->ky[2], ws->ky[3]};
     const bool fused = fused_small(f);
+    const bool close_once = close_once_route(f);
     for (int i = 0; i < n_steps; ++i) {
         const double t = (double)t0 + i * h;
         for (int s = 0; s < 4; ++s) {
@@ -93,11 +113,16 @@
                                                   s == 3 ? &pre : nullptr, nullptr, nullptr, k[s], stream));
                 continue;
             }
-            GODE_TRY(gode_gn_time_gemm_f32(&xin, n, d, f->groups, f->eps, f->gamma, f->beta, f->W, d, 1,
-                                           (float)(t + C38[s] * h), ws->S, stream));
+            bool p_formed = false;
+            if (s == 3 && close_once) {
+                GODE_TRY(gf_last_stage(f, cur, k, h, (float)(t + C38[s] * h), ws->S, nullptr, k[3], &p_formed, stream));
+            } else {
+                GODE_TRY(gode_gn_time_gemm_f32(&xin, n, d, f->groups, f->eps, f->gamma, f->beta, f->W, d, 1,
+                                               (float)(t + C38[s] * h), ws->S, stream));
+            }
             gode_spmm_epilogue_t ep = {};
             ep.bias = f->b; ep.relu = 1; ep.alpha = 1.f;
-            if (s == 3) { ep.pre = combine_terms(cur, k, h); ep.alpha = (float)(h * B38[3]); }
+            if (s == 3) { ep.pre = p_formed ? one_term(k[3]) : combine_terms(cur, k, h); ep.alpha = (float)(h * B38[3]); }
             GODE_TRY(spmm(f->A, ws->S, k[s], d, &ep, stream));
         }
         float* tmp = cur; cur = k[3]; k[3] = tmp;
@@ -171,6 +196,8 @@
         GODE_TRY(gode_gn_time_gemm_xout_f32(&yin0, n, d, f->groups, f->eps, f->gamma, f->beta, f->W, d, 1,
                                             (float)((double)t0), Sbuf[0], x_out_of(0), stream));
     }
+    const bool close_once = bw && close_once_route(f);
+    bool py_formed = false;
     bool wg_pending = false;
     float stage_t[4] = {0.f, 0.f, 0.f, 0.f};
     for (int g = 0; g < total; ++g) {
@@ -206,7 +233,17 @@
             ? gode_spmm_y2_colsum_rows(f->A.items ? f->A.n_items : f->A.n_rows, f->A.items ? f->A.n_long : 0, d) : 0;
         if (y2rows > 0) ep.Y2_colsum = ws->y2_colsum;
         gode_lincomb_t apre; apre.n = 0;
-        if (s == 3) { ep.pre = combine_terms(ycur, ky, h); ep.alpha = (float)(h * B38[3]); apre = combine_terms(acur, ka, h); }
+        if (s == 3) {
+            ep.pre = py_formed ? one_term(ky[3]) : combine_terms(ycur, ky, h);
+            ep.alpha = (float)(h * B38[3]);
+            apre = combine_terms(acur, ka, h);
+            if (close_once && ain.n == apre.n) {
+                ep.cot_out = ka[3];
+                for (int j = 0; j < apre.n; ++j) ep.cot_out_coef[j] = apre.coef[j];
+                apre = one_term(ka[3]);
+            }
+            py_formed = false;
+        }
         if (two && g > 0) GODE_HIP(hipStreamWaitEvent(hs, ov->gf, 0));
         GODE_TRY(spmm(f->A, Sbuf[g & 1], ky[s], d, &ep, stream));
         float* ycur_n = ycur; float* ky_n[4] = {ky[0], ky[1], ky[2], ky[3]};
@@ -242,9 +279,14 @@
             if (g + 1 < total) {
                 const int i2 = (g + 1) / 4, s2 = (g + 1) % 4;
                 gode_lincomb_t yin2 = stage_terms(ycur_n, ky_n, s2, h);
-                GODE_TRY(gode_gn_time_gemm_xout_f32(&yin2, n, d, f->groups, f->eps, f->gamma, f->beta, f->W, d, 1,
-                                                    (float)((double)t0 + i2 * h + C38[s2] * h), Sbuf[(g + 1) & 1],
-                                                    x_out_of(g + 1), stream));
+                if (s2 == 3 && close_once) {
+                    GODE_TRY(gf_last_stage(f, ycur_n, ky_n, h, (float)((double)t0 + i2 * h + C38[s2] * h), Sbuf[(g + 1) & 1],
+                                           x_out_of(g + 1), ky_n[3], &py_formed, stream));
+                } else {
+                    GODE_TRY(gode_gn_time_gemm_xout_f32(&yin2, n, d, f->groups, f->eps, f->gamma, f->beta, f->W, d, 1,
+                                                        (float)((double)t0 + i2 * h + C38[s2] * h), Sbuf[(g + 1) & 1],
+                                                        x_out_of(g + 1), stream));
+                }
                 if (two) GODE_HIP(hipEventRecord(ov->gf, hs));
             }
             if (two) { GODE_HIP(hipStreamWaitEvent(hs, ov->wg, 0)); wg_pending = false; }
@@ -474,6 +516,7 @@
     const int64_t n = f->n, d = f->d, nd = n * d;
     const double h = ((double)t1 - (double)t0) / n_steps;
     const bool fused = fused_small(f);
+    const bool close_once = close_once_route(f);
     if (y0 != save) {
         gode_lincomb_t c; c.n = 1; c.coef[0] = 1.f; c.ptr[0] = y0;
         GODE_TRY(gode_lincomb_f32(save, &c, nd, stream));
@@ -496,13 +539,18 @@
                 }
                 continue;
             }
-            GODE_TRY(gode_gn_time_gemm_f32(&xin, n, d, f->groups, f->eps, f->gamma, f->beta, f->W, d, 1, ts, ws->S, stream));
+            bool p_formed = false;
+            if (s == 3 && close_once) {
+                GODE_TRY(gf_last_stage(f, y, k, h, ts, ws->S, nullptr, ynext, &p_formed, stream));
+            } else {
+                GODE_TRY(gode_gn_time_gemm_f32(&xin, n, d, f->groups, f->eps, f->gamma, f->beta, f->W, d, 1, ts, ws->S, stream));
+            }
             gode_spmm_epilogue_t ep = {};
             ep.bias = f->b; ep.relu = 1; ep.alpha = 1.f;
             if (s < 3) {
                 GODE_TRY(spmm(f->A, ws->S, k[s], d, &ep, stream));
             } else {
-                ep.pre = combine_terms(y, k, h); ep.alpha = (float)(h * B38[3]);
+                ep.pre = p_formed ? one_term(ynext) : combine_terms(y, k, h); ep.alpha = (float)(h * B38[3]);
                 GODE_TRY(spmm_save(f->A, ws->S, ynext, d, &ep, k[3], stream));
             }
         }
diff --git a/graph_odenet_amd/csrc/options.h b/graph_odenet_amd/csrc/options.h
--- a/graph_odenet_amd/csrc/options.h
+++ b/graph_odenet_amd/csrc/options.h
@@ -8,3 +8,4 @@
 int gode_opt_small_fused();
 int gode_opt_bwd_wgrad();
 int gode_opt_y2_colsum();
+int gode_opt_rk_close_once();
diff --git a/graph_odenet_amd/csrc/spmm.hip b/graph_odenet_amd/csrc/spmm.hip
--- a/graph_odenet_amd/csrc/spmm.hip
+++ b/graph_odenet_amd/csrc/spmm.hip
@@ -13,9 +13,11 @@
     float* colpart;
     int64_t colpart_row0;
     float* K;
+    float* Y3;
+    float c3[GODE_MAX_TERMS];
 };
 
-template <int LPR>
+template <int LPR, bool OUT3 = false>
 __device__ __forceinline__ float4 epilogue_store4(const Epilogue& ep, float4 z, int row, int lane,
                                                   int64_t d, float* Y, int64_t ldy) {
     if (ep.bias) {
@@ -35,7 +37,14 @@
     *reinterpret_cast<float4*>(Y + (int64_t)row * ldy + lane * 4) = y;
     if (ep.Y2) {
         const int64_t o = (int64_t)row * d + lane * 4;
-        float4 g = lc_load4(ep.cot, o);
+        float4 g;
+        if (OUT3) {
+            float4 g3;
+            lc_load4_pair(ep.cot, ep.c3, o, g, g3);
+            *reinterpret_cast<float4*>(ep.Y3 + o) = g3;
+        } else {
+            g = lc_load4(ep.cot, o);
+        }
         g.x = z.x > 0.f ? g.x : 0.f; g.y = z.y > 0.f ? g.y : 0.f;
         g.z = z.z > 0.f ? g.z : 0.f; g.w = z.w > 0.f ? g.w : 0.f;
         *reinterpret_cast<float4*>(ep.Y2 + o) = g;
@@ -60,7 +69,7 @@
     }
 }
 
-template <int LPR>
+template <int LPR, bool OUT3 = false>
 __global__ __launch_bounds__(256) void spmm_vec4_kernel(
     const int* __restrict__ rowptr, const int* __restrict__ col, const float* __restrict__ val,
     const int4* __restrict__ items, int n_items, float* __restrict__ partial,
@@ -111,18 +120,18 @@
     if (ep.colpart) {
         float4 g = make_float4(0.f, 0.f, 0.f, 0.f);
         if (active) {
-            if (slot < 0) g = epilogue_store4<LPR>(ep, acc, row, lane, (int64_t)LPR * 4, Y, ldy);
+            if (slot < 0) g = epilogue_store4<LPR, OUT3>(ep, acc, row, lane, (int64_t)LPR * 4, Y, ldy);
             else *reinterpret_cast<float4*>(partial + (int64_t)slot * (LPR * 4) + lane * 4) = acc;
         }
         block_colsum_store<LPR>(g, ep.colpart + (int64_t)blockIdx.x * (LPR * 4));
         return;
     }
     if (!active) return;
-    if (slot < 0) epilogue_store4<LPR>(ep, acc, row, lane, (int64_t)LPR * 4, Y, ldy);
+    if (slot < 0) epilogue_store4<LPR, OUT3>(ep, acc, row, lane, (int64_t)LPR * 4, Y, ldy);
     else *reinterpret_cast<float4*>(partial + (int64_t)slot * (LPR * 4) + lane * 4) = acc;
 }
 
-template <int LPR>
+template <int LPR, bool OUT3 = false>
 __global__ __launch_bounds__(256) void spmm_vec4_wave_kernel(
     const int* __restrict__ rowptr, const int* __restrict__ col, const float* __restrict__ val,
     const int4* __restrict__ items, int n_items, float* __restrict__ partial,
@@ -169,11 +178,11 @@
         acc.z += __shfl_xor(acc.z, off, 64); acc.w += __shfl_xor(acc.w, off, 64);
     }
     if (sub != 0) return;
-    if (slot < 0) epilogue_store4<LPR>(ep, acc, row, lane, (int64_t)LPR * 4, Y, ldy);
+    if (slot < 0) epilogue_store4<LPR, OUT3>(ep, acc, row, lane, (int64_t)LPR * 4, Y, ldy);
     else *reinterpret_cast<float4*>(partial + (int64_t)slot * (LPR * 4) + lane * 4) = acc;
 }
 
-template <int LPR>
+template <int LPR, bool OUT3 = false>
 __global__ __launch_bounds__(256) void spmm_finish_vec4_kernel(
     const int4* __restrict__ long_rows, int n_long, const float* __restrict__ partial,
     float* __restrict__ Y, int64_t ldy, Epilogue ep)
@@ -202,11 +211,11 @@
     }
     if (ep.colpart) {
         float4 g = make_float4(0.f, 0.f, 0.f, 0.f);
-        if (active) g = epilogue_store4<LPR>(ep, acc, lr.x, lane, (int64_t)LPR * 4, Y, ldy);
+        if (active) g = epilogue_store4<LPR, OUT3>(ep, acc, lr.x, lane, (int64_t)LPR * 4, Y, ldy);
         block_colsum_store<LPR>(g, ep.colpart + (ep.colpart_row0 + blockIdx.x) * (LPR * 4));
         return;
     }
-    epilogue_store4<LPR>(ep, acc, lr.x, lane, (int64_t)LPR * 4, Y, ldy);
+    epilogue_store4<LPR, OUT3>(ep, acc, lr.x, lane, (int64_t)LPR * 4, Y, ldy);
 }
 
 __device__ __forceinline__ void epilogue_store1(const Epilogue& ep, float z, int row, int c, int64_t d,
@@ -221,6 +230,13 @@
         const int64_t o = (int64_t)row * d + c;
         const float g = lc_load1(ep.cot, o);
         ep.Y2[o] = z > 0.f ? g : 0.f;
+        if (ep.Y3) {
+            float g3 = 0.f;
+#pragma unroll
+            for (int j = 0; j < GODE_MAX_TERMS; ++j)
+                if (j < ep.cot.n) g3 = fmaf(ep.c3[j], ep.cot.ptr[j][o], g3);
+            ep.Y3[o] = g3;
+        }
     }
 }
 
@@ -292,21 +308,21 @@
     }
 }
 
-template <int LPR>
+template <int LPR, bool OUT3>
 int launch_vec4(const int* rowptr, const int* col, const float* val, const int4* items, int n_items,
                 const int4* long_rows, int n_long, float* partial, const float* X, int64_t ldx,
                 float* Y, int64_t ldy, const Epilogue& ep, hipStream_t s) {
     if (LPR < 64 && n_items > 0 && n_items <= 65536) {
         if (ep.colpart) return GODE_E_UNSUPPORTED;
         const int64_t wb = ((int64_t)n_items * 64 + 255) / 256;
-        const int slot = gode_prof_begin(s, (int64_t)LPR * 4, n_items, (int64_t)ep.pre.n + ep.cot.n + (ep.Y2 ? 1 : 0));
-        hipLaunchKernelGGL(spmm_vec4_wave_kernel<LPR>, dim3((unsigned)wb), dim3(256), 0, s,
+        const int slot = gode_prof_begin(s, (int64_t)LPR * 4, n_items, (int64_t)ep.pre.n + ep.cot.n + (ep.Y2 ? 1 : 0) + (ep.Y3 ? 1 : 0));
+        hipLaunchKernelGGL((spmm_vec4_wave_kernel<LPR, OUT3>), dim3((unsigned)wb), dim3(256), 0, s,
                            rowptr, col, val, items, n_items, partial, X, ldx, Y, ldy, ep);
         gode_prof_end(s, slot);
         GODE_LAUNCH_CHECK();
         if (n_long > 0) {
             const int64_t b2 = ((int64_t)n_long * LPR + 255) / 256;
-            hipLaunchKernelGGL(spmm_finish_vec4_kernel<LPR>, dim3((unsigned)b2), dim3(256), 0, s,
+            hipLaunchKernelGGL((spmm_finish_vec4_kernel<LPR, OUT3>), dim3((unsigned)b2), dim3(256), 0, s,
                                long_rows, n_long, partial, Y, ldy, ep);
             GODE_LAUNCH_CHECK();
         }
@@ -315,8 +331,8 @@
     const int64_t threads = (int64_t)n_items * LPR;
     const int64_t blocks = (threads + 255) / 256;
     if (blocks > 0) {
-        const int slot = gode_prof_begin(s, (int64_t)LPR * 4, n_items, (int64_t)ep.pre.n + ep.cot.n + (ep.Y2 ? 1 : 0));
-        hipLaunchKernelGGL(spmm_vec4_kernel<LPR>, dim3((unsigned)blocks), dim3(256), 0, s,
+        const int slot = gode_prof_begin(s, (int64_t)LPR * 4, n_items, (int64_t)ep.pre.n + ep.cot.n + (ep.Y2 ? 1 : 0) + (ep.Y3 ? 1 : 0));
+        hipLaunchKernelGGL((spmm_vec4_kernel<LPR, OUT3>), dim3((unsigned)blocks), dim3(256), 0, s,
                            rowptr, col, val, items, n_items, partial, X, ldx, Y, ldy, ep);
         gode_prof_end(s, slot);
         GODE_LAUNCH_CHECK();
@@ -325,7 +341,7 @@
         const int64_t b2 = ((int64_t)n_long * LPR + 255) / 256;
         Epilogue ep2 = ep;
         ep2.colpart_row0 = blocks;
-        hipLaunchKernelGGL(spmm_finish_vec4_kernel<LPR>, dim3((unsigned)b2), dim3(256), 0, s,
+        hipLaunchKernelGGL((spmm_finish_vec4_kernel<LPR, OUT3>), dim3((unsigned)b2), dim3(256), 0, s,
                            long_rows, n_long, partial, Y, ldy, ep2);
         GODE_LAUNCH_CHECK();
     }
@@ -373,17 +389,24 @@
     ep.pre = make_lincomb(pre); ep.cot = make_lincomb(cot); ep.Y2 = Y2;
     ep.colpart = (epi && Y2) ? epi->Y2_colsum : nullptr; ep.colpart_row0 = 0;
     ep.K = K;
+    ep.Y3 = (epi && Y2) ? epi->cot_out : nullptr;
+    for (int j = 0; j < GODE_MAX_TERMS; ++j) ep.c3[j] = (ep.Y3 && j < ep.cot.n) ? epi->cot_out_coef[j] : 0.f;
+    if (ep.Y3) {
+        if (ep.Y3 == Y || ep.Y3 == Y2 || ep.Y3 == K) return GODE_E_RANGE;
+        for (int j = 0; j < ep.cot.n; ++j) if (ep.Y3 == ep.cot.ptr[j]) return GODE_E_RANGE;
+    }
     if (ep.colpart && ((((uintptr_t)ep.colpart) & 15) || gode_spmm_y2_colsum_rows(n_items, n_long, d) == 0)) return GODE_E_UNSUPPORTED;
 
     const bool al = !(((uintptr_t)X) & 15) && !(((uintptr_t)Y) & 15) && (ldx % 4 == 0) && (ldy % 4 == 0) &&
                     (!bias || !(((uintptr_t)bias) & 15)) && (!partial || !(((uintptr_t)partial) & 15)) &&
                     (!Y2 || (!(((uintptr_t)Y2) & 15) && lincomb_aligned16(cot))) && lincomb_aligned16(pre) &&
-                    !(((uintptr_t)K) & 15);
+                    !(((uintptr_t)K) & 15) && !(((uintptr_t)ep.Y3) & 15);
     const int4* it4 = reinterpret_cast<const int4*>(items);
     const int4* lr4 = reinterpret_cast<const int4*>(long_rows);
     if (al && d % 4 == 0) {
         switch (d / 4) {
-#define GODE_CASE(L) case L: return launch_vec4<L>(rowptr, col, val, it4, (int)n_items, lr4, (int)n_long, partial, X, ldx, Y, ldy, ep, s);
+#define GODE_CASE(L) case L: return ep.Y3 ? launch_vec4<L, true>(rowptr, col, val, it4, (int)n_items, lr4, (int)n_long, partial, X, ldx, Y, ldy, ep, s) \
+                                        : launch_vec4<L, false>(rowptr, col, val, it4, (int)n_items, lr4, (int)n_long, partial, X, ldx, Y, ldy, ep, s);
             GODE_CASE(1) GODE_CASE(2) GODE_CASE(4) GODE_CASE(8) GODE_CASE(16) GODE_CASE(32) GODE_CASE(64)
 #undef GODE_CASE
             default: break;
@@ -393,7 +416,7 @@
     int G = 1; while (G < d && G < 64) G <<= 1;
     if (d == 1 && it4 != nullptr) {
         const int64_t blocks = ((int64_t)n_items * 64 + 255) / 256;
-        const int slot = gode_prof_begin(s, 1, n_items, (int64_t)ep.pre.n + ep.cot.n + (ep.Y2 ? 1 : 0));
+        const int slot = gode_prof_begin(s, 1, n_items, (int64_t)ep.pre.n + ep.cot.n + (ep.Y2 ? 1 : 0) + (ep.Y3 ? 1 : 0));
         hipLaunchKernelGGL(spmv_wave_kernel, dim3((unsigned)blocks), dim3(256), 0, s,
                            rowptr, col, val, it4, (int)n_items, partial, X, ldx, Y, ldy, ep);
         gode_prof_end(s, slot);
diff --git a/graph_odenet_amd/ops.py b/graph_odenet_amd/ops.py
--- a/graph_odenet_amd/ops.py
+++ b/graph_odenet_amd/ops.py
@@ -28,7 +28,8 @@
     return n
 
 
-def spmm(graph, X, bias=None, relu=False, out=None, cot_terms=None, out2=None, pre_terms=None, alpha=1.0, out2_colsum=None):
+def spmm(graph, X, bias=None, relu=False, out=None, cot_terms=None, out2=None, pre_terms=None, alpha=1.0, out2_colsum=None,
+         cot_out=None, cot_out_coefs=None):
     lib = _lib.load()
     _need(X, "X")
     _need(bias, "bias")
@@ -76,6 +77,15 @@
                 if out2_colsum.numel() != spmm_y2_colsum_rows(graph, d) * d or out2_colsum.numel() == 0:
                     raise ValueError("spmm: out2_colsum must be spmm_y2_colsum_rows(graph, d) x d (and the shape must support it)")
                 ep.Y2_colsum = out2_colsum.data_ptr()
+            if cot_out is not None:
+                _need(cot_out, "cot_out")
+                if cot_out.numel() != graph.n_rows * d or cot_out_coefs is None or len(cot_out_coefs) != len(cot_terms):
+                    raise ValueError("spmm: cot_out must be n_rows x d with one coefficient per cotangent term")
+                ep.cot_out = cot_out.data_ptr()
+                for j, cj in enumerate(cot_out_coefs):
+                    ep.cot_out_coef[j] = float(cj)
+        elif cot_out is not None:
+            raise ValueError("spmm: cot_out needs cot_terms")
     partial = graph.partial(d)
     rc = lib.gode_spmm_csr_f32(ptr(graph.rowptr), ptr(graph.col), ptr(graph.val),
                                ptr(graph.items), graph.n_items,
@@ -164,7 +174,8 @@
     return out
 
 
-def gn_time_gemm(x_terms, n_rows, d_in, groups, eps, gamma, beta, W, has_time, t, out=None, x_out=None):
+def gn_time_gemm(x_terms, n_rows, d_in, groups, eps, gamma, beta, W, has_time, t, out=None, x_out=None, aux_coefs=None,
+                 aux_out=None):
     lib = _lib.load()
     _need(W, "W"); _need(gamma, "gamma"); _need(beta, "beta")
     if _need_terms(x_terms, "x") != n_rows * d_in:
@@ -180,6 +191,15 @@
         _need(x_out, "x_out")
         if x_out.numel() != n_rows * d_in:
             raise ValueError("gn_time_gemm: x_out has wrong size")
+    if aux_out is not None:
+        _need(aux_out, "aux_out")
+        if aux_out.numel() != n_rows * d_in or aux_coefs is None or len(aux_coefs) != len(x_terms):
+            raise ValueError("gn_time_gemm: aux_out must be n_rows x d_in with one coefficient per term")
+        ac = (ctypes.c_float * len(aux_coefs))(*[float(c) for c in aux_coefs])
+        check(lib.gode_gn_time_gemm_xout_aux_f32(ctypes.byref(lc), n_rows, d_in, groups, float(eps), ptr(gamma), ptr(beta),
+                                                 ptr(W), d_out, 1 if has_time else 0, float(t), ptr(out), ptr(x_out),
+                                                 ac, ptr(aux_out), stream_ptr()), "gode_gn_time_gemm_xout_aux_f32")
+        return out
     check(lib.gode_gn_time_gemm_xout_f32(ctypes.byref(lc), n_rows, d_in, groups, float(eps), ptr(gamma), ptr(beta),
                                          ptr(W), d_out, 1 if has_time else 0, float(t), ptr(out), ptr(x_out),
                                          stream_ptr()), "gode_gn_time_gemm_xout_f32")
diff --git a/include/graphode.h b/include/graphode.h
--- a/include/graphode.h
+++ b/include/graphode.h
@@ -36,6 +36,8 @@
     gode_lincomb_t cot;
     float*         Y2;
     float*         Y2_colsum;
+    float*         cot_out;
+    float          cot_out_coef[GODE_MAX_TERMS];
 } gode_spmm_epilogue_t;
 
 int64_t gode_spmm_y2_colsum_rows(int64_t n_items, int64_t n_long, int64_t d);
@@ -82,6 +84,11 @@
                                int32_t groups, float eps, const float* gamma, const float* beta,
                                const float* W, int64_t d_out, int has_time, float t,
                                float* S, float* x_out, void* stream);
+int gode_gn_time_gemm_xout_aux_f32(const gode_lincomb_t* xin , int64_t n_rows, int64_t d_in,
+                                   int32_t groups, float eps, const float* gamma, const float* beta,
+                                   const float* W, int64_t d_out, int has_time, float t,
+                                   float* S, float* x_out , const float* aux_coef ,
+                                   float* aux_out, void* stream);
 
 int gode_gn_time_gemm_pair_f32(const gode_lincomb_t* xin , int64_t n_rows, int64_t d, int32_t groups, float eps,
                                const float* gamma, const float* beta, const float* Wa, const float* Wb,
```
